# chennachaos/PFEMFort

Measured on AMD Instinct MI355X. Metric: DOF/s (assembly+CG-to-tol), higher is better.
Workload: dtype f64

## Files before the change

### include/pfem_amd_diag.h

```cpp
#ifndef PFEM_AMD_DIAG_H
#define PFEM_AMD_DIAG_H

#include "pfem_amd.h"

#ifdef __cplusplus
extern "C" {
#endif

#define PFEM_ASSEMBLY_GATHER 0
#define PFEM_ASSEMBLY_SCATTER 1
int pfem_solver_set_assembly_mode(pfem_solver *s, int mode);
int pfem_solver_assembly_info(pfem_solver *s, int *gather_form, int *hub_nodes, int *block_threads, int64_t *lds_bytes);
#define PFEM_SPMV_AUTO 0
#define PFEM_SPMV_INT32 1
#define PFEM_SPMV_GAPS16 2
#define PFEM_SPMV_GROUPED 3
int pfem_solver_set_spmv_format(pfem_solver *s, int format);
int pfem_solver_get_spmv_format(pfem_solver *s, int *bits_per_column);
int pfem_solver_get_spmv_row_group(pfem_solver *s, int *rows_per_lane);
int pfem_solver_get_spmv_gap_table(pfem_solver *s, int *entries);
int pfem_solver_get_spmv_value_dictionary(pfem_solver *s, int *entries);
int pfem_solver_amg_value_dictionaries(pfem_solver *s, int max_levels, int *n_levels, int *entries);
int pfem_solver_get_spmv_gap_escapes(pfem_solver *s, int *in_use);
int pfem_solver_spmv_bytes(pfem_solver *s, int64_t *format_bytes);

int pfem_solver_amg_info(pfem_solver *s, int max_levels, int *n_levels, int64_t *rows, int64_t *nnz, double *lambda_max,
                         double *symbolic_ms, double *numeric_ms, int *cheb_degree, int *fine_degree, double *eig_ratio, double *coarse_scale);
int pfem_solver_amg_aggregates(pfem_solver *s, int level, int32_t *agg);
int pfem_solver_amg_transfer(pfem_solver *s, int level, int *rbm, int *fine_bs, int *coarse_bs, int *dim, int64_t *n_nodes, double *node_xyz);
int pfem_solver_amg_layout(pfem_solver *s, int max_levels, int *coupled, int *distributed_levels, int64_t *first_dof, int64_t *local_rows);
int pfem_solver_incidence_patterns(pfem_solver *s, int *count, int *longest);
int pfem_solver_amg_aggregation(pfem_solver *s, int max_levels, int *n_levels, int *kind);
int pfem_solver_amg_comm_counts(pfem_solver *s, int *exchanges_per_cycle, int *allreduces_per_cycle);
int pfem_solver_amg_cycle_profile(pfem_solver *s, int max_levels, int *n_levels, int *exchanges, double *exchange_ms,
                                  int64_t *exchange_doubles, int *allreduces, double *allreduce_ms, int64_t *allreduce_doubles,
                                  double *cycle_ms);
int pfem_solver_amg_pairing(pfem_solver *s, int *lattice_levels);
int pfem_solver_amg_cycle(pfem_solver *s, int *cycle, int *last_level_visited_twice);
int pfem_solver_amg_level0_epilogue(pfem_solver *s, int *taken);
int pfem_solver_amg_galerkin_from_codes(pfem_solver *s, int *taken);
int pfem_solver_amg_level_values(pfem_solver *s, int level, int64_t max_values, double *vals, int64_t *stored);

int pfem_eval_elems(pfem_solver *s, const double *elemData, const double *timeData,
                    double *K_out, double *F_out);

int pfem_matrix_info(pfem_solver *s, int64_t *n_owned, int64_t *n_local, int64_t *nnz,
                     int64_t *stored_entries);

int pfem_spmv(pfem_solver *s, const double *x, double *y);
int pfem_bench_spmv(pfem_solver *s, int reps, double *ms_per_launch);

typedef struct pfem_timings {
    double pattern_ms;
    double assemble_ms;
    double solve_ms;
    double spmv_ms_total;
    int64_t spmv_launches;
    double upload_ms;
    double event_overhead_ms;
    double iface_ms_total;
    double scalar_ms_total;
    int64_t comm_samples;
    double exposed_ms_total;
    int64_t graph_iterations;
    double host_enqueue_ms;
    int64_t host_enqueued_iterations;
    double host_comm_ms;
} pfem_timings;
int pfem_get_timings(pfem_solver *s, pfem_timings *t);
int pfem_solver_profile_spmv(pfem_solver *s, int enable);

int pfem_solver_comm_selftest(pfem_solver *s, int64_t count, int64_t *bad);
int pfem_solver_comm_bench(pfem_solver *s, int64_t count, int reps, double *ms_per_exchange, double *ms_per_allreduce);
int pfem_solver_comm_bench_sizes(pfem_solver *s, int64_t count, int64_t allreduce_count, int reps, int slab_neighbours,
                                 double *ms_per_exchange, double *ms_per_allreduce);
int pfem_solver_comm_info(pfem_solver *s, int *n_peers, int64_t *doubles_per_exchange, int64_t *boundary_slices,
                          int64_t *total_slices);
int pfem_solver_comm_describe(pfem_solver *s, char *backend, int backend_len, int *backend_ranks, int *backend_device,
                              int *backend_version, int *solver_device, int *overlapped_form);

#ifdef __cplusplus
}
#endif
#endif
```

### pfemfort_amd/_lib.py

```python
from __future__ import annotations

import ctypes as C
import os

_HERE = os.path.dirname(os.path.abspath(__file__))
LIB_PATH = os.environ.get("PFEM_AMD_LIB") or os.path.join(_HERE, "libpfem_amd.so")

OK, ERR_ARG, ERR_STATE, ERR_NEG_JAC, ERR_HIP, ERR_NOGPU, ERR_NOMEM, ERR_DIVERGED, ERR_PATTERN, ERR_COMM = range(10)
POISSON_TRIA, POISSON_TET, ELAST_TET, POISSON_TRIA_INLINE, ELAST_TRIA = 1, 2, 3, 4, 5
SOLVER_EMPTY, PATTERN_OK, INIT_OK, ASSEMBLY_OK, FACTORISE_OK = 1, 2, 3, 4, 5
INSERT_VALUES, ADD_VALUES = 1, 2

NPELEM = {POISSON_TRIA: 3, POISSON_TET: 4, ELAST_TET: 4, POISSON_TRIA_INLINE: 3, ELAST_TRIA: 3}
NDOF = {POISSON_TRIA: 1, POISSON_TET: 1, ELAST_TET: 3, POISSON_TRIA_INLINE: 1, ELAST_TRIA: 2}
NDIM = {POISSON_TRIA: 2, POISSON_TET: 3, ELAST_TET: 3, POISSON_TRIA_INLINE: 2, ELAST_TRIA: 2}


class PfemError(RuntimeError):
    def __init__(self, code: int, where: str, detail: str = ""):
        self.code = code
        msg = f"{where}: error {code} ({_strerror(code)})"
        if detail:
            msg += f" -- {detail}"
        super().__init__(msg)
# ... 8 lines not shown
                ("host_comm_ms", C.c_double)]


HOST_ALLREDUCE_FN = C.CFUNCTYPE(C.c_int, C.c_void_p, C.POINTER(C.c_double), C.c_int64)
HOST_EXCHANGE_FN = C.CFUNCTYPE(C.c_int, C.c_void_p, C.c_int, C.POINTER(C.c_int), C.POINTER(C.c_int64),
                               C.POINTER(C.c_double), C.POINTER(C.c_double))
RCCL_ID_BYTES = 256

_P = C.c_void_p
_I, _L, _D = C.c_int, C.c_int64, C.c_double

SIGNATURES = {
    "pfem_version": [],
    "pfem_strerror": [_I],
    "pfem_last_error_string": [],
    "pfem_device_count": [_P],
    "pfem_device_info": [_I, _P, _I, _P, _P, _P],
    "pfem_device_memory": [_I, _P, _P],
    "pfem_poisson_tria_ke": [_P] * 7,
    "pfem_poisson_tet_ke": [_P] * 8,
    "pfem_elast_tet_ke": [_P] * 8,
    "pfem_elast_tria_ke": [_P] * 7,
    "pfem_gen_box_tets": [_D, _D, _I, _D, _D, _I, _D, _D, _I, _I, _I, _I, _I, _P, _P, _P, _P, _P, _P],
    "pfem_dof_numbering": [_L, _I, _L, _P, _P, _P, _I, _P, _P, _P, _P, _P, _P, _P, _P, _P, _P],
    "pfem_renumber_mesh": [_L, _I, _L, _I, _P, _P, _P, _P, _P, _P],
    "pfem_elem_dof_array": [_L, _I, _I, _P, _P, _P],
    "pfem_assy_for_soln": [_L, _I, _P, _P],
    "pfem_partition_box_slabs": [_I, _I, _I, _I, _P, _P],
    "pfem_partition_box_slabs_axis": [_I, _I, _I, _I, _I, _P, _P],
    "pfem_partition_rcb": [_L, _I, _P, _L, _I, _P, _I, _P, _P],
    "pfem_text_table_shape": [C.c_char_p, _L, _P, _P],
    "pfem_text_table_parse": [C.c_char_p, _L, _L, _I, _P],
    "pfem_write_vtk": [C.c_char_p, _I, _L, _L, _I, _I, _P, _P, _P, _P],
    "pfem_write_temp_dat": [C.c_char_p, _L, _P, _P, _P],
    "pfem_solver_create": [_P, _L, _L, _L, _P, _P, _I],
    "pfem_solver_destroy": [_P],
    "pfem_solver_set_stream": [_P, _P],
    "pfem_solver_set_tolerances": [_P, _D, _D, _D, _I],
    "pfem_solver_status": [_P, _P],
    "pfem_solver_set_zero": [_P],
    "pfem_solver_print_info": [_P],
    "pfem_mat_set_values": [_P, _I, _P, _I, _P, _P, _I],
    "pfem_vec_set_values": [_P, _I, _P, _P, _I],
    "pfem_solver_assemble_matrix_and_vector": [_P, _I, _P, _P, _P, _P],
    "pfem_solver_factorise": [_P],
    "pfem_solver_solve": [_P, _P, _P, _P],
    "pfem_solver_factorise_and_solve": [_P, _P, _P, _P],
    "pfem_solver_get_solution": [_P, _P],
    "pfem_solver_get_history": [_P, _P, _I, _P],
    "pfem_mesh_upload": [_P, _I, _L, _P, _L, _P, _P, _P],
    "pfem_box_slab_sizes": [_I, _I, _I, _I, _I, _I, _I, _P, _P, _P, _P, _P],
    "pfem_mesh_generate_box": [_P, _I, _D, _D, _I, _D, _D, _I, _D, _D, _I, _I, _I, _I],
    "pfem_box_slab_sizes_axis": [_I, _I, _I, _I, _I, _I, _I, _I, _P, _P, _P, _P, _P, _P, _P, _P],
    "pfem_mesh_generate_box_axis": [_P, _I, _D, _D, _I, _D, _D, _I, _D, _D, _I, _I, _I, _I, _I],
    "pfem_mesh_download": [_P, _P, _P, _P, _P],
    "pfem_pattern_build": [_P],
    "pfem_assemble": [_P, _P, _P],
    "pfem_solver_set_assembly_mode": [_P, _I],
    "pfem_solver_assembly_info": [_P, _P, _P, _P, _P],
    "pfem_solver_set_spmv_format": [_P, _I],
    "pfem_solver_get_spmv_format": [_P, _P],
    "pfem_solver_get_spmv_row_group": [_P, _P],
    "pfem_solver_get_spmv_gap_table": [_P, _P],
    "pfem_solver_get_spmv_value_dictionary": [_P, _P],
    "pfem_solver_amg_value_dictionaries": [_P, _I, _P, _P],
    "pfem_solver_get_spmv_gap_escapes": [_P, _P],
    "pfem_solver_spmv_bytes": [_P, _P],
    "pfem_solver_set_preconditioner": [_P, _I],
    "pfem_solver_get_preconditioner": [_P, _P],
    "pfem_solver_set_cg_single_reduction": [_P, _I],
    "pfem_solver_amg_info": [_P, _I, _P, _P, _P, _P, _P, _P, _P, _P, _P, _P],
    "pfem_solver_amg_aggregates": [_P, _I, _P],
    "pfem_solver_amg_transfer": [_P, _I, _P, _P, _P, _P, _P, _P],
    "pfem_solver_amg_layout": [_P, _I, _P, _P, _P, _P],
    "pfem_solver_amg_aggregation": [_P, _I, _P, _P],
    "pfem_solver_incidence_patterns": [_P, _P, _P],
    "pfem_solver_amg_comm_counts": [_P, _P, _P],
    "pfem_solver_amg_cycle_profile": [_P, _I, _P, _P, _P, _P, _P, _P, _P, _P],
    "pfem_solver_amg_pairing": [_P, _P],
    "pfem_solver_set_amg_options": [_P, _I, _I, _D, _D],
    "pfem_solver_set_amg_cycle": [_P, _I],
    "pfem_solver_amg_cycle": [_P, _P, _P],
    "pfem_solver_amg_level0_epilogue": [_P, _P],
    "pfem_solver_amg_galerkin_from_codes": [_P, _P],
    "pfem_solver_amg_level_values": [_P, _I, _L, _P, _P],
    "pfem_eval_elems": [_P, _P, _P, _P, _P],
    "pfem_rhs_add_values": [_P, _L, _P, _P],
    "pfem_matrix_info": [_P, _P, _P, _P, _P],
    "pfem_get_local_to_global": [_P, _P],
    "pfem_get_csr": [_P, _P, _P, _P],
    "pfem_get_rhs": [_P, _P],
    "pfem_spmv": [_P, _P, _P],
    "pfem_bench_spmv": [_P, _I, _P],
    "pfem_get_timings": [_P, _P],
    "pfem_solver_profile_spmv": [_P, _I],
    "pfem_neighbour_plan": [_I, _I, _P, _P, _P, _P, _P, _P, _P, _P, _P],
    "pfem_solver_set_neighbours": [_P, _I, _P, _P, _P],
    "pfem_rccl_unique_id": [_P],
    "pfem_solver_set_comm_rccl": [_P, _I, _I, _P],
    "pfem_solver_set_comm_host": [_P, _I, _I, HOST_ALLREDUCE_FN, HOST_EXCHANGE_FN, _P],
    "pfem_solver_comm_bench": [_P, C.c_int64, _I, _P, _P],
    "pfem_solver_comm_bench_sizes": [_P, C.c_int64, C.c_int64, _I, _I, _P, _P],
    "pfem_solver_set_comm_peer": [_P, _I, _I, HOST_ALLREDUCE_FN, HOST_EXCHANGE_FN, _P],
    "pfem_solver_comm_shutdown": [_P],
    "pfem_solver_comm_info": [_P, _P, _P, _P, _P],
    "pfem_solver_comm_describe": [_P, _P, _I, _P, _P, _P, _P, _P],
    "pfem_solver_comm_selftest": [_P, _L, _P],
    "pfem_get_ghosts": [_P, _P, _P],
    "pfem_find_ghosts": [_L, _P, _L, _L, _P, _P],
}
_RESTYPES = {"pfem_strerror": C.c_char_p, "pfem_last_error_string": C.c_char_p}

_lib = None


def lib() -> C.CDLL:
    global _lib
    if _lib is None:
        if not os.path.exists(LIB_PATH):
            raise ImportError(
                f"{LIB_PATH} not found: build the HIP extension first "
                "(python -c 'import __graft_entry__ as g; g.build()'). pfemfort_amd has no CPU fallback.")
        L = C.CDLL(LIB_PATH)
        for name, args in SIGNATURES.items():
            fn = getattr(L, name)
            fn.argtypes = args
            fn.restype = _RESTYPES.get(name, C.c_int)
        _lib = L
    return _lib


def _strerror(code: int) -> str:
    try:
        return lib().pfem_strerror(code).decode()
    except Exception:
        return "?"


def check(rc: int, where: str) -> None:
    if rc != OK:
        raise PfemError(rc, where, lib().pfem_last_error_string().decode())


def device_count() -> int:
    n = C.c_int(0)
    check(lib().pfem_device_count(C.byref(n)), "pfem_device_count")
    return n.value


def device_memory(device: int = 0) -> dict:
    f = C.c_int64(0); t = C.c_int64(0)
    check(lib().pfem_device_memory(device, C.byref(f), C.byref(t)), "pfem_device_memory")
    return {"free_bytes": f.value, "total_bytes": t.value}


def device_info(device: int = 0) -> dict:
    name = C.create_string_buffer(256)
    cu = C.c_int(0); mem = C.c_int64(0); clk = C.c_int(0)
    check(lib().pfem_device_info(device, name, 256, C.byref(cu), C.byref(mem), C.byref(clk)), "pfem_device_info")
    return {"name": name.value.decode(), "compute_units": cu.value, "hbm_bytes": mem.value, "clock_khz": clk.value}
```

### pfemfort_amd/csrc/pfem_amg.inc

```

constexpr int kAmgMaxLevels = 14;
constexpr int kAmgMatchRounds = 8;
constexpr int kAmgPasses = 3;
constexpr int64_t kAmgReplicateRows = 150000;
constexpr int kAmgRetryBlock = -7701;

inline bool amg_in_effect(const pfem_solver *s)
{
    return s->pc == PFEM_PC_GAMG;
}

inline SellDev amg_sell(const pfem_solver *s, const AmgLevel &L, int64_t rows)
{
    SellDev A;
    if (L.fine) {
        A = s->sell();
    } else {
        A.slice_off = L.slice_off.p;
        A.rowlen = L.rowlen.p;
        A.cols = L.cols.p;
        A.vals = L.vals.p;
    }
    A.n_rows = rows;
    A.n_slices = (rows + 63) / 64;
// ... 467 lines not shown
    PFEM_TRY(cand.reserve(static_cast<size_t>(n)));
    PFEM_TRY(is_root.reserve(static_cast<size_t>(n) + 1));
    PFEM_TRY(rank.reserve(static_cast<size_t>(n) + 1));
    PFEM_HIP(hipMemsetAsync(match.p, 0xff, sizeof(int32_t) * n, s->stream));
    const int64_t *gptr = G.ptr.p;
    const int32_t *gcol = G.col.p;
    const double *gw = G.w.p, *gd = G.diag.p;
    hipLaunchKernelGGL(k_amg_lat_pick, dim3(grid_for(n)), dim3(kBlock), 0, s->stream, n, gptr, gcol, gw, gd, pos, shift, cand.p);
    hipLaunchKernelGGL(k_amg_match_commit, dim3(grid_for(n)), dim3(kBlock), 0, s->stream, n, static_cast<const int32_t *>(cand.p), match.p);
    if (absorb) {
        hipLaunchKernelGGL(k_amg_lat_absorb, dim3(grid_for(n)), dim3(kBlock), 0, s->stream, n, gptr, gcol, gw, gd, pos, shift,
                           static_cast<const int32_t *>(match.p), cand.p);
        hipLaunchKernelGGL(k_amg_lat_join, dim3(grid_for(n)), dim3(kBlock), 0, s->stream, n, static_cast<const int32_t *>(cand.p), match.p);
    }
    PFEM_TRY(check_kernel("k_amg_lat_*"));
    PFEM_HIP(hipMemsetAsync(is_root.p + n, 0, sizeof(int32_t), s->stream));
    hipLaunchKernelGGL(k_amg_match_finish, dim3(grid_for(n)), dim3(kBlock), 0, s->stream, n, match.p, is_root.p);
    PFEM_TRY(amg_exclusive_sum(s, temp, is_root.p, rank.p, n + 1));
    PFEM_TRY(agg_step.reserve(static_cast<size_t>(n)));
    hipLaunchKernelGGL(k_amg_agg_ids, dim3(grid_for(n)), dim3(kBlock), 0, s->stream, n, static_cast<const int32_t *>(match.p),
                       static_cast<const int32_t *>(rank.p), agg_step.p);
    PFEM_TRY(check_kernel("k_amg_agg_ids"));
    int32_t total = 0;
    PFEM_HIP(hipMemcpyAsync(&total, rank.p + n, sizeof(int32_t), hipMemcpyDeviceToHost, s->stream));
    PFEM_HIP(hipStreamSynchronize(s->stream));
    *na = total;
    return PFEM_OK;
}

int amg_sell_from_keys(pfem_solver *s, AmgWork &W, const uint64_t *ukeys, int64_t nnz, AmgLevel &C)
{
    DevBuf<char> &temp = W.temp;
    const int64_t n = C.n_loc;
    C.nnz = nnz;
    C.n_slices = (n + 63) / 64;
    PFEM_TRY(C.rowptr.alloc(static_cast<size_t>(n) + 1));
    PFEM_TRY(C.rowlen.alloc(static_cast<size_t>(std::max<int64_t>(n, 1))));
    PFEM_TRY(C.slice_off.alloc(static_cast<size_t>(C.n_slices) + 1));
    DevBuf<int64_t> &slice_entries = W.slice_entries;
    PFEM_TRY(slice_entries.reserve(static_cast<size_t>(C.n_slices) + 1));
    hipLaunchKernelGGL(k_row_bounds, dim3(grid_for(std::max<int64_t>(nnz, n + 1))), dim3(kBlock), 0, s->stream, ukeys, nnz, n, C.rowptr.p);
    hipLaunchKernelGGL(k_slice_sizes, dim3(grid_for(C.n_slices * 64)), dim3(kBlock), 0, s->stream, static_cast<const int64_t *>(C.rowptr.p), n,
                       C.n_slices, C.rowlen.p, slice_entries.p);
    PFEM_TRY(check_kernel("k_slice_sizes (gamg)"));
    PFEM_TRY(amg_exclusive_sum(s, temp, slice_entries.p, C.slice_off.p, C.n_slices + 1));
    int64_t stored = 0;
    PFEM_HIP(hipMemcpyAsync(&stored, C.slice_off.p + C.n_slices, sizeof(int64_t), hipMemcpyDeviceToHost, s->stream));
    PFEM_HIP(hipStreamSynchronize(s->stream));
    C.stored = stored;
    PFEM_TRY(C.cols.alloc(static_cast<size_t>(std::max<int64_t>(stored, 1))));
    PFEM_TRY(C.vals.alloc(static_cast<size_t>(std::max<int64_t>(stored, 1))));
    hipLaunchKernelGGL(k_fill_sell, dim3(grid_for(C.n_slices * 64)), dim3(kBlock), 0, s->stream, ukeys, static_cast<const int64_t *>(C.rowptr.p), n,
                       C.n_slices, static_cast<const int64_t *>(C.slice_off.p), C.cols.p);
    PFEM_TRY(check_kernel("k_fill_sell (gamg)"));
    PFEM_HIP(hipMemsetAsync(C.vals.p, 0, sizeof(double) * std::max<int64_t>(stored, 1), s->stream));
    return PFEM_OK;
}

int amg_alloc_vectors(pfem_solver *s, AmgLevel &L)
{
    const size_t n = static_cast<size_t>(std::max<int64_t>(L.n_loc, 1));
    const size_t g = L.fine ? static_cast<size_t>(kVecGuard) : 0;
    const size_t nv = n;
    PFEM_TRY(L.dinv.alloc(n));
    PFEM_TRY(L.t.alloc(nv));
    PFEM_TRY(L.r.alloc(n));
    if (!L.fine) PFEM_TRY(L.b.alloc(n));
    PFEM_TRY(L.x_store.alloc(nv + 2 * g));
    PFEM_TRY(L.dd_store.alloc(nv + 2 * g));
    PFEM_HIP(hipMemsetAsync(L.x_store.p, 0, sizeof(double) * (nv + 2 * g), s->stream));
    PFEM_HIP(hipMemsetAsync(L.dd_store.p, 0, sizeof(double) * (nv + 2 * g), s->stream));
    L.x = L.x_store.p + g;
    L.dd = L.dd_store.p + g;
    PFEM_TRY(L.lam.alloc(1));
    PFEM_TRY(L.part_max.alloc(static_cast<size_t>(grid_for((L.n_loc + 63) / 64 * 64))));
    return PFEM_OK;
}

inline bool amg_galerkin_by_entry()
{
    static const bool v = std::getenv("PFEM_AMG_GALERKIN_MAPS") != nullptr;
    return v;
}
inline void amg_galerkin(pfem_solver *s, const AmgLevel &L, AmgLevel &C, const SellDev &A, bool extras = false, VdState *vstate = nullptr,
                         bool from_codes = false)
{
    C.bound_fresh = C.vd_direct = false;
    if (L.code_of.p && !amg_galerkin_by_entry()) {
        if (C.n_loc < 1) return;
        LatGalExtra X{nullptr, nullptr, nullptr, nullptr, nullptr};
        if (extras && C.dinv.p && C.t.p && C.n_loc == C.n) {
            X.dinv_out = C.dinv.p;
            X.ratio_out = C.t.p;
            C.bound_fresh = true;
            if (vstate && C.vd_have_dict && C.vd_hash_ok && C.vhash.p && C.vcodes.p && C.vcodes.n >= static_cast<size_t>(C.stored) && !C.vd_refused) {
                const VdState reset{C.vd_n, 0, 0, 0};
                (void)hipMemcpyAsync(vstate, &reset, sizeof reset, hipMemcpyHostToDevice, s->stream);
                X.vhash = C.vhash.p;
                X.codes = C.vcodes.p;
                X.vstate = vstate;
                C.vd_direct = true;
            }
        }
        if (from_codes) {
            hipLaunchKernelGGL(k_lat_galerkin_codes, dim3(static_cast<unsigned>((C.n_loc + kLatGalThreads - 1) / kLatGalThreads)), dim3(kLatGalThreads),
                               sizeof(double) * static_cast<size_t>(std::max(s->vd_n, 1)), s->stream, C.n_loc, static_cast<const int32_t *>(L.mem_ptr.p),
                               static_cast<const int32_t *>(L.mem_idx.p), static_cast<const int64_t *>(s->d_rslice_off.p),
                               static_cast<const unsigned long long *>(s->d_vcodes.p), static_cast<const uint32_t *>(L.glat.p),
                               static_cast<const double *>(s->d_vdict.p), s->vd_n, static_cast<const uint32_t *>(L.code_mask.p),
                               static_cast<const int64_t *>(C.slice_off.p), C.vals.p, X);
            return;
        }
        hipLaunchKernelGGL(k_lat_galerkin, dim3(static_cast<unsigned>((C.n_loc + kLatGalThreads - 1) / kLatGalThreads)), dim3(kLatGalThreads), 0, s->stream, A, C.n_loc,
                           static_cast<const int32_t *>(L.mem_ptr.p), static_cast<const int32_t *>(L.mem_idx.p), static_cast<const uint8_t *>(L.code_of.p),
                           static_cast<const uint32_t *>(L.code_mask.p), static_cast<const int64_t *>(C.slice_off.p), C.vals.p, X);
        return;
    }
    hipLaunchKernelGGL(k_amg_galerkin, dim3(grid_for(L.nnz_c)), dim3(kBlock), 0, s->stream, L.nnz_c, static_cast<const int64_t *>(L.src_ptr.p),
                       static_cast<const int32_t *>(L.src_slot.p), static_cast<const int64_t *>(L.dst_slot.p),
                       static_cast<const double *>(A.vals), C.vals.p);
}

int amg_couple_level(pfem_solver *s, AmgWork &W, AmgLevel &L, AmgLevel &C, bool overlap, int cb, const std::vector<double> *nc_of)
{
    std::vector<int64_t> rank_off;
    if (cb > 0 && nc_of) {
        rank_off.assign(nc_of->size() + 1, 0);
        for (size_t q = 0; q < nc_of->size(); ++q) rank_off[q + 1] = rank_off[q] + static_cast<int64_t>((*nc_of)[q]);
    }
    auto node_base = [&](int64_t g) -> int64_t {
        const size_t q = static_cast<size_t>(std::upper_bound(rank_off.begin(), rank_off.end(), g) - rank_off.begin()) - 1;
        return rank_off[q] + (g - rank_off[q]) / cb * cb;
    };
    const PlanRef P = amg_plan(s, L);
    const std::vector<int32_t> &fine_lidx = L.fine ? s->h_send_lidx : L.plan.send_lidx;
    const int64_t n = L.n, n_loc = L.n_loc, n_ghost = n_loc - n, nc = C.n;
    double bad = s->nranks > 52 ? 1.0 : 0.0;
    DevBuf<double> &v = W.vals;
    DevBuf<double> &w = W.svals;
    DevBuf<double> d_mask, d_gm;
    DevBuf<int32_t> d_table;
    DevBuf<uint64_t> &gkeys = W.keys, &gskeys = W.skeys, &gukeys = W.ukeys;
    DevBuf<int32_t> &gidx = W.idx, &gsidx = W.skey32;
    DevBuf<int64_t> &gstart = W.start;
    {
        int rc = v.reserve(static_cast<size_t>(std::max<int64_t>(n_loc, 1)));
        if (rc == PFEM_OK) rc = w.reserve(static_cast<size_t>(std::max<int64_t>(n_loc, 1)));
        if (rc == PFEM_OK) rc = d_mask.alloc(static_cast<size_t>(std::max<int64_t>(nc, 1)));
        if (rc == PFEM_OK) rc = d_gm.alloc(static_cast<size_t>(std::max<int64_t>(n_ghost, 1)));
        if (rc == PFEM_OK) rc = d_table.alloc(static_cast<size_t>(std::max<int64_t>(n_ghost, 1)));
        if (rc == PFEM_OK) rc = gkeys.reserve(static_cast<size_t>(std::max<int64_t>(n_ghost, 1)));
        if (rc == PFEM_OK) rc = gskeys.reserve(static_cast<size_t>(std::max<int64_t>(n_ghost, 1)));
        if (rc == PFEM_OK) rc = gidx.reserve(static_cast<size_t>(std::max<int64_t>(n_ghost, 1)));
        if (rc == PFEM_OK) rc = gsidx.reserve(static_cast<size_t>(std::max<int64_t>(n_ghost, 1)));
        if (rc == PFEM_OK) rc = W.head.reserve(static_cast<size_t>(n_ghost) + 1);
        if (rc == PFEM_OK) rc = W.rank.reserve(static_cast<size_t>(n_ghost) + 1);
        if (rc == PFEM_OK) rc = gukeys.reserve(static_cast<size_t>(std::max<int64_t>(n_ghost, 1)));
        if (rc == PFEM_OK) rc = gstart.reserve(static_cast<size_t>(n_ghost) + 1);
        if (rc == PFEM_OK && n_ghost > 0) {
            size_t tb = 0;
            if (hipcub::DeviceRadixSort::SortPairs(nullptr, tb, gkeys.p, gskeys.p, gidx.p, gsidx.p, static_cast<int>(n_ghost), 0, 40, s->stream) != hipSuccess) rc = PFEM_ERR_HIP;
            if (rc == PFEM_OK && tb > W.temp.n) { (void)hipStreamSynchronize(s->stream); rc = W.temp.alloc(tb); }
            size_t ts = 0;
            if (rc == PFEM_OK && hipcub::DeviceScan::ExclusiveSum(nullptr, ts, W.head.p, W.rank.p, static_cast<int>(n_ghost + 1), s->stream) != hipSuccess) rc = PFEM_ERR_HIP;
            if (rc == PFEM_OK && ts > W.temp.n) { (void)hipStreamSynchronize(s->stream); rc = W.temp.alloc(ts); }
        }
        PFEM_TRY(amg_agree(s, rc));
    }
    bool self_peer = false;
    for (int k = 0; k < P.np; ++k) self_peer = self_peer || P.peers[k] == s->rank;
    const double undo = self_peer ? 0.5 : 1.0;
    auto as_id = [undo](double x) { return static_cast<int64_t>(undo * x + 0.5); };
    hipLaunchKernelGGL(k_amg_gid_vector, dim3(grid_for(n_loc)), dim3(kBlock), 0, s->stream, n, n_loc, static_cast<const int32_t *>(L.agg.p), C.gid_off, v.p);
    PFEM_TRY(check_kernel("k_amg_gid_vector"));
    PFEM_TRY(exchange_sum(s, P, v.p, overlap));
    std::vector<double> h_sh(static_cast<size_t>(P.n_send));
    std::vector<uint64_t> h_ug;
    int64_t m_g = 0;
    {
        auto ghosts = [&]() -> int {
            if (P.n_send > 0) {
                hipLaunchKernelGGL(k_pack_send, dim3(grid_for(P.n_send)), dim3(kBlock), 0, s->stream, static_cast<const double *>(v.p), P.send_lidx, P.n_send,
                                   s->d_send.p, static_cast<const CgCtl *>(nullptr));
                PFEM_HIP(hipMemcpyAsync(h_sh.data(), s->d_send.p, sizeof(double) * h_sh.size(), hipMemcpyDeviceToHost, s->stream));
            }
            if (n_ghost > 0) {
                hipLaunchKernelGGL(k_amg_ghost_keys, dim3(grid_for(n_ghost)), dim3(kBlock), 0, s->stream, n_ghost, static_cast<const double *>(v.p + n), undo,
                                   gkeys.p, gidx.p);
                size_t tb = W.temp.n;
                PFEM_HIP(hipcub::DeviceRadixSort::SortPairs(W.temp.p, tb, gkeys.p, gskeys.p, gidx.p, gsidx.p, static_cast<int>(n_ghost), 0, 40, s->stream));
                PFEM_TRY(amg_unique_runs(s, W, gskeys.p, n_ghost, gukeys, gstart, &m_g, false));
                h_ug.resize(static_cast<size_t>(m_g));
                if (m_g > 0) PFEM_HIP(hipMemcpyAsync(h_ug.data(), gukeys.p, sizeof(uint64_t) * h_ug.size(), hipMemcpyDeviceToHost, s->stream));
            }
            PFEM_HIP(hipStreamSynchronize(s->stream));
            return PFEM_OK;
        };
        const int rc = ghosts();
        if (rc != PFEM_OK) bad = 1.0;
    }
    std::vector<int32_t> table;
    C.ghost_gid.clear();
    if (cb > 0) {
// ... 1452 lines not shown
        }
        if (L.bs > 1) {
            PFEM_TRY(C.node_of.alloc(static_cast<size_t>(nc)));
            PFEM_TRY(C.comp_of.alloc(static_cast<size_t>(nc)));
            hipLaunchKernelGGL(k_amg_coarse_nodes, dim3(grid_for(nslots)), dim3(kBlock), 0, s->stream, nslots, L.bs,
                               static_cast<const int32_t *>(flag.p), static_cast<const int32_t *>(rank.p), C.node_of.p, C.comp_of.p);
            PFEM_TRY(check_kernel("k_amg_coarse_nodes"));
        }
        {
            DevBuf<int32_t> &cnt = W.cnt, &idx = W.idx, &skey = W.skey32;
            PFEM_TRY(cnt.reserve(static_cast<size_t>(nc_loc) + 1));
            PFEM_TRY(idx.reserve(static_cast<size_t>(std::max<int64_t>(R, 1))));
            PFEM_TRY(skey.reserve(static_cast<size_t>(std::max<int64_t>(R, 1))));
            PFEM_TRY(L.mem_ptr.alloc(static_cast<size_t>(nc_loc) + 1));
            PFEM_TRY(L.mem_idx.alloc(static_cast<size_t>(std::max<int64_t>(R, 1))));
            PFEM_HIP(hipMemsetAsync(cnt.p, 0, sizeof(int32_t) * (nc_loc + 1), s->stream));
            hipLaunchKernelGGL(k_amg_count, dim3(grid_for(R)), dim3(kBlock), 0, s->stream, R, static_cast<const int32_t *>(L.agg.p), cnt.p);
            PFEM_TRY(amg_exclusive_sum(s, temp, cnt.p, L.mem_ptr.p, nc_loc + 1));
            hipLaunchKernelGGL(k_amg_iota, dim3(grid_for(R)), dim3(kBlock), 0, s->stream, R, idx.p);
            size_t tb = 0;
            const int ni = static_cast<int>(R);
            PFEM_HIP(hipcub::DeviceRadixSort::SortPairs(nullptr, tb, L.agg.p, skey.p, idx.p, L.mem_idx.p, ni, 0, 32, s->stream));
            if (tb > temp.n) { PFEM_HIP(hipStreamSynchronize(s->stream)); PFEM_TRY(temp.alloc(tb)); }
            PFEM_HIP(hipcub::DeviceRadixSort::SortPairs(temp.p, tb, L.agg.p, skey.p, idx.p, L.mem_idx.p, ni, 0, 32, s->stream));
            PFEM_HIP(hipStreamSynchronize(s->stream));
        }
        phase(l, "coarse dofs + member lists");
        {
            DevBuf<uint64_t> &keys = W.keys, &skeys = W.skeys;
            DevBuf<uint64_t> ukeys;
            DevBuf<int32_t> &slots = W.slots;
            PFEM_TRY(keys.reserve(static_cast<size_t>(L.stored)));
            PFEM_TRY(slots.reserve(static_cast<size_t>(L.stored)));
            PFEM_HIP(hipMemsetAsync(keys.p, 0xff, sizeof(uint64_t) * static_cast<size_t>(L.stored), s->stream));
            PFEM_HIP(hipMemsetAsync(slots.p, 0, sizeof(int32_t) * static_cast<size_t>(L.stored), s->stream));
            const SellDev Ar = amg_sell(s, L, R);
            hipLaunchKernelGGL(k_amg_emit_rap_keys, dim3(grid_for(Ar.n_slices * 64)), dim3(kBlock), 0, s->stream, Ar,
                               static_cast<const int32_t *>(L.agg.p), static_cast<int32_t>(R), keys.p, slots.p);
            PFEM_TRY(check_kernel("k_amg_emit_rap_keys"));
            PFEM_TRY(skeys.reserve(static_cast<size_t>(L.stored)));
            PFEM_TRY(L.src_slot.alloc(static_cast<size_t>(L.stored)));
            const int ni = static_cast<int>(L.stored);
            size_t tb = 0;
            PFEM_HIP(hipcub::DeviceRadixSort::SortPairs(nullptr, tb, keys.p, skeys.p, slots.p, L.src_slot.p, ni, 0, 64, s->stream));
            if (tb > temp.n) { PFEM_HIP(hipStreamSynchronize(s->stream)); PFEM_TRY(temp.alloc(tb)); }
            PFEM_HIP(hipcub::DeviceRadixSort::SortPairs(temp.p, tb, keys.p, skeys.p, slots.p, L.src_slot.p, ni, 0, 64, s->stream));
            PFEM_HIP(hipStreamSynchronize(s->stream));
            int64_t nnz_c = 0;
            PFEM_TRY(amg_unique_runs(s, W, skeys.p, L.stored, ukeys, L.src_ptr, &nnz_c));
            if (nnz_c > 0) {
                uint64_t last = 0;
                PFEM_HIP(hipMemcpyAsync(&last, ukeys.p + (nnz_c - 1), sizeof(uint64_t), hipMemcpyDeviceToHost, s->stream));
                PFEM_HIP(hipStreamSynchronize(s->stream));
                if (last == ~0ull) --nnz_c;
            }
            L.nnz_c = nnz_c;
            PFEM_TRY(amg_sell_from_keys(s, W, ukeys.p, nnz_c, C));
            PFEM_TRY(L.dst_slot.alloc(static_cast<size_t>(std::max<int64_t>(nnz_c, 1))));
            hipLaunchKernelGGL(k_amg_dst_slots, dim3(grid_for(nnz_c)), dim3(kBlock), 0, s->stream, nnz_c, static_cast<const uint64_t *>(ukeys.p),
                               static_cast<const int64_t *>(C.rowptr.p), static_cast<const int64_t *>(C.slice_off.p), L.dst_slot.p);
            PFEM_TRY(check_kernel("k_amg_dst_slots"));
            PFEM_HIP(hipStreamSynchronize(s->stream));
        }
        phase(l, "Galerkin maps + coarse pattern");
        if (coupled) PFEM_TRY(amg_agree(s, C.stored > INT_MAX ? PFEM_ERR_ARG : PFEM_OK));
        else if (C.stored > INT_MAX) return PFEM_ERR_ARG;
        M.lev.push_back(std::move(Cp));
        {
            AmgLevel &Cn = *M.lev.back();
            amg_galerkin(s, L, Cn, A);
            PFEM_TRY(check_kernel("k_amg_galerkin (symbolic)"));
        }
        n_global = nc_global;
        if (coupled && n_global > kAmgDense && n_global <= static_cast<double>(replicate_rows)) {
            PFEM_TRY(amg_replicate(s, M, W, *M.lev.back(), static_cast<int64_t>(n_global), overlap));
            phase(l, "replicated levels");
            break;
        }
    }
    M.n_last_global = coupled ? static_cast<int64_t>(n_global) : M.lev.back()->n;
    return PFEM_OK;
}

int amg_finish_levels(pfem_solver *s, Amg &M, bool coupled)
{
    for (auto &L : M.lev) PFEM_TRY(amg_alloc_vectors(s, *L));
    AmgLevel &last = *M.lev.back();
    const int64_t n_last = M.n_last_global;
    M.dense = n_last >= 1 && n_last <= kAmgDense && M.lev.size() > 1 && !M.rep;
    if (M.dense) {
        PFEM_TRY(M.dense_inv.alloc(static_cast<size_t>(n_last * n_last)));
        const int bytes = static_cast<int>(n_last * n_last * sizeof(double));
        if (bytes > 65536) {
            PFEM_HIP(hipFuncSetAttribute(reinterpret_cast<const void *>(k_amg_dense_inverse), hipFuncAttributeMaxDynamicSharedMemorySize, bytes));
            PFEM_HIP(hipFuncSetAttribute(reinterpret_cast<const void *>(k_amg_dense_inverse_of), hipFuncAttributeMaxDynamicSharedMemorySize, bytes));
        }
        if (coupled) {
            PFEM_TRY(M.dense_glob.alloc(static_cast<size_t>(n_last * n_last)));
            PFEM_TRY(M.bx_glob.alloc(static_cast<size_t>(2 * kAmgDense)));
            PFEM_TRY(amg_level_gids(s, last));
        }
    }
    if (coupled) PFEM_TRY(M.lam_all.alloc(static_cast<size_t>(std::max<int64_t>(256, 2 * static_cast<int64_t>(M.lev.size()) * s->nranks))));
    M.fused = !coupled && [] { const char *e = std::getenv("PFEM_AMG_FUSED"); return e ? std::atoi(e) != 0 : true; }();
    M.tail_from = -1;
    for (size_t l = 1; l < M.lev.size() && !coupled; ++l)
        if (M.lev[l]->n <= kAmgTailRows && M.lev[l]->nnz <= kAmgTailNnz && M.lev.size() - l <= static_cast<size_t>(kAmgTailLevels)) { M.tail_from = static_cast<int>(l); break; }
    M.w_to = M.tail_from > 0 ? M.tail_from : static_cast<int>(M.lev.size()) - 2;
    M.tail_lds_allowed = 0;
    if (M.tail_from > 0) {
        int64_t rows = 0;
        for (size_t l = static_cast<size_t>(M.tail_from); l < M.lev.size(); ++l) rows += M.lev[l]->n;
        const AmgLevel &T0 = *M.lev[static_cast<size_t>(M.tail_from)];
        const size_t need = static_cast<size_t>(6 * rows) * sizeof(double) + static_cast<size_t>(T0.stored) * 12 + static_cast<size_t>((T0.n + 63) / 64 + 2) * 8;
        if (need > 65536 && need <= 156 * 1024) {
            if (hipFuncSetAttribute(reinterpret_cast<const void *>(k_amg_tail), hipFuncAttributeMaxDynamicSharedMemorySize, static_cast<int>(need)) == hipSuccess)
                M.tail_lds_allowed = need;
            else
                (void)hipGetLastError();
        }
    }
    return PFEM_OK;
}


void amg_knobs(Amg &M)
{
    const char *er = std::getenv("PFEM_AMG_EIG_RATIO"), *cs = std::getenv("PFEM_AMG_COARSE_SCALE");
    M.eig_ratio = er ? std::max(1.5, std::atof(er)) : (M.eig_ratio_given ? M.eig_ratio_opt : M.eig_ratio_auto);
    M.coarse_scale = cs ? std::atof(cs) : (M.coarse_scale_given ? M.coarse_scale_opt : M.coarse_scale_auto);
    if (M.rep) { M.rep->eig_ratio = M.eig_ratio; M.rep->coarse_scale = M.coarse_scale; }
}

int amg_symbolic(pfem_solver *s, bool multi, bool overlap)
{
    if (!s->amg) s->amg.reset(new (std::nothrow) Amg());
    if (!s->amg) return PFEM_ERR_NOMEM;
    Amg &M = *s->amg;
    const auto t0 = std::chrono::steady_clock::now();
    const bool verbose = std::getenv("PFEM_AMG_VERBOSE") != nullptr;
    const size_t malloc_calls0 = dev_pool().st_malloc_calls;
    const size_t malloc_bytes0 = dev_pool().st_malloc;
    const double malloc_ms0 = dev_pool().st_malloc_ms;
    const size_t reused0 = dev_pool().st_reused;
    auto since_t0 = [&](const char *what) {
        if (!verbose) return;
        (void)hipStreamSynchronize(s->stream);
        std::fprintf(stderr, "  gamg symbolic: %-40s at %9.2f ms\n", what, std::chrono::duration<double, std::milli>(std::chrono::steady_clock::now() - t0).count());
    };
    M.coupled = multi && !M.coupled_refused && [] { const char *e = std::getenv("PFEM_AMG_COUPLED"); return e ? std::atoi(e) != 0 : true; }();
    const bool coupled = M.coupled;
    if (const char *e = std::getenv("PFEM_AMG_CHEB_DEGREE")) M.cheb_degree = std::max(1, std::min(6, std::atoi(e)));
    if (const char *e = std::getenv("PFEM_AMG_FINE_DEGREE")) M.fine_degree = std::max(0, std::min(6, std::atoi(e)));
    M.lev.clear();
    M.rep.reset();
    M.rbm = false;
    M.symbolic_ok = false;
    M.dense = false;
    M.graph.invalidate();
    {
        const int rc_size = s->stored > INT_MAX ? PFEM_ERR_ARG : PFEM_OK;
        if (rc_size != PFEM_OK) set_last_error("gamg: more than 2^31-1 stored matrix entries on one device");
        if (coupled) PFEM_TRY(amg_agree(s, rc_size));
        else PFEM_TRY(rc_size);
    }
    std::unique_ptr<AmgWork> Wp(new (std::nothrow) AmgWork());
    if (!Wp) return PFEM_ERR_NOMEM;
    AmgWork &W = *Wp;
    {
        std::unique_ptr<AmgLevel> L0(new (std::nothrow) AmgLevel());
        if (!L0) return PFEM_ERR_NOMEM;
        L0->fine = true;
        L0->n = s->n_owned;
        L0->n_loc = s->n_loc;
        L0->gid_off = s->row_start;
        L0->n_slices = (s->n_owned + 63) / 64;
        L0->stored = s->stored;
        L0->nnz = s->nnz;
        int64_t owned_groups = s->n_groups;
        if (s->grouped && s->n_groups > 0 && s->n_ghost > 0) {
            std::vector<int32_t> row0(static_cast<size_t>(s->n_groups));
            PFEM_HIP(hipMemcpyAsync(row0.data(), s->d_group_row0.p, sizeof(int32_t) * row0.size(), hipMemcpyDeviceToHost, s->stream));
            PFEM_HIP(hipStreamSynchronize(s->stream));
            owned_groups = std::lower_bound(row0.begin(), row0.end(), static_cast<int32_t>(s->n_owned)) - row0.begin();
        }
        if (s->grouped && owned_groups > 0 && owned_groups < s->n_owned) {
            L0->bs = kGroupRows;
            L0->n_nodes = owned_groups;
            PFEM_TRY(L0->node_of.alloc(static_cast<size_t>(s->n_loc)));
            PFEM_TRY(L0->comp_of.alloc(static_cast<size_t>(s->n_loc)));
            hipLaunchKernelGGL(k_row_group_index, dim3(grid_for(s->n_groups)), dim3(kBlock), 0, s->stream,
                               static_cast<const int32_t *>(s->d_group_row0.p), s->n_groups, L0->node_of.p);
            hipLaunchKernelGGL(k_amg_comp_of, dim3(grid_for(s->n_loc)), dim3(kBlock), 0, s->stream, s->n_loc,
                               static_cast<const int32_t *>(L0->node_of.p), static_cast<const int32_t *>(s->d_group_row0.p), L0->comp_of.p);
            PFEM_TRY(check_kernel("k_amg_comp_of"));
        } else {
            L0->bs = 1;
            L0->n_nodes = s->n_owned;
        }
        if (!multi || coupled) {
            const int nd = s->mesh.ndof;
            bool cand = s->have_mesh && nd == s->mesh.ndim && nd >= 2 && s->n_owned % nd == 0 && s->n_loc % nd == 0 && (multi || s->n_owned >= 2 * nd);
            const int64_t nn0 = cand ? s->n_loc / nd : 0;
// ... 238 lines not shown
    if (any_old) {
        PFEM_TRY(read_states());
        for (int l : cand) {
            AmgLevel &L = *M.lev[static_cast<size_t>(l)];
            if (!L.vd_have_dict) continue;
            if (st[static_cast<size_t>(l)].miss) build.push_back(l);
            else { L.vd_ok = true; L.vd_hash_ok = L.vhash.p != nullptr; }
        }
    }
    if (build.empty()) return PFEM_OK;
    for (int l : build) {
        AmgLevel &L = *M.lev[static_cast<size_t>(l)];
        const unsigned grid = static_cast<unsigned>(std::min<int64_t>((L.stored + kBlock - 1) / kBlock, 4096));
        PFEM_HIP(hipMemsetAsync(L.vtable.p, 0xff, sizeof(unsigned long long) * kVdTable, s->stream));
        PFEM_HIP(hipMemsetAsync(M.vd_states.p + l, 0, sizeof(VdState), s->stream));
        hipLaunchKernelGGL(k_vd_collect, dim3(grid), dim3(kBlock), 0, s->stream, static_cast<const double *>(L.vals.p), L.stored, L.vtable.p, M.vd_states.p + l);
        hipLaunchKernelGGL(k_vd_finish, dim3(1), dim3(1024), 0, s->stream, static_cast<const unsigned long long *>(L.vtable.p), L.vdict.p, M.vd_states.p + l);
        PFEM_TRY(check_kernel("k_vd_collect / k_vd_finish (coarse level)"));
        L.vd_hash_ok = false;
        if (!L.vhash.p) PFEM_TRY(L.vhash.alloc(kVdHashSlots));
        PFEM_HIP(hipMemsetAsync(L.vhash.p, 0xff, sizeof(VdHashEntry) * kVdHashSlots, s->stream));
        hipLaunchKernelGGL(k_vd_hash_build, dim3((kVdMax + kBlock - 1) / kBlock), dim3(kBlock), 0, s->stream, static_cast<const double *>(L.vdict.p),
                           static_cast<const VdState *>(M.vd_states.p + l), L.vhash.p);
        PFEM_TRY(check_kernel("k_vd_hash_build (coarse level)"));
        PFEM_TRY(encode(L, l));
    }
    PFEM_TRY(read_states());
    for (int l : build) {
        AmgLevel &L = *M.lev[static_cast<size_t>(l)];
        const VdState &v = st[static_cast<size_t>(l)];
        if (v.fail || v.count < 1 || v.count > kVdMax || v.miss) {
            L.vd_ok = L.vd_have_dict = L.vd_hash_ok = false;
            L.vd_refused = true;
        } else {
            L.vd_n = v.count;
            L.vd_have_dict = true;
            L.vd_ok = true;
            L.vd_hash_ok = L.vhash.p != nullptr;
        }
        if (std::getenv("PFEM_VD_VERBOSE"))
            std::fprintf(stderr, "  value dictionary, level %d: %d distinct values among %lld slots%s\n", l, v.count, static_cast<long long>(L.stored),
                         L.vd_ok ? "" : " -- the level keeps its fp64 values");
    }
    return PFEM_OK;
}

int amg_level0_codes(pfem_solver *s, Amg &M, AmgLevel &L, bool *yes)
{
    *yes = false;
    const char *e = std::getenv("PFEM_AMG_GALERKIN_CODES");
    if (e && std::atoi(e) == 0) return PFEM_OK;
    if (&M != s->amg.get() || M.coupled || M.rbm || cg_multi(s) || !L.fine || L.rbm || L.bs != 1 || !L.code_of.p || !L.code_mask.p || amg_galerkin_by_entry() ||
        s->n_hubs != 0 || L.stored != s->stored || L.glat_refused)
        return PFEM_OK;
    if (!valdict_enabled() || !s->use_rel() || s->rel_gap32 || s->vd_rows != kRelRows || !(s->vd_ok && s->vd_current && s->vd_have_dict) || s->vd_miss_step ||
        s->vd_n < 1 || s->vd_n > kVdMax || !s->d_vcodes.p || !s->d_vdict.p || !s->d_relk.p || !s->d_rslice_off.p || s->r_stored < 1 ||
        s->d_vcodes.n < static_cast<size_t>(s->r_stored))
        return PFEM_OK;
    if (!L.glat.p || L.glat_for != s->r_stored) {
        PFEM_TRY(L.glat.alloc(static_cast<size_t>(s->r_stored)));
        L.glat_for = -1;
        PFEM_HIP(hipMemsetAsync(L.glat.p, 0xff, sizeof(uint32_t) * static_cast<size_t>(s->r_stored), s->stream));
        PFEM_HIP(hipMemsetAsync(s->d_err.p, 0, sizeof(int), s->stream));
        hipLaunchKernelGGL(k_lat_group_codes, dim3(grid_for(L.n)), dim3(kBlock), 0, s->stream, amg_sell(s, L), static_cast<const uint8_t *>(L.code_of.p),
                           static_cast<const uint8_t *>(s->d_relk.p), static_cast<const int64_t *>(s->d_rslice_off.p), reinterpret_cast<uint8_t *>(L.glat.p),
                           s->d_err.p);
        PFEM_TRY(check_kernel("k_lat_group_codes"));
        int bad = 0;
        PFEM_TRY(fetch_err(s, &bad));
        PFEM_HIP(hipMemsetAsync(s->d_err.p, 0, sizeof(int), s->stream));
        if (bad) { L.glat.release(); L.glat_refused = true; return PFEM_OK; }
        L.glat_for = s->r_stored;
    }
    *yes = true;
    return PFEM_OK;
}

int amg_numeric(pfem_solver *s, Amg &M, bool overlap)
{
    M.galerkin_from_codes = false;
    if (M.coupled) return amg_numeric_coupled(s, M, overlap);
    const bool fresh = M.galerkin_fresh;
    M.galerkin_fresh = false;
    for (size_t l = 0; l < M.lev.size(); ++l) {
        AmgLevel &L = *M.lev[l];
        const SellDev A = amg_sell(s, L);
        if (l + 1 < M.lev.size() && !fresh) {
            AmgLevel &C = *M.lev[l + 1];
            if (L.rbm) amg_rbm_galerkin(s, L, C, A);
            else {
                bool from_codes = false;
                if (l == 0) PFEM_TRY(amg_level0_codes(s, M, L, &from_codes));
                amg_galerkin(s, L, C, A, !M.rbm && !M.coupled, M.vd_states.p ? M.vd_states.p + (l + 1) : nullptr, from_codes);
                if (from_codes) M.galerkin_from_codes = true;
                if (l == 0 && std::getenv("PFEM_VD_VERBOSE"))
                    std::fprintf(stderr, "  gamg numeric: level 1 summed from %s\n", from_codes ? "the SpMV's value codes" : "the fp64 row form");
            }
        }
        const unsigned g = grid_for(A.n_slices * 64);
        if (!L.fine && L.bound_fresh && !fresh) {
            L.bound_fresh = false;
            if (L.n > 65536) {
                const unsigned gm = std::min<unsigned>(g, 512u);
                hipLaunchKernelGGL(k_amg_max_rows, dim3(gm), dim3(kBlock), 0, s->stream, static_cast<const double *>(L.t.p), L.n, L.part_max.p);
                hipLaunchKernelGGL(k_amg_max, dim3(1), dim3(1024), 0, s->stream, static_cast<const double *>(L.part_max.p), static_cast<int64_t>(gm), L.lam.p);
            } else {
                hipLaunchKernelGGL(k_amg_max, dim3(1), dim3(1024), 0, s->stream, static_cast<const double *>(L.t.p), L.n, L.lam.p);
            }
            continue;
        }
        if (L.fine && s->asm_bound_fresh && &M == s->amg.get()) {
            const unsigned gm = std::min<unsigned>(g, 2048u);
            hipLaunchKernelGGL(k_amg_max_rows, dim3(gm), dim3(kBlock), 0, s->stream, static_cast<const double *>(L.t.p), L.n, L.part_max.p);
            hipLaunchKernelGGL(k_amg_max, dim3(1), dim3(1024), 0, s->stream, static_cast<const double *>(L.part_max.p), static_cast<int64_t>(gm), L.lam.p);
            s->asm_bound_fresh = false;
        } else {
        hipLaunchKernelGGL(k_amg_diag_bound, dim3(g), dim3(kBlock), 0, s->stream, A, static_cast<int32_t>(L.n), L.dinv.p, L.part_max.p);
        hipLaunchKernelGGL(k_amg_max, dim3(1), dim3(1024), 0, s->stream, static_cast<const double *>(L.part_max.p), static_cast<int64_t>(g), L.lam.p);
        }
        if (M.rbm) {
            if (!M.lam2.p) PFEM_TRY(M.lam2.alloc(1));
            hipLaunchKernelGGL(k_rbm_bound_sym, dim3(g), dim3(kBlock), 0, s->stream, A, static_cast<int32_t>(L.n), static_cast<const double *>(L.dinv.p),
                               static_cast<double *>(nullptr), L.part_max.p);
            hipLaunchKernelGGL(k_amg_max, dim3(1), dim3(1024), 0, s->stream, static_cast<const double *>(L.part_max.p), static_cast<int64_t>(g), M.lam2.p);
            hipLaunchKernelGGL(k_rbm_min2, dim3(1), dim3(64), 0, s->stream, static_cast<const double *>(M.lam2.p), L.lam.p);
        }
    }
    PFEM_TRY(check_kernel("gamg numeric"));
    if (M.dense) {
        AmgLevel &L = *M.lev.back();
        hipLaunchKernelGGL(k_amg_dense_inverse, dim3(1), dim3(1024), static_cast<size_t>(L.n * L.n) * sizeof(double), s->stream, amg_sell(s, L),
                           M.dense_inv.p);
        PFEM_TRY(check_kernel("k_amg_dense_inverse"));
    }
    return amg_value_codes(s, M);
}

inline void amg_rbm_restrict_launch(pfem_solver *s, const AmgLevel &L, AmgLevel &C, int64_t nc_nodes, int64_t nn, const double *b, const double *t, double ratio,
                                    double *dd_c, double *x_c, const CgCtl *ctl, int64_t n_own_nodes)
{
    static const bool wide_on = [] { const char *e = std::getenv("PFEM_RBM_RESTRICT_WIDE"); return e ? std::atoi(e) != 0 : true; }();
    const bool wide = wide_on && nc_nodes > 0 && nn >= 16 * nc_nodes;
    if (wide) {
        PFEM_RBM_DISPATCH(L.bs, L.dim, hipLaunchKernelGGL((k_rbm_restrict_wide<FB, DIM>), dim3(grid_for(nc_nodes * kRbmWide)), dim3(kBlock), 0, s->stream, nc_nodes,
            static_cast<const int32_t *>(L.mem_ptr.p), static_cast<const int32_t *>(L.mem_idx.p), static_cast<const double *>(L.roff.p), nn,
            b, t, C.b.p, static_cast<const double *>(C.dinv.p), static_cast<const double *>(C.lam.p), ratio, dd_c, x_c, ctl, n_own_nodes));
    } else {
        PFEM_RBM_DISPATCH(L.bs, L.dim, hipLaunchKernelGGL((k_rbm_restrict<FB, DIM>), dim3(grid_for(nc_nodes)), dim3(kBlock), 0, s->stream, nc_nodes,
            static_cast<const int32_t *>(L.mem_ptr.p), static_cast<const int32_t *>(L.mem_idx.p), static_cast<const double *>(L.roff.p), nn,
            b, t, C.b.p, static_cast<const double *>(C.dinv.p), static_cast<const double *>(C.lam.p), ratio, dd_c, x_c, ctl, n_own_nodes));
    }
}

int amg_smooth(pfem_solver *s, const Amg &M, AmgLevel &L, const double *b, bool zero_guess, int deg, const CgCtl *ctl, bool first_done = false,
               bool overlap = false)
{
    const int64_t nv = amg_rows(M, L);
    const unsigned gv = vec_grid(nv);
    const double *t0 = nullptr;
    const PlanRef P = M.coupled ? amg_plan(s, L) : PlanRef{};
    const bool cf = M.coupled && M.coupled_fused && P.row_sh != nullptr;
    const ShareSum S = cf ? ShareSum{P.row_sh, P.sh_ptr, P.sh_src, s->d_recv.p} : ShareSum{nullptr, nullptr, nullptr, nullptr};
    auto product = [&](const double *x) -> int {
        if (!cf) {
            amg_spmv(s, M, L, x, L.t.p);
            if (M.coupled) PFEM_TRY(exchange_sum(s, P, L.t.p, overlap, ctl));
            return PFEM_OK;
        }
        if (L.fine) {
            amg_spmv(s, M, L, x, L.t.p);
            if (P.n_send > 0)
                hipLaunchKernelGGL(k_pack_send, dim3(grid_for(P.n_send)), dim3(kBlock), 0, s->stream, static_cast<const double *>(L.t.p), P.send_lidx, P.n_send,
                                   s->d_send.p, ctl);
        } else {
            const SellDev A = amg_sell(s, L, nv);
            if (L.vd_ok && L.vcodes.p)
                hipLaunchKernelGGL(k_amg_spmv_pack_vd, dim3(spmv_grid(A.n_slices)), dim3(kBlock), sizeof(double) * static_cast<size_t>(L.vd_n), s->stream, A,
                                   static_cast<const uint16_t *>(L.vcodes.p), static_cast<const double *>(L.vdict.p), L.vd_n, x, L.t.p, S, s->d_send.p, ctl);
            else
            hipLaunchKernelGGL(k_amg_spmv_pack, dim3(spmv_grid(A.n_slices)), dim3(kBlock), 0, s->stream, A, x, L.t.p, S, s->d_send.p, ctl);
        }
        return exchange_only(s, P, overlap);
    };
    if (!zero_guess) {
        PFEM_TRY(product(L.x));
        t0 = L.t.p;
    }
    double *r_store = (deg > 1 && !zero_guess) ? L.r.p : nullptr;
    if (!first_done)
        hipLaunchKernelGGL(k_amg_cheb_first, dim3(gv), dim3(kBlock), 0, s->stream, nv, b, t0, static_cast<const double *>(L.dinv.p),
                           static_cast<const double *>(L.lam.p), M.eig_ratio, r_store, deg > 1 ? L.dd : static_cast<double *>(nullptr), L.x, ctl, S);
    const double *r_in = zero_guess ? b : L.r.p;
    for (int k = 1; k < deg; ++k) {
        PFEM_TRY(product(L.dd));
        const bool more = k + 1 < deg;
        hipLaunchKernelGGL(k_amg_cheb_next, dim3(gv), dim3(kBlock), 0, s->stream, nv, k, r_in, static_cast<const double *>(L.t.p),
                           static_cast<const double *>(L.dinv.p), static_cast<const double *>(L.lam.p), M.eig_ratio, more ? L.r.p : nullptr,
                           static_cast<const double *>(L.dd), more ? L.dd : nullptr, L.x, ctl, S);
        r_in = L.r.p;
    }
    return PFEM_OK;
}

enum { kLast0Smooth = 0, kLast0Product = 1, kLast0Epilogue = 2 };
double *amg_apply(pfem_solver *s, Amg &M, const double *r, const CgCtl *ctl, bool first0_done = false, int last0 = kLast0Smooth);
double *amg_apply_coupled(pfem_solver *s, Amg &M, const double *r, const CgCtl *ctl, bool overlap)
{
    const int nl = static_cast<int>(M.lev.size());
    {
// ... 46 lines not shown
        if (amg_smooth(s, M, L, b, true, deg_of(l), ctl, false, overlap) != PFEM_OK) return nullptr;
        amg_spmv(s, M, L, L.x, L.t.p);
        if (L.rbm)
            amg_rbm_restrict_launch(s, L, C, C.n_loc / C.bs, L.n_loc / L.bs, b, static_cast<const double *>(L.t.p), M.eig_ratio, nullptr, nullptr, ctl, L.n_nodes);
        {
            const PlanRef PC = amg_plan(s, C);
            const bool cf = M.coupled_fused && PC.row_sh != nullptr && !L.rbm;
            const ShareSum SC = cf ? ShareSum{PC.row_sh, PC.sh_ptr, PC.sh_src, s->d_recv.p} : ShareSum{nullptr, nullptr, nullptr, nullptr};
            if (!L.rbm)
            hipLaunchKernelGGL(k_amg_restrict, dim3(grid_for(C.n_loc)), dim3(kBlock), 0, s->stream, C.n_loc, static_cast<const int32_t *>(L.mem_ptr.p),
                           static_cast<const int32_t *>(L.mem_idx.p), b, static_cast<const double *>(L.t.p), C.b.p, static_cast<const double *>(C.dinv.p),
                           static_cast<const double *>(C.lam.p), M.eig_ratio, static_cast<double *>(nullptr), static_cast<double *>(nullptr), ctl,
                           static_cast<int32_t>(L.n), SC, s->d_send.p);
            if (cf) {
                if (exchange_only(s, PC, overlap) != PFEM_OK) return nullptr;
                if (PC.n_sh > 0)
                    hipLaunchKernelGGL(k_unpack_sum, dim3(grid_for(PC.n_sh)), dim3(kBlock), 0, s->stream, C.b.p, PC.sh_lidx, PC.sh_ptr, PC.sh_src, PC.n_sh,
                                       static_cast<const double *>(s->d_recv.p), ctl);
            } else if (exchange_sum(s, PC, C.b.p, overlap, ctl) != PFEM_OK) {
                return nullptr;
            }
        }
    }
    for (int l = nl - 2; l >= 0; --l) {
        AmgLevel &L = *M.lev[static_cast<size_t>(l)];
        AmgLevel &C = *M.lev[static_cast<size_t>(l) + 1];
        const double *b = l == 0 ? r : L.b.p;
        s->xprof_level = l;
        if (L.rbm) {
            PFEM_RBM_DISPATCH(L.bs, L.dim, hipLaunchKernelGGL((k_rbm_prolong<FB, DIM>), dim3(vec_grid(L.n_loc / L.bs)), dim3(kBlock), 0, s->stream, L.n_loc / L.bs,
                static_cast<const int32_t *>(L.node_agg.p), static_cast<const double *>(L.roff.p), L.n_loc / L.bs, static_cast<const double *>(C.x),
                M.coarse_scale, L.x, ctl));
        } else
        hipLaunchKernelGGL(k_amg_prolong, dim3(vec_grid(L.n_loc)), dim3(kBlock), 0, s->stream, L.n_loc, static_cast<const int32_t *>(L.agg.p),
                           static_cast<const double *>(C.x), M.coarse_scale, L.x, ctl);
        if (amg_smooth(s, M, L, b, false, deg_of(l), ctl, false, overlap) != PFEM_OK) return nullptr;
    }
    return M.lev[0]->x;
}

double *amg_apply(pfem_solver *s, Amg &M, const double *r, const CgCtl *ctl, bool first0_done, int last0)
{
    const int nl = static_cast<int>(M.lev.size());
    if (M.lev[0]->fine && s->n_ghost > 0) (void)hipMemsetAsync(M.lev[0]->x + s->n_owned, 0, sizeof(double) * static_cast<size_t>(s->n_ghost), s->stream);
    const bool fuse = M.fused && M.cheb_degree == 2;
    const int tail = (M.fused && M.tail_from > 0) ? M.tail_from : nl;
    auto deg_of = [&](int l) { return (l == 0 && M.fine_degree > 0) ? M.fine_degree : M.cheb_degree; };
    auto fused_level = [&](int l) { return fuse && l >= 1 && l < tail && l < nl - 1; };
    auto ep = [&](int mode, AmgLevel &L, const double *xin, const double *r_in, int step, int add_dd0, double *r_out, double *dd_out, double *x) {
        const SellDev A = amg_sell(s, L);
        const dim3 grid(spmv_grid(A.n_slices)), block(kBlock);
        const double *dinv = L.dinv.p, *lam = L.lam.p;
        if (L.gptr.p && (L.bs == 6 || L.bs == 3)) {
            const int64_t *gp = L.gptr.p;
            const int32_t *gc = L.gcol.p;
#define PFEM_BLK_EP(MODEV, CBV) hipLaunchKernelGGL((k_rbm_spmv_ep<MODEV, CBV>), grid, block, 0, s->stream, A, gp, gc, xin, r_in, dinv, lam, M.eig_ratio, step, add_dd0, r_out, dd_out, x, ctl)
            if (L.bs == 6) { if (mode == kEpNextLast) PFEM_BLK_EP(kEpNextLast, 6); else if (mode == kEpResid) PFEM_BLK_EP(kEpResid, 6); else PFEM_BLK_EP(kEpFirstRes, 6); }
            else { if (mode == kEpNextLast) PFEM_BLK_EP(kEpNextLast, 3); else if (mode == kEpResid) PFEM_BLK_EP(kEpResid, 3); else PFEM_BLK_EP(kEpFirstRes, 3); }
#undef PFEM_BLK_EP
            return;
        }
        if (L.vd_ok && L.vcodes.p) {
            const uint16_t *q = L.vcodes.p;
            const double *d = L.vdict.p;
            const size_t lds = sizeof(double) * static_cast<size_t>(L.vd_n);
            if (mode == kEpNextLast) hipLaunchKernelGGL(k_amg_spmv_ep_vd<kEpNextLast>, grid, block, lds, s->stream, A, q, d, L.vd_n, xin, r_in, dinv, lam, M.eig_ratio, step, add_dd0, r_out, dd_out, x, ctl);
            else if (mode == kEpResid) hipLaunchKernelGGL(k_amg_spmv_ep_vd<kEpResid>, grid, block, lds, s->stream, A, q, d, L.vd_n, xin, r_in, dinv, lam, M.eig_ratio, step, add_dd0, r_out, dd_out, x, ctl);
            else hipLaunchKernelGGL(k_amg_spmv_ep_vd<kEpFirstRes>, grid, block, lds, s->stream, A, q, d, L.vd_n, xin, r_in, dinv, lam, M.eig_ratio, step, add_dd0, r_out, dd_out, x, ctl);
            return;
        }
        if (mode == kEpNextLast) hipLaunchKernelGGL(k_amg_spmv_ep<kEpNextLast>, grid, block, 0, s->stream, A, xin, r_in, dinv, lam, M.eig_ratio, step, add_dd0, r_out, dd_out, x, ctl);
        else if (mode == kEpResid) hipLaunchKernelGGL(k_amg_spmv_ep<kEpResid>, grid, block, 0, s->stream, A, xin, r_in, dinv, lam, M.eig_ratio, step, add_dd0, r_out, dd_out, x, ctl);
        else hipLaunchKernelGGL(k_amg_spmv_ep<kEpFirstRes>, grid, block, 0, s->stream, A, xin, r_in, dinv, lam, M.eig_ratio, step, add_dd0, r_out, dd_out, x, ctl);
    };
    auto run_tail = [&]() {
        AmgTail T{};
        T.nlev = nl - tail;
        T.deg = M.cheb_degree;
        T.coarsest_deg = M.coarsest_sweeps;
        T.dense_n = M.dense ? static_cast<int>(M.lev.back()->n) : 0;
        T.dense_inv = M.dense_inv.p;
        T.ratio = M.eig_ratio;
        T.scale = M.coarse_scale;
        for (int q = 0; q < T.nlev; ++q) {
            AmgLevel &L = *M.lev[static_cast<size_t>(tail + q)];
            AmgTailLevel &t = T.lev[q];
            t.A = amg_sell(s, L);
            t.dinv = L.dinv.p; t.lam = L.lam.p;
            t.x = L.x; t.dd = L.dd; t.t = L.t.p; t.r = L.r.p; t.b = L.b.p;
            t.agg = L.agg.p; t.mem_ptr = L.mem_ptr.p; t.mem_idx = L.mem_idx.p;
            t.n = L.n; t.nc = L.nc; t.stored = L.stored;
            t.rbm_dim = L.rbm ? L.dim : 0; t.fb = L.bs; t.nn = L.n_nodes; t.node_agg = L.node_agg.p; t.roff = L.roff.p;
        }
        int64_t rows = 0;
        for (int q = 0; q < T.nlev; ++q) rows += T.lev[q].n;
        const size_t vec_b = static_cast<size_t>(6 * rows) * sizeof(double);
        const bool use_lds = vec_b <= 65536;
        const AmgTailLevel &t0 = T.lev[0];
        const size_t mat_b = (T.nlev > 1 && t0.stored > 0) ? static_cast<size_t>(t0.stored) * 12 + static_cast<size_t>(t0.A.n_slices + 2) * 8 : 0;
        const bool mat = use_lds && mat_b > 0 && vec_b + mat_b <= 156 * 1024;
        const size_t lds = use_lds ? vec_b + (mat ? mat_b : 0) : 0;
        const bool mat_ok = mat && (lds <= 65536 || lds <= M.tail_lds_allowed);
        hipLaunchKernelGGL(k_amg_tail, dim3(1), dim3(1024), use_lds ? (mat_ok ? lds : vec_b) : 0, s->stream, T, ctl, use_lds ? 1 : 0,
                           mat_ok ? t0.stored : static_cast<int64_t>(0));
    };
    std::function<void(int)> visit = [&](int l) {
        AmgLevel &L = *M.lev[static_cast<size_t>(l)];
        const double *b = l == 0 ? r : L.b.p;
        if (l == tail) { run_tail(); return; }
        if (l == nl - 1) {
            if (M.dense) {
                hipLaunchKernelGGL(k_amg_dense_apply, dim3(1), dim3(kAmgDense), 0, s->stream, static_cast<int>(L.n),
                                   static_cast<const double *>(M.dense_inv.p), b, L.x, ctl);
            } else {
                (void)amg_smooth(s, M, L, b, true, nl == 1 ? M.cheb_degree : M.coarsest_sweeps, ctl);
            }
            return;
        }
        AmgLevel &C = *M.lev[static_cast<size_t>(l) + 1];
        const double *res = nullptr, *res_t = nullptr;
        if (fused_level(l)) {
            ep(kEpNextLast, L, L.dd, b, 1, 0, nullptr, nullptr, L.x);
            ep(kEpResid, L, L.x, b, 0, 0, L.r.p, nullptr, nullptr);
            res = L.r.p;
        } else {
            (void)amg_smooth(s, M, L, b, true, deg_of(l), ctl, l == 0 && first0_done);
            amg_spmv(s, M, L, L.x, L.t.p);
            res = b;
            res_t = L.t.p;
        }
        const bool first_below = fused_level(l + 1);
        if (L.rbm) {
            amg_rbm_restrict_launch(s, L, C, C.n_nodes, L.n_nodes, res, res_t, M.eig_ratio, first_below ? C.dd : static_cast<double *>(nullptr),
                                    first_below ? C.x : static_cast<double *>(nullptr), ctl, L.n_nodes);
        } else
        hipLaunchKernelGGL(k_amg_restrict, dim3(grid_for(C.n)), dim3(kBlock), 0, s->stream, C.n, static_cast<const int32_t *>(L.mem_ptr.p),
                           static_cast<const int32_t *>(L.mem_idx.p), res, res_t, C.b.p, static_cast<const double *>(C.dinv.p),
                           static_cast<const double *>(C.lam.p), M.eig_ratio, first_below ? C.dd : static_cast<double *>(nullptr),
                           first_below ? C.x : static_cast<double *>(nullptr), ctl);
        visit(l + 1);
        if (M.cycle_gamma > 1 && l + 1 <= M.w_to && l + 1 < nl - 1 && C.x1.p) {
            amg_spmv(s, M, C, C.x, C.t.p);
            hipLaunchKernelGGL(k_amg_w_between, dim3(vec_grid(C.n)), dim3(kBlock), 0, s->stream, C.n, C.b.p, static_cast<const double *>(C.t.p), C.x, C.x1.p,
                               static_cast<const double *>(C.dinv.p), static_cast<const double *>(C.lam.p), M.eig_ratio,
                               first_below ? C.dd : static_cast<double *>(nullptr), ctl);
            visit(l + 1);
            hipLaunchKernelGGL(k_amg_w_add, dim3(vec_grid(C.n)), dim3(kBlock), 0, s->stream, C.n, C.x, static_cast<const double *>(C.x1.p), ctl);
        }
        if (L.rbm) {
            PFEM_RBM_DISPATCH(L.bs, L.dim, hipLaunchKernelGGL((k_rbm_prolong<FB, DIM>), dim3(vec_grid(L.n_nodes)), dim3(kBlock), 0, s->stream, L.n_nodes,
                static_cast<const int32_t *>(L.node_agg.p), static_cast<const double *>(L.roff.p), L.n_nodes, static_cast<const double *>(C.x),
                M.coarse_scale, L.x, ctl));
        } else
        hipLaunchKernelGGL(k_amg_prolong, dim3(vec_grid(L.n)), dim3(kBlock), 0, s->stream, L.n, static_cast<const int32_t *>(L.agg.p),
                           static_cast<const double *>(C.x), M.coarse_scale, L.x, ctl);
        if (fused_level(l)) {
            ep(kEpFirstRes, L, L.x, b, 0, 0, L.r.p, L.dd, nullptr);
            ep(kEpNextLast, L, L.dd, L.r.p, 1, 1, nullptr, nullptr, L.x);
        } else if (l == 0 && last0 == kLast0Epilogue) {
            const unsigned gs = spmv_blocks(s);
            double *prz = s->d_part_ep.p, *pzz = prz + gs, *frz = pzz + gs, *fzz = frz + kFoldBlocks;
            launch_spmv_level0_ep(s, L.x, Level0Ep{b, L.dinv.p, L.lam.p, M.eig_ratio, L.t.p, prz, pzz}, ctl);
            hipLaunchKernelGGL(k_fold_partials2, dim3(kFoldBlocks, 2), dim3(kBlock), 0, s->stream, static_cast<const double *>(prz),
                               static_cast<const double *>(pzz), static_cast<int>(gs), frz, fzz, ctl);
        } else if (l == 0 && last0 == kLast0Product) {
            amg_spmv(s, M, L, L.x, L.t.p);
        } else {
            (void)amg_smooth(s, M, L, b, false, deg_of(l), ctl);
        }
    };
    visit(0);
    return last0 == kLast0Epilogue ? M.lev[0]->t.p : M.lev[0]->x;
}

int amg_cycle_shape(pfem_solver *s, Amg &M)
{
    if (const char *e = std::getenv("PFEM_AMG_CYCLE")) M.cycle_gamma = (e[0] == 'w' || e[0] == 'W' || e[0] == '2') ? 2 : 1;
    else if (!M.cycle_given) M.cycle_gamma = 1;
    if (M.coupled) M.cycle_gamma = 1;
    if (M.cycle_gamma > 1)
        for (int l = 1; l <= M.w_to && l + 1 < static_cast<int>(M.lev.size()); ++l) {
            AmgLevel &L = *M.lev[static_cast<size_t>(l)];
            if (L.x1.n < static_cast<size_t>(std::max<int64_t>(L.n_loc, 1))) PFEM_TRY(L.x1.alloc(static_cast<size_t>(std::max<int64_t>(L.n_loc, 1))));
        }
    return PFEM_OK;
}

int run_pcg_amg(pfem_solver *s)
{
    const int64_t n = s->n_loc;
    const bool multi = cg_multi(s);
    mark_group_vals(s);
    PFEM_TRY(refresh_group_vals(s));
    bool overlap = false;
    PFEM_TRY(agree_overlap(s, multi, &overlap));
    PFEM_TRY(cg_require_comm(s, multi));
    if (multi && !s->rhs_summed) {
        PFEM_TRY(exchange_sum(s, s->d_rhs.p, overlap));
        s->rhs_summed = true;
    }
    bool did_symbolic = false;
    if (!s->amg || !s->amg->symbolic_ok) {
        did_symbolic = true;
        int rc = amg_symbolic(s, multi, overlap);
        if (rc == kAmgRetryBlock) {
            s->amg->coupled_refused = true;
            rc = amg_symbolic(s, multi, overlap);
        }
        PFEM_TRY(rc);
        s->asm_bound_fresh = false;
        for (auto &L : s->amg->lev) L->bound_fresh = L->vd_direct = false;
    }
    Amg &M = *s->amg;
    amg_knobs(M);
    PFEM_TRY(amg_cycle_shape(s, M));
    M.coupled_fused = [] { const char *e = std::getenv("PFEM_AMG_COUPLED_FUSED"); return e ? std::atoi(e) != 0 : true; }();
    if (M.coupled && M.coupled_fused && !s->d_row_sh.p && s->n_loc > 0) {
        PFEM_TRY(s->d_row_sh.alloc(static_cast<size_t>(s->n_loc)));
        PFEM_HIP(hipMemsetAsync(s->d_row_sh.p, 0xff, sizeof(int32_t) * static_cast<size_t>(s->n_loc), s->stream));
        if (s->n_sh > 0)
            hipLaunchKernelGGL(k_amg_fill_row_sh, dim3(grid_for(s->n_sh)), dim3(kBlock), 0, s->stream, s->n_sh, static_cast<const int32_t *>(s->d_sh_lidx.p), s->d_row_sh.p);
        PFEM_TRY(check_kernel("k_amg_fill_row_sh (level 0)"));
    }
    if (!M.ev_num0) PFEM_HIP(hipEventCreate(&M.ev_num0));
    if (!M.ev_num1) PFEM_HIP(hipEventCreate(&M.ev_num1));
    hipEvent_t ea = M.ev_num0, eb = M.ev_num1;
    PFEM_HIP(hipEventRecord(ea, s->stream));
    M.galerkin_fresh = did_symbolic;
    if (M.rep) M.rep->galerkin_fresh = did_symbolic;
    PFEM_TRY(amg_numeric(s, M, overlap));
    PFEM_HIP(hipEventRecord(eb, s->stream));
    const unsigned gv = vec_grid(n), gs = spmv_blocks(s);
    const dim3 block(kBlock);
    if (s->d_part_pw.n < gs + 2) PFEM_TRY(s->d_part_pw.alloc(gs + 2));
    double *part_pw = s->d_part_pw.p, *part_rz = s->d_part.p, *part_zz = s->d_part.p + kMaxGrid, *scal_pw = s->d_part.p + 2 * kMaxGrid;
    double *sbuf = s->d_sbuf.p;
    CgCtl *ctl = s->d_ctl.p;
    PFEM_TRY(cg_reset_control(s, ctl));
    double host_comm_s = 0.0;
    const int deg0 = M.fine_degree > 0 ? M.fine_degree : M.cheb_degree;
    const bool fuse_first0 = M.fused && M.lev.size() > 1 && !M.coupled;
    const bool fuse_last0 = M.fused && M.lev.size() > 1 && deg0 == 1 && !M.coupled;
    const bool rows4 = !multi && spmv_has_level0_ep(s);
    const bool ep0 = rows4 && fuse_last0;
    const int last0 = ep0 ? kLast0Epilogue : (fuse_last0 ? kLast0Product : kLast0Smooth);
    M.level0_ep = ep0;
    if (rows4 && s->d_part_ep.n < 2 * static_cast<size_t>(gs) + 2 * kFoldBlocks) PFEM_TRY(s->d_part_ep.alloc(2 * static_cast<size_t>(gs) + 2 * kFoldBlocks));
    double *ep_rz = s->d_part_ep.p, *ep_zz = ep_rz ? ep_rz + gs : nullptr, *fold_rz = ep_rz ? ep_zz + gs : nullptr, *fold_zz = ep_rz ? fold_rz + kFoldBlocks : nullptr;
    bool use_vgraph = false;
    {
        const int graph_env = cg_graph_env();
        const bool coupled_capturable = multi && M.coupled && !overlap && s->comm && s->comm->capturable() && s->comm->p2p_capturable() &&
                                        (!M.rep || M.n_last_global <= s->comm->allreduce_capture_limit());
        if ((!multi || coupled_capturable) && graph_env && s->stream != nullptr) {
            std::vector<uint64_t> key = {reinterpret_cast<uint64_t>(s->d_r.p), reinterpret_cast<uint64_t>(ctl), reinterpret_cast<uint64_t>(s->stream),
                                         reinterpret_cast<uint64_t>(s->d_vals.p), reinterpret_cast<uint64_t>(s->d_cols.p), reinterpret_cast<uint64_t>(s->d_rvals.p),
                                         reinterpret_cast<uint64_t>(s->d_gvals.p), reinterpret_cast<uint64_t>(s->d_dwords.p), spmv_key(s),
                                         static_cast<uint64_t>(M.cheb_degree), static_cast<uint64_t>(M.fine_degree), static_cast<uint64_t>(M.dense),
                                         static_cast<uint64_t>(M.eig_ratio * 1e6), static_cast<uint64_t>(M.coarse_scale * 1e6), static_cast<uint64_t>(M.lev.size()),
                                         static_cast<uint64_t>(M.fused), static_cast<uint64_t>(M.tail_from + 1), static_cast<uint64_t>(M.coupled),
                                         static_cast<uint64_t>(M.cycle_gamma), static_cast<uint64_t>(M.w_to + 1),
                                         static_cast<uint64_t>(M.coupled_fused), reinterpret_cast<uint64_t>(s->d_send.p), reinterpret_cast<uint64_t>(s->d_recv.p),
                                         reinterpret_cast<uint64_t>(s->comm), reinterpret_cast<uint64_t>(M.rep.get()), reinterpret_cast<uint64_t>(M.bx_glob.p),
                                         static_cast<uint64_t>(last0), ep0 ? reinterpret_cast<uint64_t>(s->d_part_ep.p) : 0, ep0 ? static_cast<uint64_t>(gs) : 0,
                                         reinterpret_cast<uint64_t>(M.lev[0]->t.p), reinterpret_cast<uint64_t>(M.lev[0]->dinv.p)};
            auto level_key = [&](const std::unique_ptr<AmgLevel> &L) {
                key.push_back(reinterpret_cast<uint64_t>(L->x)); key.push_back(reinterpret_cast<uint64_t>(L->vals.p)); key.push_back(static_cast<uint64_t>(L->n));
                key.push_back(L->vd_ok ? static_cast<uint64_t>(L->vd_n + 1) : 0); key.push_back(reinterpret_cast<uint64_t>(L->vcodes.p));
            };
            for (auto &L : M.lev) level_key(L);
            if (M.rep) for (auto &L : M.rep->lev) level_key(L);
            PFEM_TRY(M.graph.ensure(s->stream, std::move(key), {s->stream}, [&](int) {
                if (M.coupled) return amg_apply_coupled(s, M, s->d_r.p, ctl, overlap) != nullptr;
                (void)amg_apply(s, M, s->d_r.p, ctl, fuse_first0, last0);
                return true;
            }, &use_vgraph));
        }
    }
    auto precondition = [&](const CgCtl *c) -> double * {
        if (use_vgraph && c == ctl) {
            if (hipGraphLaunch(M.graph.exec[0], s->stream) != hipSuccess) return nullptr;
            return ep0 ? M.lev[0]->t.p : M.lev[0]->x;
        }
        if (M.coupled) return amg_apply_coupled(s, M, s->d_r.p, c, overlap);
        double *z = amg_apply(s, M, s->d_r.p, c, c == ctl && fuse_first0, c == ctl ? last0 : kLast0Smooth);
        if (c == ctl && fuse_last0) return z;
        if (multi && exchange_sum(s, z, overlap) != PFEM_OK) return nullptr;
        return z;
    };
    auto dots = [&](double *z, const CgCtl *c, hipEvent_t *cev) -> int {
        if (c == ctl && ep0) return PFEM_OK;
        if (c == ctl && rows4) {
            hipLaunchKernelGGL(k_pc_dots_rows4, dim3(gs), block, 0, s->stream, c, s->n_owned, static_cast<const double *>(s->d_r.p),
                               static_cast<const double *>(z), ep_rz, ep_zz);
// ... 120 lines not shown
```

### pfemfort_amd/csrc/pfem_amg_kernels.hpp

```cpp
#pragma once

namespace pfem {

__device__ __forceinline__ int64_t amg_edge_key(int32_t i, int32_t j, int32_t hi_, int32_t hj_, double w, double di, double dj)
{
    if (!(w < 0.0) || !(di > 0.0) || !(dj > 0.0)) return -1;
    const double s = -w / sqrt(di * dj);
    int b = static_cast<int>(floor(8.0 * log2(s))) + 2048;
    b = b < 1 ? 1 : (b > 4095 ? 4095 : b);
    const int64_t lo = hi_ < hj_ ? hi_ : hj_, hi = hi_ < hj_ ? hj_ : hi_;
    const int64_t close = 0x7fffffffLL - (hi - lo);
    const int64_t par = (lo & 1) == 0;
    const int64_t a = i < j ? i : j, c = i < j ? j : i;
    const int64_t h = ((a * 2654435761LL + c * 40503LL) >> 7) & 0x7ffffLL;
    return (static_cast<int64_t>(b) << 51) | (close << 20) | (par << 19) | h;
}

__global__ void __launch_bounds__(kBlock) k_amg_match_pick(int64_t n, const int64_t *__restrict__ gptr, const int32_t *__restrict__ gcol,
                                                            const double *__restrict__ gw, const double *__restrict__ gdiag,
                                                            const int32_t *__restrict__ hint ,
                                                            const int32_t *__restrict__ match, int32_t *__restrict__ cand)
{
    const int64_t i = static_cast<int64_t>(blockIdx.x) * kBlock + threadIdx.x;
    if (i >= n) return;
// ... 345 lines not shown
                                                             int32_t *__restrict__ n_entries, int32_t *__restrict__ n_pairs, int *__restrict__ too_long)
{
    __shared__ uint16_t cnt[kLatCodes][kBlock];
    const int64_t I = static_cast<int64_t>(blockIdx.x) * kBlock + threadIdx.x;
    if (I == na) { n_entries[na] = 0; n_pairs[na] = 0; }
    if (I >= na) return;
    const int t = threadIdx.x;
#pragma unroll
    for (int c = 0; c < kLatCodes; ++c) cnt[c][t] = 0;
    const int32_t pc = pos_c[I];
    const int bix = pc & 0x3ff, biy = (pc >> 10) & 0x3ff, biz = (pc >> 20) & 0x3ff;
    int pairs = 0;
    for (int32_t m = mem_ptr[I]; m < mem_ptr[I + 1]; ++m) {
        const int64_t i = mem_idx[m];
        const int64_t base = A.slice_off[i >> 6] + (i & 63);
        const int len = A.rowlen[i];
        pairs += len;
        for (int k = 0; k < len; ++k) ++cnt[lat_code(B, pos[A.cols[base + 64LL * k]], bix, biy, biz)][t];
    }
    int entries = 0;
#pragma unroll
    for (int c = 0; c < kLatCodes; ++c) {
        const uint16_t v = cnt[c][t];
        code_cnt[static_cast<int64_t>(c) * na + I] = v;
        entries += v != 0;
    }
    n_entries[I] = entries;
    n_pairs[I] = pairs;
    if (pairs > 0xffff) *too_long = 1;
}
template <bool MAPS>
__global__ void __launch_bounds__(kBlock) k_lat_codes_fill(SellDev A, const int32_t *__restrict__ pos, LatBricks B, int64_t na,
                                                            const int32_t *__restrict__ mem_ptr, const int32_t *__restrict__ mem_idx,
                                                            const int32_t *__restrict__ pos_c, const int32_t *__restrict__ brick_rank,
                                                            const uint16_t *__restrict__ code_cnt, const int32_t *__restrict__ entry_off,
                                                            const int32_t *__restrict__ pair_off, uint64_t *__restrict__ ukeys,
                                                            int64_t *__restrict__ src_ptr, int32_t *__restrict__ src_slot,
                                                            uint8_t *__restrict__ code_of, uint32_t *__restrict__ code_mask)
{
    __shared__ uint16_t at[kLatCodes][kBlock];
    const int64_t I = static_cast<int64_t>(blockIdx.x) * kBlock + threadIdx.x;
    if (I >= na) return;
    const int t = threadIdx.x;
    const int32_t pc = pos_c[I];
    const int bix = pc & 0x3ff, biy = (pc >> 10) & 0x3ff, biz = (pc >> 20) & 0x3ff;
    const int64_t p0 = pair_off[I];
    int64_t e = entry_off[I];
    int run = 0;
#pragma unroll
    for (int c = 0; c < kLatCodes; ++c) {
        const int v = code_cnt[static_cast<int64_t>(c) * na + I];
        at[c][t] = static_cast<uint16_t>(run);
        if (v != 0) {
            const int bx = bix + c % 3 - 1, by = biy + (c / 3) % 3 - 1, bz = biz + c / 9 - 1;
            const int32_t J = brick_rank[lat_linear(B, bx, by, bz)];
            ukeys[e] = (static_cast<uint64_t>(I) << 32) | static_cast<uint32_t>(J);
            if (MAPS) src_ptr[e] = p0 + run;
            ++e;
        }
        run += v;
    }
    if (MAPS && I == na - 1) src_ptr[e] = p0 + run;
    uint32_t mask = 0;
    for (int32_t m = mem_ptr[I]; m < mem_ptr[I + 1]; ++m) {
        const int64_t i = mem_idx[m];
        const int64_t base = A.slice_off[i >> 6] + (i & 63);
        const int len = A.rowlen[i];
        for (int k = 0; k < len; ++k) {
            const int64_t q = base + 64LL * k;
            const int c = lat_code(B, pos[A.cols[q]], bix, biy, biz);
            if (MAPS) src_slot[p0 + at[c][t]++] = static_cast<int32_t>(q);
            code_of[q] = static_cast<uint8_t>(c);
            mask |= 1u << c;
        }
    }
    code_mask[I] = mask;
}
constexpr int kLatGalThreads = 128;
struct LatGalExtra {
    double *dinv_out, *ratio_out;
    const VdHashEntry *vhash;
    uint16_t *codes;
    VdState *vstate;
};
__device__ __forceinline__ void lat_galerkin_row_out(const double (&acc)[kLatCodes][kLatGalThreads], int t, int64_t I, const uint32_t *__restrict__ code_mask,
                                                     const int64_t *__restrict__ c_slice_off, double *__restrict__ coarse_vals, const LatGalExtra &X)
{
    const int64_t out0 = c_slice_off[I >> 6] + (I & 63);
    double *out = coarse_vals + out0;
    const uint32_t mask = code_mask[I];
    int r = 0;
    double sabs = 0.0;
    bool missed = false;
#pragma unroll
    for (int c = 0; c < kLatCodes; ++c)
        if (mask & (1u << c)) {
            const double v = acc[c][t];
            out[64LL * r] = v;
            sabs += fabs(v);
            if (X.vhash) {
                int code = vd_hash_find(X.vhash, static_cast<unsigned long long>(__double_as_longlong(v)));
                if (code < 0) { missed = true; code = 0; }
                X.codes[out0 + 64LL * r] = static_cast<uint16_t>(code);
            }
            ++r;
        }
    if (X.dinv_out) {
        const double d = (mask & (1u << 13)) ? acc[13][t] : 0.0;
        const bool pos = d > 0.0;
        X.dinv_out[I] = pos ? 1.0 / d : 1.0;
        X.ratio_out[I] = pos ? sabs / d : 1.0;
    }
    if (missed) X.vstate->miss = 1;
}
__global__ void __launch_bounds__(kLatGalThreads) k_lat_galerkin(SellDev A, int64_t na, const int32_t *__restrict__ mem_ptr,
                                                                  const int32_t *__restrict__ mem_idx, const uint8_t *__restrict__ code_of,
                                                                  const uint32_t *__restrict__ code_mask, const int64_t *__restrict__ c_slice_off,
                                                                  double *__restrict__ coarse_vals, LatGalExtra X)
{
    __shared__ double acc[kLatCodes][kLatGalThreads];
    const int64_t I = static_cast<int64_t>(blockIdx.x) * kLatGalThreads + threadIdx.x;
    if (I >= na) return;
    const int t = threadIdx.x;
#pragma unroll
    for (int c = 0; c < kLatCodes; ++c) acc[c][t] = 0.0;
    const int32_t m0 = mem_ptr[I], m1 = mem_ptr[I + 1];
    for (int32_t mb = m0; mb < m1; mb += 8) {
        int32_t mi[8];
        int len[8];
        int64_t base[8];
#pragma unroll
        for (int j = 0; j < 8; ++j) mi[j] = mb + j < m1 ? __builtin_nontemporal_load(mem_idx + mb + j) : -1;
#pragma unroll
        for (int j = 0; j < 8; ++j) {
            len[j] = mi[j] >= 0 ? A.rowlen[mi[j]] : 0;
            base[j] = mi[j] >= 0 ? A.slice_off[mi[j] >> 6] + (mi[j] & 63) : 0;
        }
#pragma unroll
        for (int j = 0; j < 8; ++j) {
            for (int k0 = 0; k0 < len[j]; k0 += 16) {
                double v[16];
                uint8_t c[16];
#pragma unroll
                for (int e = 0; e < 16; ++e) {
                    const bool in = k0 + e < len[j];
                    const int64_t q = base[j] + 64LL * (k0 + e);
                    v[e] = in ? __builtin_nontemporal_load(A.vals + q) : 0.0;
                    c[e] = in ? __builtin_nontemporal_load(code_of + q) : static_cast<uint8_t>(0);
                }
#pragma unroll
                for (int e = 0; e < 16; ++e)
                    if (k0 + e < len[j]) acc[c[e]][t] += v[e];
            }
        }
    }
    lat_galerkin_row_out(acc, t, I, code_mask, c_slice_off, coarse_vals, X);
}
constexpr int kLatGalChunk = 16;
__global__ void __launch_bounds__(kBlock) k_lat_group_codes(SellDev A, const uint8_t *__restrict__ code_of, const uint8_t *__restrict__ relk,
                                                             const int64_t *__restrict__ rslice_off, uint8_t *__restrict__ glat, int *__restrict__ bad)
{
    const int64_t r = static_cast<int64_t>(blockIdx.x) * kBlock + threadIdx.x;
    if (r >= A.n_rows) return;
    const int64_t base = A.slice_off[r >> 6] + (r & 63);
    const int len = A.rowlen[r];
    const int64_t g = r >> 2;
    const int64_t off = rslice_off[g >> 6];
    const int width = static_cast<int>((rslice_off[(g >> 6) + 1] - off) >> 6);
    uint8_t *gp = glat + 4 * (off + (g & 63)) + (r & 3);
    for (int k = 0; k < len; ++k) {
        const int64_t q = base + 64LL * k;
        const int u = relk[q];
        if (u >= width) { *bad = 1; continue; }
        gp[4LL * 64 * u] = code_of[q];
    }
}
__global__ void __launch_bounds__(kLatGalThreads) k_lat_galerkin_codes(int64_t na, const int32_t *__restrict__ mem_ptr, const int32_t *__restrict__ mem_idx,
                                                                        const int64_t *__restrict__ rslice_off, const unsigned long long *__restrict__ vcodes,
                                                                        const uint32_t *__restrict__ glat, const double *__restrict__ dict, int nd,
                                                                        const uint32_t *__restrict__ code_mask, const int64_t *__restrict__ c_slice_off,
                                                                        double *__restrict__ coarse_vals, LatGalExtra X)
{
    __shared__ double acc[kLatCodes][kLatGalThreads];
    extern __shared__ double lat_vd[];
    const int64_t I = static_cast<int64_t>(blockIdx.x) * kLatGalThreads + threadIdx.x;
    const int t = threadIdx.x;
    const bool live = I < na;
    const int32_t m0 = live ? mem_ptr[I] : 0, m1 = live ? mem_ptr[I + 1] : 0;
    for (int i = t; i < nd; i += kLatGalThreads) lat_vd[i] = dict[i];
#pragma unroll
    for (int c = 0; c < kLatCodes; ++c) acc[c][t] = 0.0;
    __syncthreads();
    if (!live) return;
    unsigned long long w[kLatGalChunk];
    uint32_t lc[kLatGalChunk];
    int64_t held = -1;
    for (int32_t mb = m0; mb < m1; mb += 8) {
        int32_t mi[8];
        int width[8];
        int64_t wb[8];
#pragma unroll
        for (int j = 0; j < 8; ++j) mi[j] = mb + j < m1 ? __builtin_nontemporal_load(mem_idx + mb + j) : -1;
#pragma unroll
        for (int j = 0; j < 8; ++j) {
            const int64_t gs = mi[j] >= 0 ? mi[j] >> 8 : 0;
            const int64_t o0 = rslice_off[gs], o1 = rslice_off[gs + 1];
            width[j] = mi[j] >= 0 ? static_cast<int>((o1 - o0) >> 6) : 0;
            wb[j] = o0 + ((mi[j] >> 2) & 63);
        }
#pragma unroll
        for (int j = 0; j < 8; ++j) {
            const int sh16 = 16 * (mi[j] & 3), sh8 = 8 * (mi[j] & 3);
            for (int k0 = 0; k0 < width[j]; k0 += kLatGalChunk) {
                if (wb[j] != held || k0 > 0) {
#pragma unroll
                    for (int e = 0; e < kLatGalChunk; ++e) {
                        const bool in = k0 + e < width[j];
                        const int64_t q = wb[j] + 64LL * (k0 + e);
                        w[e] = in ? __builtin_nontemporal_load(vcodes + q) : 0ull;
                        lc[e] = in ? __builtin_nontemporal_load(glat + q) : ~0u;
                    }
                    held = k0 == 0 ? wb[j] : -1;
                }
#pragma unroll
                for (int e = 0; e < kLatGalChunk; ++e) {
                    const uint32_t c = (lc[e] >> sh8) & 0xffu;
                    if (c < static_cast<uint32_t>(kLatCodes)) acc[c][t] += lat_vd[(w[e] >> sh16) & 0xffffu];
                }
            }
        }
    }
    lat_galerkin_row_out(acc, t, I, code_mask, c_slice_off, coarse_vals, X);
}
constexpr int kLatticeTable = 4096;
__global__ void __launch_bounds__(kBlock) k_amg_distinct(const double *__restrict__ c, int64_t n, unsigned long long *__restrict__ table,
                                                          int *__restrict__ overflow)
{
    const int64_t i = static_cast<int64_t>(blockIdx.x) * kBlock + threadIdx.x;
    const double v = (i < n ? c[i] : 0.0) + 0.0;
    const unsigned long long key = static_cast<unsigned long long>(__double_as_longlong(v));
    const unsigned long long left = __shfl_up(key, 1, 64);
    if (i >= n || ((threadIdx.x & 63) != 0 && left == key && i - 1 < n)) return;
    if (key == ~0ull) { *overflow = 1; return; }
    unsigned h = static_cast<unsigned>((key * 0x9E3779B97F4A7C15ull) >> 52) & (kLatticeTable - 1);
    for (int probe = 0; probe < kLatticeTable; ++probe) {
        if ((probe & 63) == 0 && __hip_atomic_load(overflow, __ATOMIC_RELAXED, __HIP_MEMORY_SCOPE_AGENT) != 0) return;
        const unsigned long long cur = table[h];
        if (cur == key) return;
        if (cur == ~0ull) {
            const unsigned long long old = atomicCAS(&table[h], ~0ull, key);
            if (old == ~0ull || old == key) return;
        }
        h = (h + 1) & (kLatticeTable - 1);
    }
    *overflow = 1;
}

__device__ __forceinline__ unsigned long long amg_sortable(double v)
{
    const unsigned long long b = static_cast<unsigned long long>(__double_as_longlong(v + 0.0));
    return (b >> 63) ? ~b : (b | 0x8000000000000000ull);
}
__device__ __forceinline__ double amg_unsortable(unsigned long long k)
{
    const unsigned long long b = (k >> 63) ? (k & 0x7fffffffffffffffull) : ~k;
    return __longlong_as_double(static_cast<long long>(b));
}
__global__ void __launch_bounds__(kBlock) k_amg_node_xyz(MeshDev m, int64_t n_owned, const int32_t *__restrict__ node_of, int64_t n_nodes,
                                                          double *__restrict__ xyz)
{
    const int64_t t = static_cast<int64_t>(blockIdx.x) * kBlock + threadIdx.x;
    if (t >= m.nElem * m.npe) return;
    const int64_t e = t % m.nElem;
    const int a = static_cast<int>(t / m.nElem);
    const int32_t nd = m.conn[a * m.nElem + e];
    const int32_t l = m.edof[(a * m.ndof) * m.nElem + e];
    if (l < 0 || l >= n_owned) return;
    const int64_t node = node_of ? node_of[l] : l;
    if (node >= n_nodes) return;
    for (int d = 0; d < 3; ++d) xyz[d * n_nodes + node] = d < m.ndim ? m.xyz[static_cast<int64_t>(d) * m.nNode + nd] : 0.0;
}
__global__ void __launch_bounds__(kBlock) k_amg_xyz_min(int64_t nn, const int32_t *__restrict__ node_agg, const double *__restrict__ xyz, int64_t na,
                                                         unsigned long long *__restrict__ keys)
{
    const int64_t i = static_cast<int64_t>(blockIdx.x) * kBlock + threadIdx.x;
    if (i >= nn) return;
    for (int d = 0; d < 3; ++d) atomicMin(&keys[d * na + node_agg[i]], amg_sortable(xyz[d * nn + i]));
}
__global__ void __launch_bounds__(kBlock) k_amg_xyz_decode(int64_t n, const unsigned long long *__restrict__ keys, double *__restrict__ xyz)
{
    const int64_t i = static_cast<int64_t>(blockIdx.x) * kBlock + threadIdx.x;
    if (i < n) xyz[i] = amg_unsortable(keys[i]);
}
__global__ void __launch_bounds__(kBlock) k_amg_emit_global_xyz(int64_t n_nodes_own, const int32_t *__restrict__ gid ,
                                                                 int64_t node_off, const double *__restrict__ xyz, int64_t n_glob,
                                                                 double *__restrict__ out)
{
    const int64_t i = static_cast<int64_t>(blockIdx.x) * kBlock + threadIdx.x;
    if (i >= n_nodes_own) return;
    const int64_t g = gid ? gid[i] : node_off + i;
    for (int d = 0; d < 3; ++d) out[d * n_glob + g] = xyz[d * n_nodes_own + i];
}

__device__ __forceinline__ int amg_lattice_index(const double *__restrict__ u, int n, double v)
{
    int lo = 0, hi = n;
    while (lo < hi) { const int mid = (lo + hi) >> 1; if (u[mid] < v) lo = mid + 1; else hi = mid; }
    return lo < n ? lo : n - 1;
}
__global__ void __launch_bounds__(kBlock) k_amg_lattice_pos(MeshDev m, int64_t n_owned, const double *__restrict__ ux, int nx,
                                                             const double *__restrict__ uy, int ny, const double *__restrict__ uz, int nz,
                                                             int32_t *__restrict__ pos)
{
    const int64_t t = static_cast<int64_t>(blockIdx.x) * kBlock + threadIdx.x;
    if (t >= m.nElem * m.npe) return;
// ... 227 lines not shown
__global__ void __launch_bounds__(kBlock) k_amg_dst_slots(int64_t nnz_c, const uint64_t *__restrict__ ukeys, const int64_t *__restrict__ rowptr,
                                                           const int64_t *__restrict__ slice_off, int64_t *__restrict__ dst)
{
    const int64_t c = static_cast<int64_t>(blockIdx.x) * kBlock + threadIdx.x;
    if (c >= nnz_c) return;
    const int64_t row = static_cast<int64_t>(ukeys[c] >> 32);
    dst[c] = slice_off[row >> 6] + 64LL * (c - rowptr[row]) + (row & 63);
}

__global__ void __launch_bounds__(kBlock) k_amg_galerkin(int64_t nnz_c, const int64_t *__restrict__ src_ptr, const int32_t *__restrict__ src_slot,
                                                          const int64_t *__restrict__ dst, const double *__restrict__ fine_vals,
                                                          double *__restrict__ coarse_vals)
{
    const int64_t c = static_cast<int64_t>(blockIdx.x) * kBlock + threadIdx.x;
    if (c >= nnz_c) return;
    double a = 0.0;
    int64_t q = src_ptr[c];
    const int64_t q1 = src_ptr[c + 1];
    for (; q + 8 <= q1; q += 8) {
        int32_t sl[8];
        double v[8];
#pragma unroll
        for (int k = 0; k < 8; ++k) sl[k] = src_slot[q + k];
#pragma unroll
        for (int k = 0; k < 8; ++k) v[k] = fine_vals[sl[k]];
#pragma unroll
        for (int k = 0; k < 8; ++k) a += v[k];
    }
    if (q < q1) {
        int32_t sl[8];
        double v[8];
#pragma unroll
        for (int k = 0; k < 8; ++k) sl[k] = q + k < q1 ? src_slot[q + k] : -1;
#pragma unroll
        for (int k = 0; k < 8; ++k) v[k] = sl[k] >= 0 ? fine_vals[sl[k]] : 0.0;
#pragma unroll
        for (int k = 0; k < 8; ++k)
            if (sl[k] >= 0) a += v[k];
    }
    coarse_vals[dst[c]] = a;
}

__global__ void __launch_bounds__(kBlock) k_amg_diag_bound(SellDev A, int32_t col_limit, double *__restrict__ dinv, double *__restrict__ part_max)
{
    __shared__ double sm[4];
    const int64_t r = static_cast<int64_t>(blockIdx.x) * kBlock + threadIdx.x;
    double ratio = 0.0;
    if (r < A.n_slices * 64) {
        const int64_t sl = r >> 6;
        const int64_t off = A.slice_off[sl];
        const int width = static_cast<int>((A.slice_off[sl + 1] - off) >> 6);
        double d = 0.0, s = 0.0;
        for (int k = 0; k < width; ++k) {
            const int64_t q = off + 64LL * k + (r & 63);
            const double v = A.vals[q];
            const int32_t c = A.cols[q];
            if (c == static_cast<int32_t>(r) && v != 0.0) d += v;
            if (c < col_limit) s += fabs(v);
        }
        if (r < A.n_rows) {
            const bool ok = d > 0.0;
            dinv[r] = ok ? 1.0 / d : 1.0;
            ratio = ok ? s / d : 1.0;
        }
    }
#pragma unroll
    for (int o = 32; o > 0; o >>= 1) ratio = fmax(ratio, __shfl_xor(ratio, o, 64));
    if ((threadIdx.x & 63) == 0) sm[threadIdx.x >> 6] = ratio;
    __syncthreads();
    if (threadIdx.x == 0) part_max[blockIdx.x] = fmax(fmax(sm[0], sm[1]), fmax(sm[2], sm[3]));
}
__global__ void __launch_bounds__(kBlock) k_amg_max_rows(const double *__restrict__ v, int64_t n, double *__restrict__ part_max)
{
    __shared__ double sm[4];
    double a = 0.0;
    for (int64_t i = static_cast<int64_t>(blockIdx.x) * kBlock + threadIdx.x; i < n; i += static_cast<int64_t>(gridDim.x) * kBlock)
        a = fmax(a, __builtin_nontemporal_load(v + i));
#pragma unroll
    for (int o = 32; o > 0; o >>= 1) a = fmax(a, __shfl_xor(a, o, 64));
    if ((threadIdx.x & 63) == 0) sm[threadIdx.x >> 6] = a;
    __syncthreads();
    if (threadIdx.x == 0) part_max[blockIdx.x] = fmax(fmax(sm[0], sm[1]), fmax(sm[2], sm[3]));
}
__global__ void __launch_bounds__(1024) k_amg_max(const double *__restrict__ part, int64_t n, double *out)
{
    __shared__ double sm[16];
    double a = 0.0;
    for (int64_t i = threadIdx.x; i < n; i += 1024) a = fmax(a, part[i]);
#pragma unroll
    for (int o = 32; o > 0; o >>= 1) a = fmax(a, __shfl_xor(a, o, 64));
    if ((threadIdx.x & 63) == 0) sm[threadIdx.x >> 6] = a;
    __syncthreads();
    if (threadIdx.x == 0) {
        double t = 0.0;
        for (int w = 0; w < 16; ++w) t = fmax(t, sm[w]);
        out[0] = t;
    }
}

constexpr int kAmgDense = 128;
__device__ __forceinline__ void amg_gauss_jordan(double *M, double *colp, int n, double *__restrict__ inv);
__global__ void __launch_bounds__(1024) k_amg_dense_inverse(SellDev A, double *__restrict__ inv)
{
    extern __shared__ double M[];
    __shared__ double colp[kAmgDense];
    const int n = static_cast<int>(A.n_rows);
    for (int q = threadIdx.x; q < n * n; q += 1024) M[q] = 0.0;
    __syncthreads();
    for (int r = threadIdx.x & 63; r < n; r += 64) {
        const int64_t base = A.slice_off[r >> 6] + (r & 63);
        const int len = A.rowlen[r];
        for (int k = threadIdx.x >> 6; k < len; k += 16) M[r * n + A.cols[base + 64LL * k]] = A.vals[base + 64LL * k];
    }
    __syncthreads();
    amg_gauss_jordan(M, colp, n, inv);
}
__global__ void __launch_bounds__(1024) k_amg_dense_inverse_of(const double *__restrict__ dense, int n, double *__restrict__ inv)
{
    extern __shared__ double M[];
    __shared__ double colp[kAmgDense];
    for (int q = threadIdx.x; q < n * n; q += 1024) M[q] = dense[q];
    __syncthreads();
    amg_gauss_jordan(M, colp, n, inv);
}
__device__ __forceinline__ void amg_gauss_jordan(double *M, double *colp, int n, double *__restrict__ inv)
{
    (void)colp;
    constexpr int kPer = (kAmgDense * kAmgDense + 1023) / 1024;
    const int per = (n * n + 1023) / 1024;
    int qi[kPer], qj[kPer];
#pragma unroll
    for (int u = 0; u < kPer; ++u) {
        const int q = threadIdx.x + 1024 * u;
        qi[u] = q < n * n ? q / n : -1;
        qj[u] = q < n * n ? q - qi[u] * n : 0;
    }
    for (int p = 0; p < n; ++p) {
        double nv[kPer];
        const double piv = 1.0 / M[p * n + p];
#pragma unroll
        for (int u = 0; u < kPer; ++u) {
            nv[u] = 0.0;
            if (u < per && qi[u] >= 0) {
                const int i = qi[u], j = qj[u];
                const double cp = M[i * n + p], rp = M[p * n + j] * piv;
                nv[u] = (i == p) ? (j == p ? piv : rp) : (j == p ? -cp * piv : __builtin_fma(-cp, rp, M[i * n + j]));
            }
        }
        __syncthreads();
#pragma unroll
        for (int u = 0; u < kPer; ++u)
            if (u < per && qi[u] >= 0) M[qi[u] * n + qj[u]] = nv[u];
        __syncthreads();
    }
    for (int q = threadIdx.x; q < n * n; q += 1024) inv[q] = M[q];
}
__global__ void __launch_bounds__(kBlock) k_amg_diag_abs(SellDev A, double *__restrict__ diag, double *__restrict__ rowabs)
{
    const int64_t r = static_cast<int64_t>(blockIdx.x) * kBlock + threadIdx.x;
    if (r >= A.n_rows) return;
    const int64_t base = A.slice_off[r >> 6] + (r & 63);
    const int len = A.rowlen[r];
    double d = 0.0, s = 0.0;
    for (int k = 0; k < len; ++k) {
        const double v = A.vals[base + 64LL * k];
        if (A.cols[base + 64LL * k] == static_cast<int32_t>(r)) d += v;
        s += fabs(v);
    }
    diag[r] = d;
    rowabs[r] = s;
}
__global__ void __launch_bounds__(kBlock) k_amg_dinv_ratio(int64_t n, const double *__restrict__ diag, const double *__restrict__ rowabs,
                                                            double *__restrict__ dinv, double *__restrict__ part_max)
{
    __shared__ double sm[4];
    const int64_t r = static_cast<int64_t>(blockIdx.x) * kBlock + threadIdx.x;
    double ratio = 0.0;
    if (r < n) {
        const double d = diag[r];
// ... 399 lines not shown
        int c[4];
        double v[4], xv[4];
#pragma unroll
        for (int j = 0; j < 4; ++j) { c[j] = cp[64 * (k + j)]; v[j] = vp[64 * (k + j)]; }
#pragma unroll
        for (int j = 0; j < 4; ++j) xv[j] = xin[c[j]];
#pragma unroll
        for (int j = 0; j < 4; ++j) acc = __builtin_fma(v[j], xv[j], acc);
    }
    for (; k < width; ++k) acc = __builtin_fma(vp[64 * k], xin[cp[64 * k]], acc);
    const int64_t i = (s << 6) + lane;
    if (i >= A.n_rows) return;
    y[i] = acc;
    share_pack(S, send, i, acc);
}

__global__ void __launch_bounds__(kBlock) k_amg_spmv_pack_vd(SellDev A, const uint16_t *__restrict__ codes, const double *__restrict__ dict, int nd,
                                                              const double *__restrict__ xin, double *__restrict__ y, ShareSum S,
                                                              double *__restrict__ send, const CgCtl *ctl)
{
    extern __shared__ double vd[];
    if (ctl && ctl->flag != 0) return;
    for (int i = threadIdx.x; i < nd; i += kBlock) vd[i] = dict[i];
    __syncthreads();
    const int lane = threadIdx.x & 63, wave = threadIdx.x >> 6;
    const int64_t s = (static_cast<int64_t>(blockIdx.x) << 2) + wave;
    if (s >= A.n_slices) return;
    const int64_t off = A.slice_off[s];
    const int width = static_cast<int>((A.slice_off[s + 1] - off) >> 6);
    const int32_t *__restrict__ cp = A.cols + off + lane;
    const uint16_t *__restrict__ qp = codes + off + lane;
    double acc = 0.0;
    int k = 0;
    for (; k + 4 <= width; k += 4) {
        int c[4];
        uint16_t q[4];
        double xv[4];
#pragma unroll
        for (int j = 0; j < 4; ++j) { c[j] = cp[64 * (k + j)]; q[j] = qp[64 * (k + j)]; }
#pragma unroll
        for (int j = 0; j < 4; ++j) xv[j] = xin[c[j]];
#pragma unroll
        for (int j = 0; j < 4; ++j) acc = __builtin_fma(vd[q[j]], xv[j], acc);
    }
    for (; k < width; ++k) acc = __builtin_fma(vd[qp[64 * k]], xin[cp[64 * k]], acc);
    const int64_t i = (s << 6) + lane;
    if (i >= A.n_rows) return;
    y[i] = acc;
    share_pack(S, send, i, acc);
}

}
#include "pfem_amg_rbm.hpp"
namespace pfem {

constexpr int kAmgTailRows = 1024;
constexpr int64_t kAmgTailNnz = 32768;
constexpr int kAmgTailLevels = 8;
struct AmgTailLevel {
    SellDev A;
    const double *dinv, *lam;
    double *x, *dd, *t, *r, *b;
    const int32_t *agg, *mem_ptr, *mem_idx;
    int64_t n, nc;
    int64_t stored;
    int rbm_dim, fb;
    int64_t nn;
    const int32_t *node_agg;
    const double *roff;
};
struct AmgTail {
    int nlev, deg, coarsest_deg, dense_n;
    const double *dense_inv;
    double ratio, scale;
    AmgTailLevel lev[kAmgTailLevels];
};

struct TailView {
    double *x, *dd, *t, *r, *b;
    const double *dinv;
    const int64_t *slice_off;
    const int32_t *cols;
    const double *vals;
};
__device__ inline TailView tail_view(const AmgTail &T, int l, int use_lds, int64_t mat_slots, double *lds)
{
    const AmgTailLevel &L = T.lev[l];
    TailView V{L.x, L.dd, L.t, L.r, L.b, L.dinv, L.A.slice_off, L.A.cols, L.A.vals};
    if (use_lds) {
        int64_t off = 0, tot = 0;
        for (int q = 0; q < T.nlev; ++q) {
            if (q < l) off += 6 * T.lev[q].n;
            tot += 6 * T.lev[q].n;
        }
        double *base = lds + off;
        const int64_t n = L.n;
        V.x = base; V.dd = base + n; V.t = base + 2 * n; V.r = base + 3 * n; V.b = base + 4 * n; V.dinv = base + 5 * n;
        if (l == 0 && mat_slots > 0) {
            double *mv = lds + tot;
            int64_t *so = reinterpret_cast<int64_t *>(mv + mat_slots);
            V.vals = mv;
            V.slice_off = so;
            V.cols = reinterpret_cast<int32_t *>(so + L.A.n_slices + 1);
        }
    }
    return V;
}
__device__ inline void tail_spmv(const TailView &V, int64_t n_rows, const double *x, double *y)
{
    for (int64_t i = threadIdx.x; i < n_rows; i += 1024) {
        const int64_t off = V.slice_off[i >> 6];
        const int width = static_cast<int>((V.slice_off[(i >> 6) + 1] - off) >> 6);
        const int32_t *cp = V.cols + off + (i & 63);
        const double *vp = V.vals + off + (i & 63);
        double acc = 0.0;
        int k = 0;
        for (; k + 8 <= width; k += 8) {
            int c[8];
            double v[8], xv[8];
#pragma unroll
            for (int j = 0; j < 8; ++j) { c[j] = cp[64 * (k + j)]; v[j] = vp[64 * (k + j)]; }
#pragma unroll
            for (int j = 0; j < 8; ++j) xv[j] = x[c[j]];
#pragma unroll
            for (int j = 0; j < 8; ++j) acc = __builtin_fma(v[j], xv[j], acc);
        }
        for (; k < width; ++k) acc = __builtin_fma(vp[64 * k], x[cp[64 * k]], acc);
        y[i] = acc;
    }
    __syncthreads();
}
__device__ inline void tail_smooth(const AmgTailLevel &L, const TailView &V, const double *b, bool zero_guess, int deg, double ratio, double lmax)
{
    if (!zero_guess) tail_spmv(V, L.n, V.x, V.t);
    const ChebCoef c0 = cheb_coef(lmax, ratio, 0);
    for (int64_t i = threadIdx.x; i < L.n; i += 1024) {
        const double ri = zero_guess ? b[i] : b[i] - V.t[i];
        const double di = c0.c_first * V.dinv[i] * ri;
        if (deg > 1 && !zero_guess) V.r[i] = ri;
        if (deg > 1) V.dd[i] = di;
        V.x[i] = zero_guess ? di : V.x[i] + di;
    }
    __syncthreads();
    const double *r_in = zero_guess ? b : V.r;
    for (int k = 1; k < deg; ++k) {
        tail_spmv(V, L.n, V.dd, V.t);
        const ChebCoef c = cheb_coef(lmax, ratio, k);
        const bool more = k + 1 < deg;
        for (int64_t i = threadIdx.x; i < L.n; i += 1024) {
            const double ri = r_in[i] - V.t[i];
            const double di = __builtin_fma(c.c_dd, V.dd[i], c.c_r * V.dinv[i] * ri);
            if (more) { V.r[i] = ri; V.dd[i] = di; }
            V.x[i] += di;
        }
        __syncthreads();
        r_in = V.r;
    }
}
__device__ inline void tail_rbm_restrict(const AmgTailLevel &L, const TailView &V, const AmgTailLevel &C, const TailView &VC)
{
    const int64_t nc_nodes = C.n / L.fb;
    for (int64_t a = threadIdx.x; a < nc_nodes; a += 1024) {
        double out[6];
        if (L.rbm_dim == 3) rbm_restrict_node<6, 3>(a, L.mem_ptr, L.mem_idx, L.roff, L.nn, V.b, V.t, L.nn, out);
        else rbm_restrict_node<3, 2>(a, L.mem_ptr, L.mem_idx, L.roff, L.nn, V.b, V.t, L.nn, out);
        for (int k = 0; k < L.fb; ++k) VC.b[L.fb * a + k] = out[k];
    }
}
__device__ inline void tail_rbm_prolong(const AmgTailLevel &L, const TailView &V, const TailView &VC, double scale)
{
    for (int64_t i = threadIdx.x; i < L.nn; i += 1024) {
        if (L.rbm_dim == 3) rbm_prolong_node<6, 3>(i, L.node_agg, L.roff, L.nn, VC.x, scale, V.x);
        else rbm_prolong_node<3, 2>(i, L.node_agg, L.roff, L.nn, VC.x, scale, V.x);
    }
}
__global__ void __launch_bounds__(1024) k_amg_tail(const AmgTail T, const CgCtl *ctl, int use_lds, int64_t mat_slots)
{
    extern __shared__ double tail_lds[];
    if (ctl && ctl->flag != 0) return;
    const int nl = T.nlev;
    __shared__ double lam_of[kAmgTailLevels];
    if (threadIdx.x < static_cast<unsigned>(nl)) lam_of[threadIdx.x] = T.lev[threadIdx.x].lam[0];
    if (!use_lds) __syncthreads();
    if (use_lds) {
        if (mat_slots > 0) {
            const AmgTailLevel &L = T.lev[0];
            const TailView V = tail_view(T, 0, use_lds, mat_slots, tail_lds);
            double *mv = const_cast<double *>(V.vals);
            int32_t *mc = const_cast<int32_t *>(V.cols);
            int64_t *so = const_cast<int64_t *>(V.slice_off);
            const double *__restrict__ gv = L.A.vals;
            const int32_t *__restrict__ gc = L.A.cols;
            for (int64_t q0 = threadIdx.x; q0 < mat_slots; q0 += 8 * 1024) {
                double v[8];
                int32_t c[8];
#pragma unroll
                for (int j = 0; j < 8; ++j) {
                    const int64_t q = q0 + 1024 * j;
                    v[j] = q < mat_slots ? __builtin_nontemporal_load(gv + q) : 0.0;
                    c[j] = q < mat_slots ? __builtin_nontemporal_load(gc + q) : 0;
                }
#pragma unroll
                for (int j = 0; j < 8; ++j) {
                    const int64_t q = q0 + 1024 * j;
                    if (q < mat_slots) { mv[q] = v[j]; mc[q] = c[j]; }
                }
            }
            for (int64_t q = threadIdx.x; q <= L.A.n_slices; q += 1024) so[q] = L.A.slice_off[q];
        }
        for (int l = 0; l < nl; ++l) {
            const AmgTailLevel &L = T.lev[l];
            const TailView V = tail_view(T, l, use_lds, mat_slots, tail_lds);
            double *dv = const_cast<double *>(V.dinv);
            for (int64_t i = threadIdx.x; i < L.n; i += 1024) {
                dv[i] = L.dinv[i];
                if (l == 0) V.b[i] = L.b[i];
            }
        }
        __syncthreads();
    }
    for (int l = 0; l < nl; ++l) {
        const AmgTailLevel &L = T.lev[l];
        const TailView V = tail_view(T, l, use_lds, mat_slots, tail_lds);
        if (l == nl - 1) {
            if (T.dense_n > 0) {
                const int n = T.dense_n;
                for (int i = threadIdx.x; i < n; i += 1024) {
                    double a = 0.0;
                    for (int j = 0; j < n; ++j) a = __builtin_fma(T.dense_inv[j * n + i], V.b[j], a);
                    V.x[i] = a;
                }
                __syncthreads();
            } else {
                tail_smooth(L, V, V.b, true, T.coarsest_deg, T.ratio, lam_of[l]);
            }
            break;
        }
        const AmgTailLevel &C = T.lev[l + 1];
        const TailView VC = tail_view(T, l + 1, use_lds, mat_slots, tail_lds);
        tail_smooth(L, V, V.b, true, T.deg, T.ratio, lam_of[l]);
        tail_spmv(V, L.n, V.x, V.t);
        if (L.rbm_dim) tail_rbm_restrict(L, V, C, VC);
        else
        for (int64_t a = threadIdx.x; a < C.n; a += 1024) {
            double acc = 0.0;
            for (int q = L.mem_ptr[a]; q < L.mem_ptr[a + 1]; ++q) {
                const int i = L.mem_idx[q];
                acc += V.b[i] - V.t[i];
            }
            VC.b[a] = acc;
        }
        __syncthreads();
    }
    for (int l = nl - 2; l >= 0; --l) {
        const AmgTailLevel &L = T.lev[l];
        const TailView V = tail_view(T, l, use_lds, mat_slots, tail_lds);
        const TailView VC = tail_view(T, l + 1, use_lds, mat_slots, tail_lds);
        if (L.rbm_dim) tail_rbm_prolong(L, V, VC, T.scale);
        else
        for (int64_t i = threadIdx.x; i < L.n; i += 1024) V.x[i] = __builtin_fma(T.scale, VC.x[L.agg[i]], V.x[i]);
        __syncthreads();
        tail_smooth(L, V, V.b, false, T.deg, T.ratio, lam_of[l]);
    }
    if (use_lds) {
        const TailView V = tail_view(T, 0, use_lds, mat_slots, tail_lds);
        double *x_out = T.lev[0].x;
        for (int64_t i = threadIdx.x; i < T.lev[0].n; i += 1024) x_out[i] = V.x[i];
    }
}

__global__ void __launch_bounds__(kBlock) k_pc_init(int64_t n, const double *__restrict__ b, double *__restrict__ x, double *__restrict__ r)
{
    for (int64_t i = static_cast<int64_t>(blockIdx.x) * kBlock + threadIdx.x; i < n; i += static_cast<int64_t>(gridDim.x) * kBlock) {
        x[i] = 0.0;
        r[i] = b[i];
    }
}
__global__ void __launch_bounds__(kBlock) k_pc_copy(int64_t n, const double *__restrict__ z, double *__restrict__ p)
{
    for (int64_t i = static_cast<int64_t>(blockIdx.x) * kBlock + threadIdx.x; i < n; i += static_cast<int64_t>(gridDim.x) * kBlock) p[i] = z[i];
}
__global__ void __launch_bounds__(kBlock) k_pc_update(CgCtl *ctl, int it, int64_t n, const double *part_pw, int nparts, const double *reduced_pw,
                                                       const double *__restrict__ w, double *__restrict__ r, int64_t n_pc,
                                                       const double *__restrict__ dinv, const double *__restrict__ lam, double ratio,
                                                       double *__restrict__ z0, double *__restrict__ dd0)
{
    __shared__ double sm[4];
    if (ctl->flag != 0) return;
    const double pw = reduced_pw ? *reduced_pw : sum_partials(part_pw, nparts, sm);
    if (!(pw > 0.0)) {
        if (blockIdx.x == 0 && threadIdx.x == 0) { ctl->its = it; ctl->pad_ = 1; }
        return;
    }
    const double alpha = ctl->beta[it & 1] / pw;
    if (blockIdx.x == 0 && threadIdx.x == 0) ctl->alpha = alpha;
    const double c_first = z0 ? cheb_coef(lam[0], ratio, 0).c_first : 0.0;
    for (int64_t i = static_cast<int64_t>(blockIdx.x) * kBlock + threadIdx.x; i < n; i += static_cast<int64_t>(gridDim.x) * kBlock) {
        const double ri = __builtin_fma(-alpha, w[i], r[i]);
        r[i] = ri;
        if (z0 && i < n_pc) {
            const double di = c_first * dinv[i] * ri;
            if (dd0) dd0[i] = di;
            z0[i] = di;
        }
    }
}
__global__ void __launch_bounds__(kBlock) k_pc_post_dots(const CgCtl *ctl, int64_t n, int64_t n_owned, const double *__restrict__ r,
                                                          const double *__restrict__ t, const double *__restrict__ dinv,
                                                          const double *__restrict__ lam, double ratio, double *__restrict__ z, double *part_rz,
                                                          double *part_zz)
{
    __shared__ double sm[4];
    if (ctl && ctl->flag != 0) return;
    if (ctl && ctl->pad_ != 0) {
        if (threadIdx.x == 0) { part_rz[blockIdx.x] = 0.0; part_zz[blockIdx.x] = -1.0; }
        return;
    }
    const double c_first = cheb_coef(lam[0], ratio, 0).c_first;
    double rz = 0.0, zz = 0.0;
    for (int64_t i = static_cast<int64_t>(blockIdx.x) * kBlock + threadIdx.x; i < n; i += static_cast<int64_t>(gridDim.x) * kBlock) {
        if (i < n_owned) {
            const double ri = r[i];
            const double zi = z[i] + c_first * dinv[i] * (ri - t[i]);
            z[i] = zi;
            rz = __builtin_fma(ri, zi, rz);
            zz = __builtin_fma(zi, zi, zz);
        }
    }
    const double a = block_sum(rz, sm), c = block_sum(zz, sm);
    if (threadIdx.x == 0) { part_rz[blockIdx.x] = a; part_zz[blockIdx.x] = c; }
}

__global__ void __launch_bounds__(kBlock) k_pcg1_step(CgCtl *ctl, int it, int64_t n, const double *reduced ,
                                                       const double *part_zs, int n_zs, const double *part_rz, const double *part_zz, int nparts,
                                                       const double *__restrict__ z, const double *__restrict__ sv, double *__restrict__ p,
                                                       double *__restrict__ w, double *__restrict__ x, double *__restrict__ r, double rtol,
                                                       double abstol, double dtol, double *hist, int hist_cap, int maxits)
{
    __shared__ double sm[4];
    if (ctl->flag != 0) return;
    double zs, rz, zz;
    if (reduced) { zs = reduced[0]; rz = reduced[1]; zz = reduced[2]; }
    else { zs = sum_partials(part_zs, n_zs, sm); rz = sum_partials(part_rz, nparts, sm); zz = sum_partials(part_zz, nparts, sm); }
    const bool lead = blockIdx.x == 0 && threadIdx.x == 0;
    const double rn = sqrt(zz);
    int flag = 0;
    if (it == 0 && rn <= abstol) flag = 3;
    else if (it > 0 && rn <= ctl->ttol) flag = 2;
// ... 128 lines not shown
```

### pfemfort_amd/csrc/pfem_amg_types.hpp

```cpp
#pragma once

struct AmgPlan {
    std::vector<int> peers;
    std::vector<int64_t> peer_off{0};
    std::vector<int32_t> send_lidx;
    int64_t n_send = 0, n_sh = 0;
    DevBuf<int32_t> d_send_lidx, d_sh_lidx, d_sh_ptr, d_sh_src;
    DevBuf<int32_t> d_row_sh;
};

struct AmgLevel {
    int64_t n = 0, n_slices = 0, stored = 0, nnz = 0;
    int64_t n_loc = 0;
    int64_t gid_off = 0;
    std::vector<int64_t> ghost_gid;
    AmgPlan plan;
    DevBuf<int32_t> gid;
    bool fine = false;
    DevBuf<int64_t> slice_off, rowptr;
    DevBuf<int32_t> rowlen, cols;
    DevBuf<double> vals;
    int bs = 1;
    int64_t n_nodes = 0;
    DevBuf<int32_t> node_of, comp_of;
    DevBuf<int32_t> hint;
    bool lattice = false;
    int lat_hi[3] = {0, 0, 0};
    int lat_axis = 0;
    bool lat_global = false;
    std::vector<int> lat_cuts[3];
    std::vector<char> lat_single[3];
    int lat_shift[3] = {0, 0, 0};
    int lat_occ[6] = {0, 0, 0, 0, 0, 0};
    int lat_box[6] = {0, 0, 0, 0, 0, 0};
    bool lat_full = false;
    int lat_tlo[3] = {0, 0, 0}, lat_thi[3] = {0, 0, 0};
    bool lat_nodes_global = false;
    std::vector<std::pair<int, int>> lat_str[3];
    bool lat_split = false;
    std::vector<double> lat_coord;
    DevBuf<double> xyz;
    int agg_kind = 0;
    int64_t nc = 0;
    DevBuf<int32_t> agg;
    DevBuf<int32_t> mem_ptr, mem_idx;
    int64_t nnz_c = 0;
    DevBuf<int64_t> src_ptr;
    DevBuf<int32_t> src_slot;
    DevBuf<int64_t> dst_slot;
    DevBuf<uint8_t> code_of;
    DevBuf<uint32_t> code_mask;
    DevBuf<uint32_t> glat;
    int64_t glat_for = -1;
    bool glat_refused = false;
    int dim = 0;
    bool rbm = false;
    DevBuf<double> cen;
    DevBuf<double> roff;
    DevBuf<int32_t> node_agg;
    DevBuf<int64_t> gptr;
    DevBuf<int32_t> gcol, brow;
    int64_t nblk = 0;
    DevBuf<double> dinv, t, r, b, x_store, dd_store, lam, part_max;
    DevBuf<uint16_t> vcodes;
    DevBuf<double> vdict;
    DevBuf<unsigned long long> vtable;
    int vd_n = 0;
    bool vd_ok = false, vd_have_dict = false, vd_refused = false;
    DevBuf<VdHashEntry> vhash;
    bool vd_hash_ok = false;
    bool vd_direct = false;
    bool bound_fresh = false;
    double *x = nullptr, *dd = nullptr;
    DevBuf<double> x1;
    double lam_host = 0.0;
};

struct Amg {
    std::vector<std::unique_ptr<AmgLevel>> lev;
    DevBuf<double> dense_inv;
    bool dense = false;
    bool symbolic_ok = false;
    bool galerkin_fresh = false;
    double symbolic_ms = 0.0, numeric_ms = 0.0;
    int cheb_degree = 2;
    int fine_degree = 1;
    bool eig_ratio_given = false;
    bool coarse_scale_given = false;
    double eig_ratio_opt = 0.0, coarse_scale_opt = 0.0;
    double eig_ratio_auto = 16.0, coarse_scale_auto = 1.5;
    double eig_ratio = 8.0, coarse_scale = 1.5;
    CgGraph graph;
    hipEvent_t ev_num0 = nullptr, ev_num1 = nullptr;
    ~Amg()
    {
        if (ev_num0) (void)hipEventDestroy(ev_num0);
        if (ev_num1) (void)hipEventDestroy(ev_num1);
    }
    int tail_from = -1;
    size_t tail_lds_allowed = 0;
    int cycle_gamma = 1, w_to = -1;
    bool cycle_given = false;
    bool fused = true;
    bool level0_ep = false;
    bool galerkin_from_codes = false;
    int coarsest_sweeps = 8;
    bool coupled = false;
    bool coupled_fused = true;
    bool coupled_refused = false;
    int64_t n_last_global = 0;
    DevBuf<double> dense_glob, bx_glob, lam_all;
    std::unique_ptr<Amg> rep;
    DevBuf<double> rep_buf;
    DevBuf<int32_t> rep_pack_slot;
    int64_t rep_total = 0, rep_off = 0, rep_mine = 0;
    bool rbm = false;
    DevBuf<double> lam2;
    DevBuf<VdState> vd_states;
    int cycle_exchanges = 0, cycle_allreduces = 0;
};
```

### pfemfort_amd/csrc/pfem_device.hip

```cpp
#include <hip/hip_runtime.h>
#include <hip/hip_ext.h>
#include <hipcub/hipcub.hpp>
#include <rccl/rccl.h>
#include <dlfcn.h>

#include <algorithm>
#include <chrono>
#include <climits>
#include <cmath>
#include <cstdio>
#include <cstdlib>
#include <cstring>
#include <mutex>
#include <thread>
#include <string>
#include <deque>
#include <functional>
#include <map>
#include <memory>
#include <vector>

#include "pfem_internal.hpp"
#include "pfem_vdhash.hpp"
#include "pfem_kernels.hpp"
// ... 4673 lines not shown
    s->xprof.clear();
    (void)hipEventDestroy(c0);
    (void)hipEventDestroy(c1);
    PFEM_TRY(rc);
    return s->comm->health();
}

extern "C" int pfem_solver_set_amg_options(pfem_solver *s, int cheb_degree, int fine_degree, double eig_ratio, double coarse_scale)
{
    if (!s || cheb_degree < 1 || cheb_degree > 6 || fine_degree < 0 || fine_degree > 6 || (eig_ratio > 0.0 && !(eig_ratio > 1.0))) return PFEM_ERR_ARG;
    if (!s->amg) s->amg.reset(new (std::nothrow) Amg());
    if (!s->amg) return PFEM_ERR_NOMEM;
    s->amg->cheb_degree = cheb_degree;
    s->amg->fine_degree = fine_degree;
    s->amg->graph.invalidate();
    s->amg->eig_ratio_given = eig_ratio > 0.0;
    if (eig_ratio > 0.0) s->amg->eig_ratio_opt = eig_ratio;
    s->amg->coarse_scale_given = coarse_scale > 0.0;
    if (coarse_scale > 0.0) s->amg->coarse_scale_opt = coarse_scale;
    return PFEM_OK;
}

extern "C" int pfem_solver_amg_value_dictionaries(pfem_solver *s, int max_levels, int *n_levels, int *entries)
{
    if (!s || !n_levels || !entries || max_levels < 1) return PFEM_ERR_ARG;
    *n_levels = 0;
    if (!s->amg || !s->amg->symbolic_ok) return PFEM_OK;
    for (const AmgLevelRef &r : amg_levels_of(*s->amg)) {
        if (*n_levels >= max_levels) break;
        entries[(*n_levels)++] = r.L->fine ? ((s->vd_ok && s->vd_current) ? s->vd_n : 0) : (r.L->vd_ok ? r.L->vd_n : 0);
    }
    return PFEM_OK;
}

extern "C" int pfem_solver_set_amg_cycle(pfem_solver *s, int cycle)
{
    if (!s || cycle < 0 || cycle > 2) return PFEM_ERR_ARG;
    if (!s->amg) s->amg.reset(new (std::nothrow) Amg());
    if (!s->amg) return PFEM_ERR_NOMEM;
    s->amg->cycle_given = cycle != 0;
    if (cycle != 0) s->amg->cycle_gamma = cycle;
    s->amg->graph.invalidate();
    return PFEM_OK;
}
extern "C" int pfem_solver_amg_level0_epilogue(pfem_solver *s, int *taken)
{
    if (!s || !taken) return PFEM_ERR_ARG;
    if (!s->amg || !s->amg->symbolic_ok) return PFEM_ERR_STATE;
    *taken = s->amg->level0_ep ? 1 : 0;
    return PFEM_OK;
}

extern "C" int pfem_solver_amg_galerkin_from_codes(pfem_solver *s, int *taken)
{
    if (!s || !taken) return PFEM_ERR_ARG;
    *taken = (s->amg && s->amg->symbolic_ok && s->amg->galerkin_from_codes) ? 1 : 0;
    return PFEM_OK;
}
extern "C" int pfem_solver_amg_level_values(pfem_solver *s, int level, int64_t max_values, double *vals, int64_t *stored)
{
    if (!s || !stored || level < 1 || max_values < 0 || (max_values > 0 && !vals)) return PFEM_ERR_ARG;
    if (!s->amg || !s->amg->symbolic_ok) return PFEM_ERR_STATE;
    const std::vector<AmgLevelRef> lev = amg_levels_of(*s->amg);
    if (static_cast<size_t>(level) >= lev.size()) return PFEM_ERR_STATE;
    const AmgLevel &L = *lev[static_cast<size_t>(level)].L;
    *stored = L.stored;
    const int64_t n = std::min<int64_t>(max_values, L.stored);
    if (n < 1 || !L.vals.p) return PFEM_OK;
    PFEM_TRY(use_device(s));
    PFEM_HIP(hipStreamSynchronize(s->stream));
    PFEM_HIP(hipMemcpy(vals, L.vals.p, sizeof(double) * static_cast<size_t>(n), hipMemcpyDeviceToHost));
    return PFEM_OK;
}

extern "C" int pfem_solver_amg_cycle(pfem_solver *s, int *cycle, int *last_level_visited_twice)
{
    if (!s || !cycle || !last_level_visited_twice) return PFEM_ERR_ARG;
    if (!s->amg || !s->amg->symbolic_ok) return PFEM_ERR_STATE;
    const Amg &M = *s->amg;
    *cycle = M.cycle_gamma;
    *last_level_visited_twice = M.cycle_gamma > 1 ? std::min(M.w_to, static_cast<int>(M.lev.size()) - 2) : 0;
    return PFEM_OK;
}
```

### pfemfort_amd/solver.py

```python
from __future__ import annotations

import ctypes as C

import numpy as np

from . import _lib as L
from ._lib import (ADD_VALUES, ASSEMBLY_OK, FACTORISE_OK, INIT_OK, INSERT_VALUES,
                   PATTERN_OK, SOLVER_EMPTY)


def _p(a):
    return None if a is None else a.ctypes.data_as(C.c_void_p)


def _f64(a):
    return np.ascontiguousarray(a, dtype=np.float64)


def _i32(a):
    return np.ascontiguousarray(a, dtype=np.int32)


class PetscSolver:

# ... 109 lines not shown
        self.kind = kind
        self.nElem = conn.shape[1]
        self.nNode = xyz.shape[1]

    def generateBoxMesh(self, kind, x0, x1, nEx, y0, y1, nEy, z0, z1, nEz, bc_mode=0, nparts=1, part=0, axis=2):
        L.check(L.lib().pfem_mesh_generate_box_axis(self._h, kind, x0, x1, nEx, y0, y1, nEy, z0, z1, nEz, bc_mode, axis, nparts, part),
                "pfem_mesh_generate_box_axis")
        self.kind = kind
        sz = L.lib().pfem_box_slab_sizes_axis
        n = C.c_int64(0); ne = C.c_int64(0)
        L.check(sz(nEx, nEy, nEz, bc_mode, L.NDOF[kind], axis, nparts, part, None, None, None, C.byref(n), C.byref(ne), None, None, None),
                "pfem_box_slab_sizes_axis")
        self.nElem, self.nNode = ne.value, n.value

    def downloadMesh(self):
        npe, ndof, ndim = L.NPELEM[self.kind], L.NDOF[self.kind], L.NDIM[self.kind]
        conn = np.empty((npe, self.nElem), np.int32); xyz = np.empty((ndim, self.nNode))
        edof = np.empty((npe * ndof, self.nElem), np.int32); sa = np.empty(self.nNode * ndof)
        L.check(L.lib().pfem_mesh_download(self._h, _p(conn), _p(xyz), _p(edof), _p(sa)), "pfem_mesh_download")
        return conn, xyz, edof, sa

    def buildPattern(self):
        L.check(L.lib().pfem_pattern_build(self._h), "pfem_pattern_build")

    def setAssemblyMode(self, mode):
        L.check(L.lib().pfem_solver_set_assembly_mode(self._h, {"gather": 0, "scatter": 1}[mode]),
                "pfem_solver_set_assembly_mode")

    def assemblyInfo(self):
        g = C.c_int(0); h = C.c_int(0); t = C.c_int(0); b = C.c_int64(0)
        L.check(L.lib().pfem_solver_assembly_info(self._h, C.byref(g), C.byref(h), C.byref(t), C.byref(b)), "pfem_solver_assembly_info")
        return {"gather": bool(g.value), "hub_nodes": h.value, "block_threads": t.value, "lds_bytes": b.value}

    def setSpmvFormat(self, fmt):
        L.check(L.lib().pfem_solver_set_spmv_format(self._h, {"auto": 0, "int32": 1, "gaps16": 2, "grouped": 3}[fmt]), "pfem_solver_set_spmv_format")

    def spmvColumnBits(self):
        b = C.c_int(0)
        L.check(L.lib().pfem_solver_get_spmv_format(self._h, C.byref(b)), "pfem_solver_get_spmv_format")
        return b.value

    def spmvGapTable(self):
        b = C.c_int(0)
        L.check(L.lib().pfem_solver_get_spmv_gap_table(self._h, C.byref(b)), "pfem_solver_get_spmv_gap_table")
        return b.value

    def spmvValueDictionary(self):
        b = C.c_int(0)
        L.check(L.lib().pfem_solver_get_spmv_value_dictionary(self._h, C.byref(b)), "pfem_solver_get_spmv_value_dictionary")
        return b.value

    def amgValueDictionaries(self):
        n = C.c_int(0)
        e = (C.c_int * 32)()
        L.check(L.lib().pfem_solver_amg_value_dictionaries(self._h, 32, C.byref(n), e), "pfem_solver_amg_value_dictionaries")
        return list(e[:n.value])

    def spmvGapEscapes(self):
        b = C.c_int(0)
        L.check(L.lib().pfem_solver_get_spmv_gap_escapes(self._h, C.byref(b)), "pfem_solver_get_spmv_gap_escapes")
        return bool(b.value)

    def setPreconditioner(self, pc):
        L.check(L.lib().pfem_solver_set_preconditioner(self._h, {"jacobi": 0, "pbjacobi": 1, "gamg": 2}[pc]), "pfem_solver_set_preconditioner")

    def setSingleReduction(self, on=True):
        L.check(L.lib().pfem_solver_set_cg_single_reduction(self._h, -1 if on is None else int(bool(on))),
                "pfem_solver_set_cg_single_reduction")

    def preconditioner(self):
        b = C.c_int(0)
        L.check(L.lib().pfem_solver_get_preconditioner(self._h, C.byref(b)), "pfem_solver_get_preconditioner")
        return ("jacobi", "pbjacobi", "gamg")[b.value]

    def setAmgOptions(self, cheb_degree=2, fine_degree=1, eig_ratio=None, coarse_scale=None):
        L.check(L.lib().pfem_solver_set_amg_options(self._h, cheb_degree, fine_degree, -1.0 if eig_ratio is None else eig_ratio,
                                                    -1.0 if coarse_scale is None else coarse_scale), "pfem_solver_set_amg_options")

    def setAmgCycle(self, cycle=None):
        code = {None: 0, "auto": 0, "v": 1, "w": 2}[cycle.lower() if isinstance(cycle, str) else cycle]
        L.check(L.lib().pfem_solver_set_amg_cycle(self._h, code), "pfem_solver_set_amg_cycle")

    def amgCycle(self):
        c, w, e = C.c_int(0), C.c_int(0), C.c_int(0)
        L.check(L.lib().pfem_solver_amg_cycle(self._h, C.byref(c), C.byref(w)), "pfem_solver_amg_cycle")
        L.check(L.lib().pfem_solver_amg_level0_epilogue(self._h, C.byref(e)), "pfem_solver_amg_level0_epilogue")
        return {"cycle": "w" if c.value == 2 else "v", "last_level_visited_twice": w.value, "level0_epilogue": bool(e.value)}

    def amgTransfer(self, level, xyz=False):
        rbm, fb, cb, dim = C.c_int(0), C.c_int(0), C.c_int(0), C.c_int(0)
        nn = C.c_int64(0)
        L.check(L.lib().pfem_solver_amg_transfer(self._h, level, C.byref(rbm), C.byref(fb), C.byref(cb), C.byref(dim), C.byref(nn), None), "pfem_solver_amg_transfer")
        out = {"rbm": bool(rbm.value), "fine_bs": fb.value, "coarse_bs": cb.value, "dim": dim.value, "n_nodes": nn.value}
        if xyz:
            a = np.empty((3, nn.value), np.float64)
            L.check(L.lib().pfem_solver_amg_transfer(self._h, level, C.byref(rbm), C.byref(fb), C.byref(cb), C.byref(dim), C.byref(nn), _p(a)), "pfem_solver_amg_transfer")
            out["xyz"] = a
        return out

    def incidencePatterns(self):
        n = C.c_int(0); m = C.c_int(0)
        L.check(L.lib().pfem_solver_incidence_patterns(self._h, C.byref(n), C.byref(m)), "pfem_solver_incidence_patterns")
        return n.value, m.value

    def amgAggregation(self):
        mx = 32
        nl = C.c_int(0)
        kind = (C.c_int * mx)()
        L.check(L.lib().pfem_solver_amg_aggregation(self._h, mx, C.byref(nl), kind), "pfem_solver_amg_aggregation")
        names = {0: "none", 1: "bricks", 2: "node-bricks", 3: "split-bricks", 4: "lattice-passes", 5: "matching"}
        return [names.get(kind[l], str(kind[l])) for l in range(max(nl.value - 1, 0))]

    def amgInfo(self):
        mx = 32
        nl = C.c_int(0); rows = (C.c_int64 * mx)(); nnz = (C.c_int64 * mx)(); lam = (C.c_double * mx)()
        sym = C.c_double(0); num = C.c_double(0); deg = C.c_int(0); fdeg = C.c_int(0); ratio = C.c_double(0); scale = C.c_double(0)
        L.check(L.lib().pfem_solver_amg_info(self._h, mx, C.byref(nl), rows, nnz, lam, C.byref(sym), C.byref(num), C.byref(deg),
                                             C.byref(fdeg), C.byref(ratio), C.byref(scale)), "pfem_solver_amg_info")
        n = nl.value
        gc = C.c_int(0)
        L.check(L.lib().pfem_solver_amg_galerkin_from_codes(self._h, C.byref(gc)), "pfem_solver_amg_galerkin_from_codes")
        return {"levels": n, "rows": list(rows[:n]), "nnz": list(nnz[:n]), "lambda_max": list(lam[:n]), "symbolic_ms": sym.value,
                "numeric_ms": num.value, "cheb_degree": deg.value, "fine_degree": fdeg.value, "eig_ratio": ratio.value, "coarse_scale": scale.value,
                "galerkin_from_codes": bool(gc.value)}

    def amgLevelValues(self, level):
        n = C.c_int64(0)
        L.check(L.lib().pfem_solver_amg_level_values(self._h, level, 0, None, C.byref(n)), "pfem_solver_amg_level_values")
        a = np.empty(n.value, np.float64)
        L.check(L.lib().pfem_solver_amg_level_values(self._h, level, n.value, _p(a), C.byref(n)), "pfem_solver_amg_level_values")
        return a

    def amgAggregates(self, level, n_rows):
        a = np.empty(n_rows, np.int32)
        L.check(L.lib().pfem_solver_amg_aggregates(self._h, level, _p(a)), "pfem_solver_amg_aggregates")
        return a

    def amgLayout(self):
        mx = 32
        cp, nd = C.c_int(0), C.c_int(0)
        first = np.zeros(mx, np.int64)
        loc = np.zeros(mx, np.int64)
        L.check(L.lib().pfem_solver_amg_layout(self._h, mx, C.byref(cp), C.byref(nd), _p(first), _p(loc)), "pfem_solver_amg_layout")
        nl = self.amgInfo()["levels"]
        ex, ar = C.c_int(0), C.c_int(0)
        L.check(L.lib().pfem_solver_amg_comm_counts(self._h, C.byref(ex), C.byref(ar)), "pfem_solver_amg_comm_counts")
        lat = C.c_int(0)
        L.check(L.lib().pfem_solver_amg_pairing(self._h, C.byref(lat)), "pfem_solver_amg_pairing")
        return {"coupled": bool(cp.value), "distributed_levels": nd.value, "first_dof": first[:nl].tolist(), "local_rows": loc[:nl].tolist(),
                "exchanges_per_cycle": ex.value, "allreduces_per_cycle": ar.value, "lattice_levels": lat.value}

    def amgCycleProfile(self):
        mx = 32
        nl, na = C.c_int(0), C.c_int(0)
        ex = np.zeros(mx, np.int32); ms = np.zeros(mx, np.float64); dbl = np.zeros(mx, np.int64)
        ams, adbl, cyc = C.c_double(0), C.c_int64(0), C.c_double(0)
        L.check(L.lib().pfem_solver_amg_cycle_profile(self._h, mx, C.byref(nl), _p(ex), _p(ms), _p(dbl), C.byref(na), C.byref(ams), C.byref(adbl),
                                                      C.byref(cyc)), "pfem_solver_amg_cycle_profile")
        n = nl.value
        return {"cycle_ms": cyc.value, "exchanges_per_level": ex[:n].tolist(), "exchange_ms_per_level": ms[:n].tolist(),
                "exchange_bytes_per_level": (8 * dbl[:n]).tolist(), "allreduces": na.value, "allreduce_ms": ams.value, "allreduce_bytes": 8 * adbl.value}

    def spmvRowGroup(self):
        b = C.c_int(0)
        L.check(L.lib().pfem_solver_get_spmv_row_group(self._h, C.byref(b)), "pfem_solver_get_spmv_row_group")
        return b.value

    def spmvFormatBytes(self):
        b = C.c_int64(0)
        L.check(L.lib().pfem_solver_spmv_bytes(self._h, C.byref(b)), "pfem_solver_spmv_bytes")
# ... 118 lines not shown
```

Measured before the change: 632.5 million.

## Fuse Chebyshev bound reduction into Galerkin kernel and template AMG tail LDS modes

The lattice Galerkin kernel now reduces each coarse level's eigenvalue bound as a by-product through a block-level max, and zeroes the next level's bound. This removes the separate k_amg_max launches on non-RBM fused hierarchies. The AMG tail kernel is templated on LDS and matrix-in-LDS modes, also stages the aggregation index arrays in LDS, and can raise the dynamic LDS limit for vector-only use. It also unrolls the dense coarse solve and prefetches the dense inverse. The cost is more code paths and an atomic-style bound reduction that depends on correct zero-initialisation ordering.

```diff
diff --git a/include/pfem_amd_diag.h b/include/pfem_amd_diag.h
--- a/include/pfem_amd_diag.h
+++ b/include/pfem_amd_diag.h
@@ -38,6 +38,7 @@
 int pfem_solver_amg_pairing(pfem_solver *s, int *lattice_levels);
 int pfem_solver_amg_cycle(pfem_solver *s, int *cycle, int *last_level_visited_twice);
 int pfem_solver_amg_level0_epilogue(pfem_solver *s, int *taken);
+int pfem_solver_amg_tail_from(pfem_solver *s, int *tail_from, int *tail_build, int *bounds_by_products);
 int pfem_solver_amg_galerkin_from_codes(pfem_solver *s, int *taken);
 int pfem_solver_amg_level_values(pfem_solver *s, int level, int64_t max_values, double *vals, int64_t *stored);
 
diff --git a/pfemfort_amd/_lib.py b/pfemfort_amd/_lib.py
--- a/pfemfort_amd/_lib.py
+++ b/pfemfort_amd/_lib.py
@@ -114,6 +114,7 @@
     "pfem_solver_set_amg_cycle": [_P, _I],
     "pfem_solver_amg_cycle": [_P, _P, _P],
     "pfem_solver_amg_level0_epilogue": [_P, _P],
+    "pfem_solver_amg_tail_from": [_P, _P, _P, _P],
     "pfem_solver_amg_galerkin_from_codes": [_P, _P],
     "pfem_solver_amg_level_values": [_P, _I, _L, _P, _P],
     "pfem_eval_elems": [_P, _P, _P, _P, _P],
diff --git a/pfemfort_amd/csrc/pfem_amg.inc b/pfemfort_amd/csrc/pfem_amg.inc
--- a/pfemfort_amd/csrc/pfem_amg.inc
+++ b/pfemfort_amd/csrc/pfem_amg.inc
@@ -573,17 +573,18 @@
     static const bool v = std::getenv("PFEM_AMG_GALERKIN_MAPS") != nullptr;
     return v;
 }
-inline void amg_galerkin(pfem_solver *s, const AmgLevel &L, AmgLevel &C, const SellDev &A, bool extras = false, VdState *vstate = nullptr,
-                         bool from_codes = false)
-{
-    C.bound_fresh = C.vd_direct = false;
+inline bool amg_galerkin(pfem_solver *s, const AmgLevel &L, AmgLevel &C, const SellDev &A, bool extras = false, VdState *vstate = nullptr,
+                         bool from_codes = false, double *bound = nullptr, double *zero = nullptr)
+{
+    C.bound_fresh = C.vd_direct = C.bound_done = false;
     if (L.code_of.p && !amg_galerkin_by_entry()) {
-        if (C.n_loc < 1) return;
-        LatGalExtra X{nullptr, nullptr, nullptr, nullptr, nullptr};
+        if (C.n_loc < 1) return false;
+        LatGalExtra X{nullptr, nullptr, nullptr, nullptr, nullptr, nullptr, nullptr};
         if (extras && C.dinv.p && C.t.p && C.n_loc == C.n) {
             X.dinv_out = C.dinv.p;
             X.ratio_out = C.t.p;
             C.bound_fresh = true;
+            if (bound) { X.bound = bound; X.zero = zero; C.bound_done = true; }
             if (vstate && C.vd_have_dict && C.vd_hash_ok && C.vhash.p && C.vcodes.p && C.vcodes.n >= static_cast<size_t>(C.stored) && !C.vd_refused) {
                 const VdState reset{C.vd_n, 0, 0, 0};
                 (void)hipMemcpyAsync(vstate, &reset, sizeof reset, hipMemcpyHostToDevice, s->stream);
@@ -600,16 +601,17 @@
                                static_cast<const unsigned long long *>(s->d_vcodes.p), static_cast<const uint32_t *>(L.glat.p),
                                static_cast<const double *>(s->d_vdict.p), s->vd_n, static_cast<const uint32_t *>(L.code_mask.p),
                                static_cast<const int64_t *>(C.slice_off.p), C.vals.p, X);
-            return;
+            return C.bound_done;
         }
         hipLaunchKernelGGL(k_lat_galerkin, dim3(static_cast<unsigned>((C.n_loc + kLatGalThreads - 1) / kLatGalThreads)), dim3(kLatGalThreads), 0, s->stream, A, C.n_loc,
                            static_cast<const int32_t *>(L.mem_ptr.p), static_cast<const int32_t *>(L.mem_idx.p), static_cast<const uint8_t *>(L.code_of.p),
                            static_cast<const uint32_t *>(L.code_mask.p), static_cast<const int64_t *>(C.slice_off.p), C.vals.p, X);
-        return;
+        return C.bound_done;
     }
     hipLaunchKernelGGL(k_amg_galerkin, dim3(grid_for(L.nnz_c)), dim3(kBlock), 0, s->stream, L.nnz_c, static_cast<const int64_t *>(L.src_ptr.p),
                        static_cast<const int32_t *>(L.src_slot.p), static_cast<const int64_t *>(L.dst_slot.p),
                        static_cast<const double *>(A.vals), C.vals.p);
+    return false;
 }
 
 int amg_couple_level(pfem_solver *s, AmgWork &W, AmgLevel &L, AmgLevel &C, bool overlap, int cb, const std::vector<double> *nc_of)
@@ -2228,6 +2230,31 @@
     return PFEM_OK;
 }
 
+void amg_tail_shape(const Amg &M, int tail, AmgTail &T)
+{
+    T.nlev = static_cast<int>(M.lev.size()) - tail;
+    for (int q = 0; q < T.nlev; ++q) {
+        const AmgLevel &L = *M.lev[static_cast<size_t>(tail + q)];
+        T.lev[q].n = L.n;
+        T.lev[q].rbm_dim = L.rbm ? L.dim : 0;
+        T.lev[q].stored = L.stored;
+        T.lev[q].A.n_slices = (L.n + 63) / 64;
+    }
+}
+struct TailLds { size_t vecs_b, vec_b, mat_b; };
+TailLds tail_lds_bytes(const AmgTail &T)
+{
+    int64_t rows = 0, ints = 0;
+    for (int q = 0; q < T.nlev; ++q) { rows += T.lev[q].n; ints += tail_idx_ints(T, q); }
+    TailLds W;
+    W.vecs_b = static_cast<size_t>(6 * rows) * sizeof(double);
+    W.vec_b = static_cast<size_t>(6 * rows + ((ints + 1) >> 1)) * sizeof(double);
+    const AmgTailLevel &t0 = T.lev[0];
+    W.mat_b = (T.nlev > 1 && t0.stored > 0) ? static_cast<size_t>(t0.stored) * 12 + static_cast<size_t>(t0.A.n_slices + 2) * 8 : 0;
+    return W;
+}
+constexpr size_t kAmgTailLdsMax = 156 * 1024;
+
 int amg_finish_levels(pfem_solver *s, Amg &M, bool coupled)
 {
     for (auto &L : M.lev) PFEM_TRY(amg_alloc_vectors(s, *L));
@@ -2253,18 +2280,20 @@
     for (size_t l = 1; l < M.lev.size() && !coupled; ++l)
         if (M.lev[l]->n <= kAmgTailRows && M.lev[l]->nnz <= kAmgTailNnz && M.lev.size() - l <= static_cast<size_t>(kAmgTailLevels)) { M.tail_from = static_cast<int>(l); break; }
     M.w_to = M.tail_from > 0 ? M.tail_from : static_cast<int>(M.lev.size()) - 2;
-    M.tail_lds_allowed = 0;
+    M.tail_lds_allowed = M.tail_vec_allowed = 0;
+    M.tail_build = 0;
     if (M.tail_from > 0) {
-        int64_t rows = 0;
-        for (size_t l = static_cast<size_t>(M.tail_from); l < M.lev.size(); ++l) rows += M.lev[l]->n;
-        const AmgLevel &T0 = *M.lev[static_cast<size_t>(M.tail_from)];
-        const size_t need = static_cast<size_t>(6 * rows) * sizeof(double) + static_cast<size_t>(T0.stored) * 12 + static_cast<size_t>((T0.n + 63) / 64 + 2) * 8;
-        if (need > 65536 && need <= 156 * 1024) {
-            if (hipFuncSetAttribute(reinterpret_cast<const void *>(k_amg_tail), hipFuncAttributeMaxDynamicSharedMemorySize, static_cast<int>(need)) == hipSuccess)
-                M.tail_lds_allowed = need;
-            else
-                (void)hipGetLastError();
-        }
+        AmgTail T{};
+        amg_tail_shape(M, M.tail_from, T);
+        const TailLds W = tail_lds_bytes(T);
+        const size_t need = W.vec_b + W.mat_b;
+        auto allow = [](const void *k) {
+            if (hipFuncSetAttribute(k, hipFuncAttributeMaxDynamicSharedMemorySize, static_cast<int>(kAmgTailLdsMax)) == hipSuccess) return kAmgTailLdsMax;
+            (void)hipGetLastError();
+            return static_cast<size_t>(0);
+        };
+        if (W.vecs_b <= 65536 && W.mat_b > 0 && need > 65536 && need <= kAmgTailLdsMax) M.tail_lds_allowed = allow(reinterpret_cast<const void *>(k_amg_tail<true, true>));
+        if (W.vecs_b <= 65536 && W.vec_b > 65536) M.tail_vec_allowed = allow(reinterpret_cast<const void *>(k_amg_tail<true, false>));
     }
     return PFEM_OK;
 }
@@ -2669,49 +2698,67 @@
     if (M.coupled) return amg_numeric_coupled(s, M, overlap);
     const bool fresh = M.galerkin_fresh;
     M.galerkin_fresh = false;
+    const bool own_bounds = M.fused && !M.rbm && !fresh && M.lev.size() > 1;
+    size_t zeroed = 0;
+    M.bounds_by_products = 0;
+    auto level_bound = [&](size_t l, double *zero) -> int {
+        AmgLevel &L = *M.lev[l];
+        const SellDev A = amg_sell(s, L);
+        const unsigned g = grid_for(A.n_slices * 64);
+        if (!L.fine && L.bound_fresh && !fresh) {
+            L.bound_fresh = false;
+            if (L.bound_done) { ++M.bounds_by_products; return PFEM_OK; }
+            if (L.n > 65536) {
+                const unsigned gm = std::min<unsigned>(g, 512u);
+                hipLaunchKernelGGL(k_amg_max_rows, dim3(gm), dim3(kBlock), 0, s->stream, static_cast<const double *>(L.t.p), L.n, L.part_max.p);
+                hipLaunchKernelGGL(k_amg_max, dim3(1), dim3(1024), 0, s->stream, static_cast<const double *>(L.part_max.p), static_cast<int64_t>(gm), L.lam.p, zero);
+            } else {
+                hipLaunchKernelGGL(k_amg_max, dim3(1), dim3(1024), 0, s->stream, static_cast<const double *>(L.t.p), L.n, L.lam.p, zero);
+            }
+            return PFEM_OK;
+        }
+        if (L.fine && s->asm_bound_fresh && &M == s->amg.get()) {
+            const unsigned gm = std::min<unsigned>(g, 2048u);
+            hipLaunchKernelGGL(k_amg_max_rows, dim3(gm), dim3(kBlock), 0, s->stream, static_cast<const double *>(L.t.p), L.n, L.part_max.p);
+            hipLaunchKernelGGL(k_amg_max, dim3(1), dim3(1024), 0, s->stream, static_cast<const double *>(L.part_max.p), static_cast<int64_t>(gm), L.lam.p, zero);
+            s->asm_bound_fresh = false;
+        } else {
+            hipLaunchKernelGGL(k_amg_diag_bound, dim3(g), dim3(kBlock), 0, s->stream, A, static_cast<int32_t>(L.n), L.dinv.p, L.part_max.p);
+            hipLaunchKernelGGL(k_amg_max, dim3(1), dim3(1024), 0, s->stream, static_cast<const double *>(L.part_max.p), static_cast<int64_t>(g), L.lam.p, zero);
+        }
+        if (M.rbm) {
+            if (!M.lam2.p) PFEM_TRY(M.lam2.alloc(1));
+            hipLaunchKernelGGL(k_rbm_bound_sym, dim3(g), dim3(kBlock), 0, s->stream, A, static_cast<int32_t>(L.n), static_cast<const double *>(L.dinv.p),
+                               static_cast<double *>(nullptr), L.part_max.p);
+            hipLaunchKernelGGL(k_amg_max, dim3(1), dim3(1024), 0, s->stream, static_cast<const double *>(L.part_max.p), static_cast<int64_t>(g), M.lam2.p);
+            hipLaunchKernelGGL(k_rbm_min2, dim3(1), dim3(64), 0, s->stream, static_cast<const double *>(M.lam2.p), L.lam.p);
+        }
+        return PFEM_OK;
+    };
     for (size_t l = 0; l < M.lev.size(); ++l) {
         AmgLevel &L = *M.lev[l];
         const SellDev A = amg_sell(s, L);
+        const bool bound_first = own_bounds && l == 0;
+        if (bound_first) {
+            PFEM_TRY(level_bound(0, M.lev[1]->lam.p));
+            zeroed = 1;
+        }
         if (l + 1 < M.lev.size() && !fresh) {
             AmgLevel &C = *M.lev[l + 1];
             if (L.rbm) amg_rbm_galerkin(s, L, C, A);
             else {
                 bool from_codes = false;
                 if (l == 0) PFEM_TRY(amg_level0_codes(s, M, L, &from_codes));
-                amg_galerkin(s, L, C, A, !M.rbm && !M.coupled, M.vd_states.p ? M.vd_states.p + (l + 1) : nullptr, from_codes);
+                const bool mine = own_bounds && zeroed == l + 1;
+                double *next = mine && l + 2 < M.lev.size() ? M.lev[l + 2]->lam.p : nullptr;
+                if (amg_galerkin(s, L, C, A, !M.rbm && !M.coupled, M.vd_states.p ? M.vd_states.p + (l + 1) : nullptr, from_codes, mine ? C.lam.p : nullptr, next) && next)
+                    zeroed = l + 2;
                 if (from_codes) M.galerkin_from_codes = true;
                 if (l == 0 && std::getenv("PFEM_VD_VERBOSE"))
                     std::fprintf(stderr, "  gamg numeric: level 1 summed from %s\n", from_codes ? "the SpMV's value codes" : "the fp64 row form");
             }
         }
-        const unsigned g = grid_for(A.n_slices * 64);
-        if (!L.fine && L.bound_fresh && !fresh) {
-            L.bound_fresh = false;
-            if (L.n > 65536) {
-                const unsigned gm = std::min<unsigned>(g, 512u);
-                hipLaunchKernelGGL(k_amg_max_rows, dim3(gm), dim3(kBlock), 0, s->stream, static_cast<const double *>(L.t.p), L.n, L.part_max.p);
-                hipLaunchKernelGGL(k_amg_max, dim3(1), dim3(1024), 0, s->stream, static_cast<const double *>(L.part_max.p), static_cast<int64_t>(gm), L.lam.p);
-            } else {
-                hipLaunchKernelGGL(k_amg_max, dim3(1), dim3(1024), 0, s->stream, static_cast<const double *>(L.t.p), L.n, L.lam.p);
-            }
-            continue;
-        }
-        if (L.fine && s->asm_bound_fresh && &M == s->amg.get()) {
-            const unsigned gm = std::min<unsigned>(g, 2048u);
-            hipLaunchKernelGGL(k_amg_max_rows, dim3(gm), dim3(kBlock), 0, s->stream, static_cast<const double *>(L.t.p), L.n, L.part_max.p);
-            hipLaunchKernelGGL(k_amg_max, dim3(1), dim3(1024), 0, s->stream, static_cast<const double *>(L.part_max.p), static_cast<int64_t>(gm), L.lam.p);
-            s->asm_bound_fresh = false;
-        } else {
-        hipLaunchKernelGGL(k_amg_diag_bound, dim3(g), dim3(kBlock), 0, s->stream, A, static_cast<int32_t>(L.n), L.dinv.p, L.part_max.p);
-        hipLaunchKernelGGL(k_amg_max, dim3(1), dim3(1024), 0, s->stream, static_cast<const double *>(L.part_max.p), static_cast<int64_t>(g), L.lam.p);
-        }
-        if (M.rbm) {
-            if (!M.lam2.p) PFEM_TRY(M.lam2.alloc(1));
-            hipLaunchKernelGGL(k_rbm_bound_sym, dim3(g), dim3(kBlock), 0, s->stream, A, static_cast<int32_t>(L.n), static_cast<const double *>(L.dinv.p),
-                               static_cast<double *>(nullptr), L.part_max.p);
-            hipLaunchKernelGGL(k_amg_max, dim3(1), dim3(1024), 0, s->stream, static_cast<const double *>(L.part_max.p), static_cast<int64_t>(g), M.lam2.p);
-            hipLaunchKernelGGL(k_rbm_min2, dim3(1), dim3(64), 0, s->stream, static_cast<const double *>(M.lam2.p), L.lam.p);
-        }
+        if (!bound_first) PFEM_TRY(level_bound(l, nullptr));
     }
     PFEM_TRY(check_kernel("gamg numeric"));
     if (M.dense) {
@@ -2924,6 +2971,7 @@
         T.dense_inv = M.dense_inv.p;
         T.ratio = M.eig_ratio;
         T.scale = M.coarse_scale;
+        amg_tail_shape(M, tail, T);
         for (int q = 0; q < T.nlev; ++q) {
             AmgLevel &L = *M.lev[static_cast<size_t>(tail + q)];
             AmgTailLevel &t = T.lev[q];
@@ -2934,17 +2982,15 @@
             t.n = L.n; t.nc = L.nc; t.stored = L.stored;
             t.rbm_dim = L.rbm ? L.dim : 0; t.fb = L.bs; t.nn = L.n_nodes; t.node_agg = L.node_agg.p; t.roff = L.roff.p;
         }
-        int64_t rows = 0;
-        for (int q = 0; q < T.nlev; ++q) rows += T.lev[q].n;
-        const size_t vec_b = static_cast<size_t>(6 * rows) * sizeof(double);
-        const bool use_lds = vec_b <= 65536;
-        const AmgTailLevel &t0 = T.lev[0];
-        const size_t mat_b = (T.nlev > 1 && t0.stored > 0) ? static_cast<size_t>(t0.stored) * 12 + static_cast<size_t>(t0.A.n_slices + 2) * 8 : 0;
-        const bool mat = use_lds && mat_b > 0 && vec_b + mat_b <= 156 * 1024;
-        const size_t lds = use_lds ? vec_b + (mat ? mat_b : 0) : 0;
-        const bool mat_ok = mat && (lds <= 65536 || lds <= M.tail_lds_allowed);
-        hipLaunchKernelGGL(k_amg_tail, dim3(1), dim3(1024), use_lds ? (mat_ok ? lds : vec_b) : 0, s->stream, T, ctl, use_lds ? 1 : 0,
-                           mat_ok ? t0.stored : static_cast<int64_t>(0));
+        const TailLds W = tail_lds_bytes(T);
+        const size_t lds = W.vec_b + W.mat_b;
+        const bool use_lds = W.vecs_b <= 65536 && (W.vec_b <= 65536 || W.vec_b <= M.tail_vec_allowed || lds <= M.tail_lds_allowed);
+        const bool mat_ok = use_lds && W.mat_b > 0 && lds <= kAmgTailLdsMax && (lds <= 65536 || lds <= M.tail_lds_allowed);
+        const bool vec_ok = use_lds && (W.vec_b <= 65536 || W.vec_b <= M.tail_vec_allowed);
+        M.tail_build = mat_ok ? 3 : vec_ok ? 2 : 1;
+        if (mat_ok) hipLaunchKernelGGL((k_amg_tail<true, true>), dim3(1), dim3(1024), lds, s->stream, T, ctl, T.lev[0].stored);
+        else if (vec_ok) hipLaunchKernelGGL((k_amg_tail<true, false>), dim3(1), dim3(1024), W.vec_b, s->stream, T, ctl, static_cast<int64_t>(0));
+        else hipLaunchKernelGGL((k_amg_tail<false, false>), dim3(1), dim3(1024), 0, s->stream, T, ctl, static_cast<int64_t>(0));
     };
     std::function<void(int)> visit = [&](int l) {
         AmgLevel &L = *M.lev[static_cast<size_t>(l)];
@@ -3051,7 +3097,7 @@
         }
         PFEM_TRY(rc);
         s->asm_bound_fresh = false;
-        for (auto &L : s->amg->lev) L->bound_fresh = L->vd_direct = false;
+        for (auto &L : s->amg->lev) L->bound_fresh = L->bound_done = L->vd_direct = false;
     }
     Amg &M = *s->amg;
     amg_knobs(M);
diff --git a/pfemfort_amd/csrc/pfem_amg_kernels.hpp b/pfemfort_amd/csrc/pfem_amg_kernels.hpp
--- a/pfemfort_amd/csrc/pfem_amg_kernels.hpp
+++ b/pfemfort_amd/csrc/pfem_amg_kernels.hpp
@@ -451,8 +451,23 @@
     const VdHashEntry *vhash;
     uint16_t *codes;
     VdState *vstate;
+    double *bound, *zero;
 };
-__device__ __forceinline__ void lat_galerkin_row_out(const double (&acc)[kLatCodes][kLatGalThreads], int t, int64_t I, const uint32_t *__restrict__ code_mask,
+__device__ __forceinline__ void lat_bound_out(double ratio, const LatGalExtra &X)
+{
+    if (!X.bound) return;
+    __shared__ double wmax[kLatGalThreads / 64];
+#pragma unroll
+    for (int o = 32; o > 0; o >>= 1) ratio = fmax(ratio, __shfl_xor(ratio, o, 64));
+    if ((threadIdx.x & 63) == 0) wmax[threadIdx.x >> 6] = ratio;
+    __syncthreads();
+    if (threadIdx.x == 0) {
+        double m = wmax[0];
+        for (int w = 1; w < kLatGalThreads / 64; ++w) m = fmax(m, wmax[w]);
+        atomicMax(reinterpret_cast<unsigned long long *>(X.bound), static_cast<unsigned long long>(__double_as_longlong(m)));
+    }
+}
+__device__ __forceinline__ double lat_galerkin_row_out(const double (&acc)[kLatCodes][kLatGalThreads], int t, int64_t I, const uint32_t *__restrict__ code_mask,
                                                      const int64_t *__restrict__ c_slice_off, double *__restrict__ coarse_vals, const LatGalExtra &X)
 {
     const int64_t out0 = c_slice_off[I >> 6] + (I & 63);
@@ -474,13 +489,16 @@
             }
             ++r;
         }
+    double ratio = 0.0;
     if (X.dinv_out) {
         const double d = (mask & (1u << 13)) ? acc[13][t] : 0.0;
         const bool pos = d > 0.0;
         X.dinv_out[I] = pos ? 1.0 / d : 1.0;
-        X.ratio_out[I] = pos ? sabs / d : 1.0;
+        ratio = pos ? sabs / d : 1.0;
+        X.ratio_out[I] = ratio;
     }
     if (missed) X.vstate->miss = 1;
+    return ratio;
 }
 __global__ void __launch_bounds__(kLatGalThreads) k_lat_galerkin(SellDev A, int64_t na, const int32_t *__restrict__ mem_ptr,
                                                                   const int32_t *__restrict__ mem_idx, const uint8_t *__restrict__ code_of,
@@ -489,41 +507,45 @@
 {
     __shared__ double acc[kLatCodes][kLatGalThreads];
     const int64_t I = static_cast<int64_t>(blockIdx.x) * kLatGalThreads + threadIdx.x;
-    if (I >= na) return;
     const int t = threadIdx.x;
-#pragma unroll
-    for (int c = 0; c < kLatCodes; ++c) acc[c][t] = 0.0;
-    const int32_t m0 = mem_ptr[I], m1 = mem_ptr[I + 1];
-    for (int32_t mb = m0; mb < m1; mb += 8) {
-        int32_t mi[8];
-        int len[8];
-        int64_t base[8];
-#pragma unroll
-        for (int j = 0; j < 8; ++j) mi[j] = mb + j < m1 ? __builtin_nontemporal_load(mem_idx + mb + j) : -1;
-#pragma unroll
-        for (int j = 0; j < 8; ++j) {
-            len[j] = mi[j] >= 0 ? A.rowlen[mi[j]] : 0;
-            base[j] = mi[j] >= 0 ? A.slice_off[mi[j] >> 6] + (mi[j] & 63) : 0;
-        }
-#pragma unroll
-        for (int j = 0; j < 8; ++j) {
-            for (int k0 = 0; k0 < len[j]; k0 += 16) {
-                double v[16];
-                uint8_t c[16];
-#pragma unroll
-                for (int e = 0; e < 16; ++e) {
-                    const bool in = k0 + e < len[j];
-                    const int64_t q = base[j] + 64LL * (k0 + e);
-                    v[e] = in ? __builtin_nontemporal_load(A.vals + q) : 0.0;
-                    c[e] = in ? __builtin_nontemporal_load(code_of + q) : static_cast<uint8_t>(0);
+    if (X.zero && I == 0) X.zero[0] = 0.0;
+    double ratio = 0.0;
+    if (I < na) {
+#pragma unroll
+        for (int c = 0; c < kLatCodes; ++c) acc[c][t] = 0.0;
+        const int32_t m0 = mem_ptr[I], m1 = mem_ptr[I + 1];
+        for (int32_t mb = m0; mb < m1; mb += 8) {
+            int32_t mi[8];
+            int len[8];
+            int64_t base[8];
+#pragma unroll
+            for (int j = 0; j < 8; ++j) mi[j] = mb + j < m1 ? __builtin_nontemporal_load(mem_idx + mb + j) : -1;
+#pragma unroll
+            for (int j = 0; j < 8; ++j) {
+                len[j] = mi[j] >= 0 ? A.rowlen[mi[j]] : 0;
+                base[j] = mi[j] >= 0 ? A.slice_off[mi[j] >> 6] + (mi[j] & 63) : 0;
+            }
+#pragma unroll
+            for (int j = 0; j < 8; ++j) {
+                for (int k0 = 0; k0 < len[j]; k0 += 16) {
+                    double v[16];
+                    uint8_t c[16];
+#pragma unroll
+                    for (int e = 0; e < 16; ++e) {
+                        const bool in = k0 + e < len[j];
+                        const int64_t q = base[j] + 64LL * (k0 + e);
+                        v[e] = in ? __builtin_nontemporal_load(A.vals + q) : 0.0;
+                        c[e] = in ? __builtin_nontemporal_load(code_of + q) : static_cast<uint8_t>(0);
+                    }
+#pragma unroll
+                    for (int e = 0; e < 16; ++e)
+                        if (k0 + e < len[j]) acc[c[e]][t] += v[e];
                 }
-#pragma unroll
-                for (int e = 0; e < 16; ++e)
-                    if (k0 + e < len[j]) acc[c[e]][t] += v[e];
             }
         }
-    }
-    lat_galerkin_row_out(acc, t, I, code_mask, c_slice_off, coarse_vals, X);
+        ratio = lat_galerkin_row_out(acc, t, I, code_mask, c_slice_off, coarse_vals, X);
+    }
+    lat_bound_out(ratio, X);
 }
 constexpr int kLatGalChunk = 16;
 __global__ void __launch_bounds__(kBlock) k_lat_group_codes(SellDev A, const uint8_t *__restrict__ code_of, const uint8_t *__restrict__ relk,
@@ -560,46 +582,50 @@
 #pragma unroll
     for (int c = 0; c < kLatCodes; ++c) acc[c][t] = 0.0;
     __syncthreads();
-    if (!live) return;
-    unsigned long long w[kLatGalChunk];
-    uint32_t lc[kLatGalChunk];
-    int64_t held = -1;
-    for (int32_t mb = m0; mb < m1; mb += 8) {
-        int32_t mi[8];
-        int width[8];
-        int64_t wb[8];
-#pragma unroll
-        for (int j = 0; j < 8; ++j) mi[j] = mb + j < m1 ? __builtin_nontemporal_load(mem_idx + mb + j) : -1;
-#pragma unroll
-        for (int j = 0; j < 8; ++j) {
-            const int64_t gs = mi[j] >= 0 ? mi[j] >> 8 : 0;
-            const int64_t o0 = rslice_off[gs], o1 = rslice_off[gs + 1];
-            width[j] = mi[j] >= 0 ? static_cast<int>((o1 - o0) >> 6) : 0;
-            wb[j] = o0 + ((mi[j] >> 2) & 63);
-        }
-#pragma unroll
-        for (int j = 0; j < 8; ++j) {
-            const int sh16 = 16 * (mi[j] & 3), sh8 = 8 * (mi[j] & 3);
-            for (int k0 = 0; k0 < width[j]; k0 += kLatGalChunk) {
-                if (wb[j] != held || k0 > 0) {
+    if (X.zero && I == 0) X.zero[0] = 0.0;
+    double ratio = 0.0;
+    if (live) {
+        unsigned long long w[kLatGalChunk];
+        uint32_t lc[kLatGalChunk];
+        int64_t held = -1;
+        for (int32_t mb = m0; mb < m1; mb += 8) {
+            int32_t mi[8];
+            int width[8];
+            int64_t wb[8];
+#pragma unroll
+            for (int j = 0; j < 8; ++j) mi[j] = mb + j < m1 ? __builtin_nontemporal_load(mem_idx + mb + j) : -1;
+#pragma unroll
+            for (int j = 0; j < 8; ++j) {
+                const int64_t gs = mi[j] >= 0 ? mi[j] >> 8 : 0;
+                const int64_t o0 = rslice_off[gs], o1 = rslice_off[gs + 1];
+                width[j] = mi[j] >= 0 ? static_cast<int>((o1 - o0) >> 6) : 0;
+                wb[j] = o0 + ((mi[j] >> 2) & 63);
+            }
+#pragma unroll
+            for (int j = 0; j < 8; ++j) {
+                const int sh16 = 16 * (mi[j] & 3), sh8 = 8 * (mi[j] & 3);
+                for (int k0 = 0; k0 < width[j]; k0 += kLatGalChunk) {
+                    if (wb[j] != held || k0 > 0) {
+#pragma unroll
+                        for (int e = 0; e < kLatGalChunk; ++e) {
+                            const bool in = k0 + e < width[j];
+                            const int64_t q = wb[j] + 64LL * (k0 + e);
+                            w[e] = in ? __builtin_nontemporal_load(vcodes + q) : 0ull;
+                            lc[e] = in ? __builtin_nontemporal_load(glat + q) : ~0u;
+                        }
+                        held = k0 == 0 ? wb[j] : -1;
+                    }
 #pragma unroll
                     for (int e = 0; e < kLatGalChunk; ++e) {
-                        const bool in = k0 + e < width[j];
-                        const int64_t q = wb[j] + 64LL * (k0 + e);
-                        w[e] = in ? __builtin_nontemporal_load(vcodes + q) : 0ull;
-                        lc[e] = in ? __builtin_nontemporal_load(glat + q) : ~0u;
+                        const uint32_t c = (lc[e] >> sh8) & 0xffu;
+                        if (c < static_cast<uint32_t>(kLatCodes)) acc[c][t] += lat_vd[(w[e] >> sh16) & 0xffffu];
                     }
-                    held = k0 == 0 ? wb[j] : -1;
-                }
-#pragma unroll
-                for (int e = 0; e < kLatGalChunk; ++e) {
-                    const uint32_t c = (lc[e] >> sh8) & 0xffu;
-                    if (c < static_cast<uint32_t>(kLatCodes)) acc[c][t] += lat_vd[(w[e] >> sh16) & 0xffffu];
                 }
             }
         }
-    }
-    lat_galerkin_row_out(acc, t, I, code_mask, c_slice_off, coarse_vals, X);
+        ratio = lat_galerkin_row_out(acc, t, I, code_mask, c_slice_off, coarse_vals, X);
+    }
+    lat_bound_out(ratio, X);
 }
 constexpr int kLatticeTable = 4096;
 __global__ void __launch_bounds__(kBlock) k_amg_distinct(const double *__restrict__ c, int64_t n, unsigned long long *__restrict__ table,
@@ -993,7 +1019,7 @@
     __syncthreads();
     if (threadIdx.x == 0) part_max[blockIdx.x] = fmax(fmax(sm[0], sm[1]), fmax(sm[2], sm[3]));
 }
-__global__ void __launch_bounds__(1024) k_amg_max(const double *__restrict__ part, int64_t n, double *out)
+__global__ void __launch_bounds__(1024) k_amg_max(const double *__restrict__ part, int64_t n, double *out, double *zero = nullptr)
 {
     __shared__ double sm[16];
     double a = 0.0;
@@ -1006,6 +1032,7 @@
         double t = 0.0;
         for (int w = 0; w < 16; ++w) t = fmax(t, sm[w]);
         out[0] = t;
+        if (zero) zero[0] = 0.0;
     }
 }
 
@@ -1571,37 +1598,53 @@
     const int64_t *slice_off;
     const int32_t *cols;
     const double *vals;
+    const int32_t *agg, *mem_ptr, *mem_idx;
+    bool mat;
+    const int64_t *lds_slice_off;
+    const int32_t *lds_cols;
+    const double *lds_vals;
 };
-__device__ inline TailView tail_view(const AmgTail &T, int l, int use_lds, int64_t mat_slots, double *lds)
+__host__ __device__ inline int64_t tail_idx_ints(const AmgTail &T, int q)
+{
+    return (q + 1 < T.nlev && !T.lev[q].rbm_dim) ? 2 * T.lev[q].n + T.lev[q + 1].n + 1 : 0;
+}
+template <bool kLds, bool kMat>
+__device__ inline TailView tail_view(const AmgTail &T, int l, int64_t mat_slots, double *lds)
 {
     const AmgTailLevel &L = T.lev[l];
-    TailView V{L.x, L.dd, L.t, L.r, L.b, L.dinv, L.A.slice_off, L.A.cols, L.A.vals};
-    if (use_lds) {
-        int64_t off = 0, tot = 0;
+    TailView V{L.x, L.dd, L.t, L.r, L.b, L.dinv, L.A.slice_off, L.A.cols, L.A.vals, L.agg, L.mem_ptr, L.mem_idx, false, nullptr, nullptr, nullptr};
+    if (kLds) {
+        int64_t off = 0, tot = 0, ioff = 0, itot = 0;
         for (int q = 0; q < T.nlev; ++q) {
-            if (q < l) off += 6 * T.lev[q].n;
+            if (q < l) { off += 6 * T.lev[q].n; ioff += tail_idx_ints(T, q); }
             tot += 6 * T.lev[q].n;
+            itot += tail_idx_ints(T, q);
         }
         double *base = lds + off;
         const int64_t n = L.n;
         V.x = base; V.dd = base + n; V.t = base + 2 * n; V.r = base + 3 * n; V.b = base + 4 * n; V.dinv = base + 5 * n;
-        if (l == 0 && mat_slots > 0) {
-            double *mv = lds + tot;
+        int32_t *ib = reinterpret_cast<int32_t *>(lds + tot) + ioff;
+        V.mem_ptr = ib;
+        V.mem_idx = ib + (l + 1 < T.nlev ? T.lev[l + 1].n + 1 : 0);
+        V.agg = V.mem_idx + n;
+        if (kMat) {
+            double *mv = lds + tot + ((itot + 1) >> 1);
             int64_t *so = reinterpret_cast<int64_t *>(mv + mat_slots);
-            V.vals = mv;
-            V.slice_off = so;
-            V.cols = reinterpret_cast<int32_t *>(so + L.A.n_slices + 1);
+            V.mat = l == 0;
+            V.lds_vals = mv;
+            V.lds_slice_off = so;
+            V.lds_cols = reinterpret_cast<int32_t *>(so + T.lev[0].A.n_slices + 1);
         }
     }
     return V;
 }
-__device__ inline void tail_spmv(const TailView &V, int64_t n_rows, const double *x, double *y)
+__device__ __forceinline__ void tail_spmv_rows(const int64_t *slice_off, const int32_t *cols, const double *vals, int64_t n_rows, const double *x, double *y)
 {
     for (int64_t i = threadIdx.x; i < n_rows; i += 1024) {
-        const int64_t off = V.slice_off[i >> 6];
-        const int width = static_cast<int>((V.slice_off[(i >> 6) + 1] - off) >> 6);
-        const int32_t *cp = V.cols + off + (i & 63);
-        const double *vp = V.vals + off + (i & 63);
+        const int64_t off = slice_off[i >> 6];
+        const int width = static_cast<int>((slice_off[(i >> 6) + 1] - off) >> 6);
+        const int32_t *cp = cols + off + (i & 63);
+        const double *vp = vals + off + (i & 63);
         double acc = 0.0;
         int k = 0;
         for (; k + 8 <= width; k += 8) {
@@ -1617,6 +1660,11 @@
         for (; k < width; ++k) acc = __builtin_fma(vp[64 * k], x[cp[64 * k]], acc);
         y[i] = acc;
     }
+}
+__device__ inline void tail_spmv(const TailView &V, int64_t n_rows, const double *x, double *y)
+{
+    if (V.mat) tail_spmv_rows(V.lds_slice_off, V.lds_cols, V.lds_vals, n_rows, x, y);
+    else tail_spmv_rows(V.slice_off, V.cols, V.vals, n_rows, x, y);
     __syncthreads();
 }
 __device__ inline void tail_smooth(const AmgTailLevel &L, const TailView &V, const double *b, bool zero_guess, int deg, double ratio, double lmax)
@@ -1663,21 +1711,25 @@
         else rbm_prolong_node<3, 2>(i, L.node_agg, L.roff, L.nn, VC.x, scale, V.x);
     }
 }
-__global__ void __launch_bounds__(1024) k_amg_tail(const AmgTail T, const CgCtl *ctl, int use_lds, int64_t mat_slots)
+template <bool kLds, bool kMat>
+__global__ void __launch_bounds__(1024) k_amg_tail(const AmgTail T, const CgCtl *ctl, int64_t mat_slots)
 {
     extern __shared__ double tail_lds[];
-    if (ctl && ctl->flag != 0) return;
+    const int stop = ctl ? ctl->flag : 0;
+    if (!kLds && stop != 0) return;
     const int nl = T.nlev;
     __shared__ double lam_of[kAmgTailLevels];
     if (threadIdx.x < static_cast<unsigned>(nl)) lam_of[threadIdx.x] = T.lev[threadIdx.x].lam[0];
-    if (!use_lds) __syncthreads();
-    if (use_lds) {
-        if (mat_slots > 0) {
+    if (!kLds) __syncthreads();
+    if (kLds) {
+        double warm = 0.0;
+        if (T.dense_n > 0 && 16 * static_cast<int>(threadIdx.x) < T.dense_n * T.dense_n) warm = T.dense_inv[16 * threadIdx.x];
+        if (kMat) {
             const AmgTailLevel &L = T.lev[0];
-            const TailView V = tail_view(T, 0, use_lds, mat_slots, tail_lds);
-            double *mv = const_cast<double *>(V.vals);
-            int32_t *mc = const_cast<int32_t *>(V.cols);
-            int64_t *so = const_cast<int64_t *>(V.slice_off);
+            const TailView V = tail_view<kLds, kMat>(T, 0, mat_slots, tail_lds);
+            double *mv = const_cast<double *>(V.lds_vals);
+            int32_t *mc = const_cast<int32_t *>(V.lds_cols);
+            int64_t *so = const_cast<int64_t *>(V.lds_slice_off);
             const double *__restrict__ gv = L.A.vals;
             const int32_t *__restrict__ gc = L.A.cols;
             for (int64_t q0 = threadIdx.x; q0 < mat_slots; q0 += 8 * 1024) {
@@ -1699,24 +1751,40 @@
         }
         for (int l = 0; l < nl; ++l) {
             const AmgTailLevel &L = T.lev[l];
-            const TailView V = tail_view(T, l, use_lds, mat_slots, tail_lds);
+            const TailView V = tail_view<kLds, kMat>(T, l, mat_slots, tail_lds);
             double *dv = const_cast<double *>(V.dinv);
             for (int64_t i = threadIdx.x; i < L.n; i += 1024) {
                 dv[i] = L.dinv[i];
                 if (l == 0) V.b[i] = L.b[i];
             }
-        }
+            if (tail_idx_ints(T, l) > 0) {
+                int32_t *mp = const_cast<int32_t *>(V.mem_ptr), *mi = const_cast<int32_t *>(V.mem_idx), *ag = const_cast<int32_t *>(V.agg);
+                for (int64_t i = threadIdx.x; i < L.n; i += 1024) { mi[i] = L.mem_idx[i]; ag[i] = L.agg[i]; }
+                for (int64_t a = threadIdx.x; a <= T.lev[l + 1].n; a += 1024) mp[a] = L.mem_ptr[a];
+            }
+        }
+        asm volatile("" ::"v"(warm));
         __syncthreads();
+        if (stop != 0) return;
     }
     for (int l = 0; l < nl; ++l) {
         const AmgTailLevel &L = T.lev[l];
-        const TailView V = tail_view(T, l, use_lds, mat_slots, tail_lds);
+        const TailView V = tail_view<kLds, kMat>(T, l, mat_slots, tail_lds);
         if (l == nl - 1) {
             if (T.dense_n > 0) {
                 const int n = T.dense_n;
                 for (int i = threadIdx.x; i < n; i += 1024) {
+                    const double *__restrict__ col = T.dense_inv + i;
                     double a = 0.0;
-                    for (int j = 0; j < n; ++j) a = __builtin_fma(T.dense_inv[j * n + i], V.b[j], a);
+                    int j = 0;
+                    for (; j + 16 <= n; j += 16) {
+                        double m[16];
+#pragma unroll
+                        for (int u = 0; u < 16; ++u) m[u] = col[(j + u) * n];
+#pragma unroll
+                        for (int u = 0; u < 16; ++u) a = __builtin_fma(m[u], V.b[j + u], a);
+                    }
+                    for (; j < n; ++j) a = __builtin_fma(col[j * n], V.b[j], a);
                     V.x[i] = a;
                 }
                 __syncthreads();
@@ -1726,15 +1794,15 @@
             break;
         }
         const AmgTailLevel &C = T.lev[l + 1];
-        const TailView VC = tail_view(T, l + 1, use_lds, mat_slots, tail_lds);
+        const TailView VC = tail_view<kLds, kMat>(T, l + 1, mat_slots, tail_lds);
         tail_smooth(L, V, V.b, true, T.deg, T.ratio, lam_of[l]);
         tail_spmv(V, L.n, V.x, V.t);
         if (L.rbm_dim) tail_rbm_restrict(L, V, C, VC);
         else
         for (int64_t a = threadIdx.x; a < C.n; a += 1024) {
             double acc = 0.0;
-            for (int q = L.mem_ptr[a]; q < L.mem_ptr[a + 1]; ++q) {
-                const int i = L.mem_idx[q];
+            for (int q = V.mem_ptr[a]; q < V.mem_ptr[a + 1]; ++q) {
+                const int i = V.mem_idx[q];
                 acc += V.b[i] - V.t[i];
             }
             VC.b[a] = acc;
@@ -1743,16 +1811,16 @@
     }
     for (int l = nl - 2; l >= 0; --l) {
         const AmgTailLevel &L = T.lev[l];
-        const TailView V = tail_view(T, l, use_lds, mat_slots, tail_lds);
-        const TailView VC = tail_view(T, l + 1, use_lds, mat_slots, tail_lds);
+        const TailView V = tail_view<kLds, kMat>(T, l, mat_slots, tail_lds);
+        const TailView VC = tail_view<kLds, kMat>(T, l + 1, mat_slots, tail_lds);
         if (L.rbm_dim) tail_rbm_prolong(L, V, VC, T.scale);
         else
-        for (int64_t i = threadIdx.x; i < L.n; i += 1024) V.x[i] = __builtin_fma(T.scale, VC.x[L.agg[i]], V.x[i]);
+        for (int64_t i = threadIdx.x; i < L.n; i += 1024) V.x[i] = __builtin_fma(T.scale, VC.x[V.agg[i]], V.x[i]);
         __syncthreads();
         tail_smooth(L, V, V.b, false, T.deg, T.ratio, lam_of[l]);
     }
-    if (use_lds) {
-        const TailView V = tail_view(T, 0, use_lds, mat_slots, tail_lds);
+    if (kLds) {
+        const TailView V = tail_view<kLds, kMat>(T, 0, mat_slots, tail_lds);
         double *x_out = T.lev[0].x;
         for (int64_t i = threadIdx.x; i < T.lev[0].n; i += 1024) x_out[i] = V.x[i];
     }
diff --git a/pfemfort_amd/csrc/pfem_amg_types.hpp b/pfemfort_amd/csrc/pfem_amg_types.hpp
--- a/pfemfort_amd/csrc/pfem_amg_types.hpp
+++ b/pfemfort_amd/csrc/pfem_amg_types.hpp
@@ -71,6 +71,7 @@
     bool vd_hash_ok = false;
     bool vd_direct = false;
     bool bound_fresh = false;
+    bool bound_done = false;
     double *x = nullptr, *dd = nullptr;
     DevBuf<double> x1;
     double lam_host = 0.0;
@@ -99,6 +100,9 @@
     }
     int tail_from = -1;
     size_t tail_lds_allowed = 0;
+    size_t tail_vec_allowed = 0;
+    int tail_build = 0;
+    int bounds_by_products = 0;
     int cycle_gamma = 1, w_to = -1;
     bool cycle_given = false;
     bool fused = true;
diff --git a/pfemfort_amd/csrc/pfem_device.hip b/pfemfort_amd/csrc/pfem_device.hip
--- a/pfemfort_amd/csrc/pfem_device.hip
+++ b/pfemfort_amd/csrc/pfem_device.hip
@@ -4779,3 +4779,14 @@
     *last_level_visited_twice = M.cycle_gamma > 1 ? std::min(M.w_to, static_cast<int>(M.lev.size()) - 2) : 0;
     return PFEM_OK;
 }
+extern "C" int pfem_solver_amg_tail_from(pfem_solver *s, int *tail_from, int *tail_build, int *bounds_by_products)
+{
+    if (!s || !tail_from || !tail_build || !bounds_by_products) return PFEM_ERR_ARG;
+    if (!s->amg || !s->amg->symbolic_ok) return PFEM_ERR_STATE;
+    const Amg &M = *s->amg;
+    const bool tail = M.fused && M.tail_from > 0;
+    *tail_from = tail ? M.tail_from : -1;
+    *tail_build = tail ? M.tail_build : 0;
+    *bounds_by_products = M.bounds_by_products;
+    return PFEM_OK;
+}
diff --git a/pfemfort_amd/solver.py b/pfemfort_amd/solver.py
--- a/pfemfort_amd/solver.py
+++ b/pfemfort_amd/solver.py
@@ -215,10 +215,17 @@
         L.check(L.lib().pfem_solver_set_amg_cycle(self._h, code), "pfem_solver_set_amg_cycle")
 
     def amgCycle(self):
-        c, w, e = C.c_int(0), C.c_int(0), C.c_int(0)
+        c, w, e, t, tb, bp = C.c_int(0), C.c_int(0), C.c_int(0), C.c_int(-1), C.c_int(0), C.c_int(0)
         L.check(L.lib().pfem_solver_amg_cycle(self._h, C.byref(c), C.byref(w)), "pfem_solver_amg_cycle")
         L.check(L.lib().pfem_solver_amg_level0_epilogue(self._h, C.byref(e)), "pfem_solver_amg_level0_epilogue")
-        return {"cycle": "w" if c.value == 2 else "v", "last_level_visited_twice": w.value, "level0_epilogue": bool(e.value)}
+        L.check(L.lib().pfem_solver_amg_tail_from(self._h, C.byref(t), C.byref(tb), C.byref(bp)), "pfem_solver_amg_tail_from")
+        return {"cycle": "w" if c.value == 2 else "v", "last_level_visited_twice": w.value, "level0_epilogue": bool(e.value),
+                "tail_from": t.value, "tail_build": [None, "memory", "lds", "lds+matrix"][tb.value]}
+
+    def amgBoundsByProducts(self):
+        t, tb, bp = C.c_int(-1), C.c_int(0), C.c_int(0)
+        L.check(L.lib().pfem_solver_amg_tail_from(self._h, C.byref(t), C.byref(tb), C.byref(bp)), "pfem_solver_amg_tail_from")
+        return bp.value
 
     def amgTransfer(self, level, xyz=False):
         rbm, fb, cb, dim = C.c_int(0), C.c_int(0), C.c_int(0), C.c_int(0)
```

Result: faster. 650.5 million (median of 6 runs) (+2.8%).
